# jypjypjypjyp/lvio_fusion

Measured on AMD Instinct MI355X. Metric: local-BA iters/sec (50 KF x 10k pts) + ICP Mpairs/sec, higher is better.
Workload: dtype f64; 1 GPU; configs[3]: full sliding-window LM iteration, 50 keyframes x 10 000 landmarks (10000 TwoCamera + 71789 TwoFrame + 9629 PoseOnly + 49 IMU factors), device-resident LM loop, one independent window per GPU; n_kf=50, n_lm=10000, parallelism=1 independent windows

## Files before the change

### lvio_fusion_amd/csrc/solver_kernels.hip

```cpp
#include <hip/hip_ext.h>
#include <algorithm>
#include <chrono>
#include <cmath>
#include <cstdlib>
#include <memory>
#include <unordered_map>

#include "factor_eval.hpp"
#include "prior_eval.hpp"
#include "lvf_internal.hpp"
#include "imu_eval.hpp"

namespace lvf {
struct TfWork;
struct LmCtl;
struct Chain;
struct StageClock;
struct SpNode { int col, row_off, m, id; };
constexpr int kSpMaxLevels = 12, kSpMaxRows = 768;
struct SpLevels { int n; int first[kSpMaxLevels]; int count[kSpMaxLevels]; };
struct JacobiDev { GP<double> h0; GP<const int> frozen; };
struct SpSrc {
  GP<const double> B; int ldB, dp; GP<const double> gc; GP<const double> radius; GP<const int> rows_nat;
  GP<int> wait_counter; int wait_target; GP<int> done_counter;
  int fenced; unsigned timeout_ticks;
  int strip_end;
  int rmw_read;
  GP<unsigned long long> dbg;
  int s_zero;
  JacobiDev jac{nullptr, nullptr};
};
struct SpArgs {
  GP<const SpNode> nodes; int first, tiles; GP<const int> rows; GP<double> S; int ld; GP<double> W; int wstride; GP<double> Lout; GP<int> fail; int nblocks; GP<const int> done;
  SpSrc src;
};
__device__ __forceinline__ void sp_ride(const int vb, const SpArgs& a);
constexpr int kFailSparse = 100000, kFailHandover = 300000;
}
struct lvf_problem {
  lvf_ctx* ctx = nullptr;
  lvf_state* st = nullptr;
  lvf_batch *tc = nullptr, *tf = nullptr, *po = nullptr, *imu = nullptr, *prior = nullptr;
  int n_kf = 0, n_lm = 0, d = 0, dp = 0, ldE = 0, dpad = 0, nb = 0;
  int ld = 0, off = 0, off_pose = 0, ndense = 0, aug = 0, sp_wstride = 0;
  lvf::SpLevels sp_levels{};
  std::vector<int> sp_tiles, sp_shmem;
  std::vector<int> sp_item0, sp_items;
  std::vector<int32_t> plan_key;
  lvf::DevBuf<lvf::SpNode> sp_nodes;
  lvf::DevBuf<int> sp_rows, sp_rows_nat, sp_owner, perm, iperm;
  lvf::DevBuf<int> lm_kmin, lm_kmax, lm_order, lm_nactive;
  bool band_ready = false;
  bool compact = false;
  lvf::DevBuf<int> lm_eoff, n_slots, tf_slot, run_first;
  lvf::DevBuf<double> slotB, slabP, slabQ, Ct, grt;
  lvf::StageClock* clk = nullptr;
  bool accum_clean = false;
  const double* chain_tcw = nullptr;
  int band_rows = 64;
  lvf::DevBuf<int4> band_work; lvf::DevBuf<int> n_band_work_dev; lvf::HostPin<int> h_n_band_work;
  int n_band_work = 0, band_rows_built = 0;
  bool band_pending = false; hipEvent_t ev_band = nullptr;
  int band_epoch = 0;
  std::vector<lvf_problem_batch*> batches;
  lvf::HostPin<int> h_run_first;
  lvf::DevBuf<unsigned long long> dbg, dbg_lin, dbg_sp;
  lvf::DevBuf<double> dbg_hist;
  lvf::DevBuf<double> sp_sync;
  lvf::DevBuf<double> sp_W, sp_L, Dinv;
  lvf::DevBuf<double> Ldiag;
  std::vector<int> perm_h;
  lvf::DevBuf<double> B, gc, C, gr, E, Cd, S, dxc, dxl, scal;
  lvf::DevBuf<double> jh0;
  lvf::DevBuf<double> poses2, vel2, ba2, bg2, invd2;
  lvf::DevBuf<uint8_t> pose_const;
  lvf::DevBuf<int> fail;
  lvf::DevBuf<lvf::TfWork> tf_work;
  lvf::HostPin<lvf::TfWork> h_tf_work;
  std::vector<uint8_t> pose_const_h;
  bool linearized = false;
  lvf::DevBuf<double2> tfs_fo, tfs_ob;
  lvf::DevBuf<int> tfs_lm, tfs_k1, tfs_k2, tfs_perm;
  lvf::HostPin<int> h_tfs_perm;
  bool tf_sorted_copy = false;
  const double2* tf_fo() const { return tf_sorted_copy ? tfs_fo.p : (const double2*)tf->ob_a.p; }
  const double2* tf_ob() const { return tf_sorted_copy ? tfs_ob.p : (const double2*)tf->ob_b.p; }
  const int* tf_lm() const { return tf_sorted_copy ? tfs_lm.p : tf->idx_a.p; }
  const int* tf_k1() const { return tf_sorted_copy ? tfs_k1.p : tf->idx_b.p; }
  const int* tf_k2() const { return tf_sorted_copy ? tfs_k2.p : tf->idx_c.p; }
  bool tf_unique_lk2 = false;
  bool tf_k1_first = false;
  double last_radius = 0;
  lvf::DevBuf<lvf::LmCtl> ctl;
  lvf::LmCtl* rec = nullptr;
  lvf::HostPin<lvf::LmCtl> h_ctl;
  lvf::Chain* chain = nullptr;
  bool chain_ready = false;
  bool no_chain = false;
  int unchained_solves = 0;
  int handover_retries = 0;
  int force_handover_timeouts = 0;
  const void* chain_state[6] = {nullptr, nullptr, nullptr, nullptr, nullptr, nullptr};
  double huber = 1.0;
  hipGraphExec_t graph_exec = nullptr;
  ~lvf_problem();
};

namespace lvf {

constexpr int kT = 256;
typedef double double4_t __attribute__((ext_vector_type(4)));
constexpr int kStripes = 32;
enum { SC_COST = 0, SC_COST_NEW = 1 * kStripes, SC_MODEL = 2 * kStripes, SC_DXNORM = 3 * kStripes, SC_XNORM = 4 * kStripes, SC_GMAX = 5 * kStripes,
       SC_N = 6 * kStripes, SC_FAIL = SC_N , SC_TICKET = SC_N + 1 , SC_ALLOC = SC_N + 2 };
static inline double stripe_sum(const double* h, int slot) { double s = 0.0; for (int k = 0; k < kStripes; ++k) s += h[slot + k]; return s; }

__device__ __forceinline__ int done_flag_issue(const int* done) { return done ? *reinterpret_cast<const volatile int*>(done) : 0; }

__device__ __forceinline__ void block_add(double v, double* dst) {
  v = wave_sum(v);
  if ((threadIdx.x & 63) == 0 && v != 0.0) atomicAdd(dst + ((blockIdx.x + blockIdx.y) & (kStripes - 1)), v);
}

struct StateP { GP<const double> poses, vel, ba, bg, inv_depth, w_kf; };

struct LmCtl {
  double radius, decrease;
  double last_radius;
  double cost, initial_cost;
  double cost_before, cost_after, model, dxnorm, xnorm, gmax;
  double huber, function_tol, gradient_tol, parameter_tol, min_rel_decrease;
  int max_iters;
  int iter, successes, invalid_run;
  int accepted, solved;
  int done, termination;
  int why, rejected;
  int jfrozen;
};

__device__ __forceinline__ void add_block66(double* __restrict__ B, int ld, int ra, int rb, const double Ja[12], const double Jb[12]) {
#pragma unroll
  for (int i = 0; i < 6; ++i)
#pragma unroll
    for (int j = 0; j < 6; ++j) {
      if (ra == rb && j > i) continue;
      atomicAdd(&B[(size_t)(ra + i) * ld + rb + j], Ja[i] * Jb[j] + Ja[6 + i] * Jb[6 + j]);
    }
}

__device__ __forceinline__ void zero_lower(double* __restrict__ p, const int ld, const unsigned long long wave, const unsigned long long n_waves) {
  const int lane = threadIdx.x & 63;
  for (unsigned long long r = wave; r < (unsigned long long)ld; r += n_waves) {
    double2* row = reinterpret_cast<double2*>(p + r * (unsigned long long)ld);
    const int end2 = min(ld, (((int)r | 63) + 1)) / 2;
    for (int c = lane; c < end2; c += 64) row[c] = make_double2(0.0, 0.0);
  }
}
__global__ __launch_bounds__(kT) void k_zero_multi(ZeroList z) {
  double* p = z.p[blockIdx.y];
  if (z.tri[blockIdx.y] > 0) { zero_lower(p, z.tri[blockIdx.y], (unsigned long long)blockIdx.x * (kT / 64) + (threadIdx.x >> 6), (unsigned long long)gridDim.x * (kT / 64)); return; }
  const unsigned long long n = z.n[blockIdx.y], n2 = n / 2;
  double2* p2 = reinterpret_cast<double2*>(p);
  for (unsigned long long i = (unsigned long long)blockIdx.x * kT + threadIdx.x; i < n2; i += (unsigned long long)gridDim.x * kT) p2[i] = make_double2(0.0, 0.0);
  if ((n & 1) && blockIdx.x == 0 && threadIdx.x == 0) p[n - 1] = 0.0;
}
__global__ __launch_bounds__(kT) void k_zero_multi_ranges(ZeroList z, int n_lm, int* __restrict__ kmin, int* __restrict__ kmax) {
  if ((int)blockIdx.y == z.count) {
    for (int l = blockIdx.x * kT + threadIdx.x; l < n_lm; l += gridDim.x * kT) { kmin[l] = 0x7fffffff; kmax[l] = -1; }
    return;
  }
  double* p = z.p[blockIdx.y];
  const unsigned long long n = z.n[blockIdx.y], n2 = n / 2;
  double2* p2 = reinterpret_cast<double2*>(p);
  for (unsigned long long i = (unsigned long long)blockIdx.x * kT + threadIdx.x; i < n2; i += (unsigned long long)gridDim.x * kT) p2[i] = make_double2(0.0, 0.0);
  if ((n & 1) && blockIdx.x == 0 && threadIdx.x == 0) p[n - 1] = 0.0;
}
__device__ __forceinline__ void zero_list_share(const ZeroList& zero, const int wg, const int n_wgs) {
  const unsigned long long t = (unsigned long long)wg * kT + threadIdx.x, nt = (unsigned long long)n_wgs * kT;
#pragma unroll
  for (int a = 0; a < kZeroListMax; ++a) {
    if (a >= zero.count) break;
    double* p = zero.p[a];
    if (zero.tri[a] > 0) { zero_lower(p, zero.tri[a], (unsigned long long)wg * (kT / 64) + (threadIdx.x >> 6), (unsigned long long)n_wgs * (kT / 64)); continue; }
    const unsigned long long cnt = zero.n[a], n2 = cnt / 2;
    double2* p2 = reinterpret_cast<double2*>(p);
    for (unsigned long long i = t; i < n2; i += nt) p2[i] = make_double2(0.0, 0.0);
    if ((cnt & 1) && t == 0) p[cnt - 1] = 0.0;
  }
}
__global__ __launch_bounds__(kT) void k_zero_table(const ZeroList* __restrict__ t) { zero_list_share(t[blockIdx.y], blockIdx.x, gridDim.x); }

template <bool COST_ONLY>
__device__ __forceinline__ void lin_tc_body(const int vb, int n, const double2* __restrict__ lo, const double2* __restrict__ ro,
                                               const int* __restrict__ lm, const int* __restrict__ kf, const double* __restrict__ wblk, StateP s,
                                               CamD left, CamD right, double huber, double* __restrict__ C,
                                               double* __restrict__ gr, double* __restrict__ cost) {
  const int i = vb * kT + threadIdx.x;
  double c = 0.0;
  if (i < n) {
    const int l = lm[i];
    const double2 a = lo[i], b = ro[i];
    double r[2], J[2];
    eval_two_camera<!COST_ONLY>(left, right, a.x, a.y, b.x, b.y, s.inv_depth[l], wblk ? wblk[i] : 5.0 * s.w_kf[kf[i]], r, J);
    double rho;
    const double sc = robust_scale(huber, r[0] * r[0] + r[1] * r[1], rho);
    c = 0.5 * rho;
    if (!COST_ONLY) {
      const double s2 = sc * sc;
      atomicAdd(&C[l], s2 * (J[0] * J[0] + J[1] * J[1]));
      atomicAdd(&gr[l], s2 * (J[0] * r[0] + J[1] * r[1]));
    }
  }
  block_add(c, cost);
}
template <bool COST_ONLY>
__global__ __launch_bounds__(kT) void k_lin_tc(int n, const double2* __restrict__ lo, const double2* __restrict__ ro,
                                               const int* __restrict__ lm, const int* __restrict__ kf, const double* __restrict__ wblk, StateP s,
                                               CamD left, CamD right, double huber, double* __restrict__ C,
                                               double* __restrict__ gr, double* __restrict__ cost) { lin_tc_body<COST_ONLY>(blockIdx.x, n, lo, ro, lm, kf, wblk, s, left, right, huber, C, gr, cost); }

// ... 467 lines not shown
                                               int ld, double* __restrict__ gc, double* __restrict__ cost) { lin_po_body<COST_ONLY>(blockIdx.x, n, n_kf, ob, kf, pwi, pw, s, cam, huber, pose_const, B, ld, gc, cost); }

struct ImuJ { GP<const double> j[8]; };
__global__ __launch_bounds__(64) void k_lin_imu(int n, int n_kf, const double* __restrict__ res, ImuJ J, const int* __restrict__ kf_i,
                                                const int* __restrict__ kf_j, const double* __restrict__ poses,
                                                const uint8_t* __restrict__ pose_const, double* __restrict__ B, int ld,
                                                double* __restrict__ gc, double* __restrict__ cost) {
  __shared__ double sJ[15 * 30];
  __shared__ double sr[15];
  __shared__ int sidx[30];
  const int f = blockIdx.x, lane = threadIdx.x;
  const int ki = kf_i[f], kj = kf_j[f];
  if (lane < 15) sr[lane] = res[(size_t)f * 15 + lane];
  if (lane < 30) {
    int g;
    if (lane < 6) g = 6 * ki + lane; else if (lane < 15) g = 6 * n_kf + 9 * ki + (lane - 6);
    else if (lane < 21) g = 6 * kj + (lane - 15); else g = 6 * n_kf + 9 * kj + (lane - 21);
    sidx[lane] = g;
  }
  for (int e = lane; e < 30; e += 64) {
    const int row = e % 15, which = e / 15;
    const double* Jr = (which ? J.j[4] : J.j[0]) + (size_t)f * 105 + 7 * row;
    const int kk = which ? kj : ki;
    const double* q = poses + 7 * kk;
    const double sc = (pose_const[kk] & 1) ? 0.0 : 1.0;
    double l3[3];
    quat_row_to_local(Jr, q, l3);
    double* o = sJ + row * 30 + (which ? 15 : 0);
    o[0] = sc * l3[0]; o[1] = sc * l3[1]; o[2] = sc * l3[2]; o[3] = sc * Jr[4]; o[4] = sc * Jr[5]; o[5] = sc * Jr[6];
  }
  for (int e = lane; e < 15 * 18; e += 64) {
    const int row = e / 18, c = e % 18, blk = c / 3, cc = c % 3;
    const int src = blk < 3 ? 1 + blk : 5 + (blk - 3);
    const double* jp = src == 1 ? J.j[1] : (src == 2 ? J.j[2] : (src == 3 ? J.j[3] : (src == 5 ? J.j[5] : (src == 6 ? J.j[6] : J.j[7]))));
    const double scv = ((pose_const[blk < 3 ? ki : kj] >> (1 + blk % 3)) & 1) ? 0.0 : 1.0;
    sJ[row * 30 + (blk < 3 ? 6 + 3 * blk : 21 + 3 * (blk - 3)) + cc] = scv * jp[(size_t)f * 45 + 3 * row + cc];
  }
  __syncthreads();
  double c = 0.0;
  if (lane < 15) c = 0.5 * sr[lane] * sr[lane];
  c = wave_sum(c);
  if (lane == 0) atomicAdd(cost + (blockIdx.x & (kStripes - 1)), c);
  for (int e = lane; e < 30 * 30; e += 64) {
    const int a = e / 30, b = e % 30;
    const int ga = sidx[a], gb = sidx[b];
    if (gb > ga || (ga == gb && a != b)) continue;
    double h = 0.0;
#pragma unroll
    for (int k = 0; k < 15; ++k) h += sJ[k * 30 + a] * sJ[k * 30 + b];
    atomicAdd(&B[(size_t)ga * ld + gb], h);
  }
  if (lane < 30) {
    double g = 0.0;
#pragma unroll
    for (int k = 0; k < 15; ++k) g += sJ[k * 30 + lane] * sr[k];
    atomicAdd(&gc[sidx[lane]], g);
  }
}

template <bool DYN = false>
__device__ __forceinline__ void lin_imu_body4(const int vb, int n, int n_kf, const double* __restrict__ res, ImuJ J, const int* __restrict__ kf_i,
                                              const int* __restrict__ kf_j, const double* __restrict__ poses,
                                              const uint8_t* __restrict__ pose_const, double* __restrict__ B, int ld,
                                              double* __restrict__ gc, double* __restrict__ cost) {
  __shared__ double sJ4[DYN ? 1 : 4 * 15 * 30];
  __shared__ double sr4[DYN ? 1 : 4 * 16];
  __shared__ int sidx4[DYN ? 1 : 4 * 32];
  extern __shared__ double lin_lds[];
  const int w = threadIdx.x >> 6, lane = threadIdx.x & 63;
  const int f = 4 * vb + w;
  const bool active = f < n;
  double* sJ = (DYN ? lin_lds : sJ4) + w * 450;
  double* sr = (DYN ? lin_lds + 1800 : sr4) + w * 16;
  int* sidx = (DYN ? reinterpret_cast<int*>(lin_lds + 1864) : sidx4) + w * 32;
  if (active) {
    const int ki = kf_i[f], kj = kf_j[f];
    if (lane < 15) sr[lane] = res[(size_t)f * 15 + lane];
    if (lane < 30) {
      int g;
      if (lane < 6) g = 6 * ki + lane; else if (lane < 15) g = 6 * n_kf + 9 * ki + (lane - 6);
      else if (lane < 21) g = 6 * kj + (lane - 15); else g = 6 * n_kf + 9 * kj + (lane - 21);
      sidx[lane] = g;
    }
    for (int e = lane; e < 30; e += 64) {
      const int row = e % 15, which = e / 15;
      const double* Jr = (which ? J.j[4] : J.j[0]) + (size_t)f * 105 + 7 * row;
      const int kk = which ? kj : ki;
      const double* q = poses + 7 * kk;
      const double sc = (pose_const[kk] & 1) ? 0.0 : 1.0;
      double l3[3];
      quat_row_to_local(Jr, q, l3);
      double* o = sJ + row * 30 + (which ? 15 : 0);
      o[0] = sc * l3[0]; o[1] = sc * l3[1]; o[2] = sc * l3[2]; o[3] = sc * Jr[4]; o[4] = sc * Jr[5]; o[5] = sc * Jr[6];
    }
    for (int e = lane; e < 15 * 18; e += 64) {
      const int row = e / 18, c = e % 18, blk = c / 3, cc = c % 3;
      const int src = blk < 3 ? 1 + blk : 5 + (blk - 3);
      const double* jp = src == 1 ? J.j[1] : (src == 2 ? J.j[2] : (src == 3 ? J.j[3] : (src == 5 ? J.j[5] : (src == 6 ? J.j[6] : J.j[7]))));
      const double scv = ((pose_const[blk < 3 ? ki : kj] >> (1 + blk % 3)) & 1) ? 0.0 : 1.0;
      sJ[row * 30 + (blk < 3 ? 6 + 3 * blk : 21 + 3 * (blk - 3)) + cc] = scv * jp[(size_t)f * 45 + 3 * row + cc];
    }
  }
  __syncthreads();
  double c = 0.0;
  if (active && lane < 15) c = 0.5 * sr[lane] * sr[lane];
  c = wave_sum(c);
  if (!active) return;
  if (lane == 0) atomicAdd(cost + (f & (kStripes - 1)), c);
  for (int e = lane; e < 30 * 30; e += 64) {
    const int a = e / 30, b = e % 30;
    const int ga = sidx[a], gb = sidx[b];
    if (gb > ga || (ga == gb && a != b)) continue;
    double h = 0.0;
#pragma unroll
    for (int k = 0; k < 15; ++k) h += sJ[k * 30 + a] * sJ[k * 30 + b];
    atomicAdd(&B[(size_t)ga * ld + gb], h);
  }
  if (lane < 30) {
    double g = 0.0;
#pragma unroll
    for (int k = 0; k < 15; ++k) g += sJ[k * 30 + lane] * sr[k];
    atomicAdd(&gc[sidx[lane]], g);
  }
}

constexpr int kEndZeroWgs = 192;
constexpr int kImuWaveLds = 225 + 480 + 480 + 16 + 16 + 16 + 248 + 32 + 2;
__device__ __forceinline__ void lin_imu_eval_body(const int f, const ImuEvalArgs& I, int n_kf, const StateP& s, const uint8_t* __restrict__ pose_const,
                                                  double* __restrict__ B, int ld, double* __restrict__ gc, double* __restrict__ cost, unsigned long long* dbg) {
  extern __shared__ double lin_lds[];
  const int tid = threadIdx.x;
  if (f >= I.n) return;
  if (f != 0 || tid != 0) dbg = nullptr;
  if (dbg) dbg[0] = wall_clock64();
  double* sS = lin_lds;
  double* sM = sS + 225;
  double* sJw = sM + 480;
  double* sr0 = sJw + 480;
  double* sr = sr0 + 16;
  int* sidx = reinterpret_cast<int*>(sr + 16);
  double* sP = reinterpret_cast<double*>(sidx + 32);
  double* sX = sP + 248;
  const int ki = I.kf_i[f], kj = I.kf_j[f];
  for (int k = tid; k < 225; k += kT) sS[k] = I.sqrt_info[(size_t)f * 225 + k];
  for (int k = tid; k < OFF_COV; k += kT) sP[k] = I.pre[(size_t)f * kPre + k];
  if (tid < 32) {
    const int kk = tid < 16 ? ki : kj, c = tid & 15;
    sX[tid] = c < 7 ? s.poses[7 * kk + c] : (c < 10 ? s.vel[3 * kk + c - 7] : (c < 13 ? s.ba[3 * kk + c - 10] : s.bg[3 * kk + c - 13]));
  }
  int* smask = reinterpret_cast<int*>(sX + 32);
  if (tid >= 32 && tid < 34) smask[tid - 32] = pose_const[tid == 32 ? ki : kj];
  for (int k = tid; k < 480; k += kT) sM[k] = 0.0;
  __syncthreads();
  if (dbg) dbg[1] = wall_clock64();
  if (tid == 0) imu_raw16<true>(sP, sX, sr0, sM);
  __syncthreads();
  if (dbg) dbg[2] = wall_clock64();
  {
    const double r = imu_weighted_residual(tid, sS, sr0);
    if (tid < 15) sr[tid] = r;
    for (int e = tid; e < 480; e += kT) sJw[e] = imu_weighted_jacobian(e, sS, sM);
    if (tid < 30) {
      int g;
      if (tid < 6) g = 6 * ki + tid; else if (tid < 15) g = 6 * n_kf + 9 * ki + (tid - 6);
      else if (tid < 21) g = 6 * kj + (tid - 15); else g = 6 * n_kf + 9 * kj + (tid - 21);
      sidx[tid] = g;
    }
  }
  __syncthreads();
  double* sJ = sM;
  if (tid < 30) {
    const int row = tid % 15, which = tid / 15;
    const double* Jr = sJw + 32 * row + (which ? 16 : 0);
    const double sc = (smask[which] & 1) ? 0.0 : 1.0;
    double l3[3];
    quat_row_to_local(Jr, sX + 16 * which, l3);
    double* o = sJ + row * 30 + (which ? 15 : 0);
    o[0] = sc * l3[0]; o[1] = sc * l3[1]; o[2] = sc * l3[2]; o[3] = sc * Jr[4]; o[4] = sc * Jr[5]; o[5] = sc * Jr[6];
  }
  for (int e = tid; e < 15 * 18; e += kT) {
    const int row = e / 18, c = e % 18;
    const int cg = c < 9 ? c / 3 : (c - 9) / 3;
    const double scv = ((smask[c < 9 ? 0 : 1] >> (1 + cg)) & 1) ? 0.0 : 1.0;
    sJ[row * 30 + (c < 9 ? 6 + c : 21 + (c - 9))] = scv * sJw[32 * row + (c < 9 ? 7 + c : 23 + (c - 9))];
  }
  __syncthreads();
  if (dbg) dbg[3] = wall_clock64();
  if (tid < 64) {
    double c = tid < 15 ? 0.5 * sr[tid] * sr[tid] : 0.0;
    c = wave_sum(c);
    if (tid == 0) atomicAdd(cost + (f & (kStripes - 1)), c);
  }
  for (int e = tid; e < 30 * 30; e += kT) {
    const int a = e / 30, b = e % 30;
    const int ga = sidx[a], gb = sidx[b];
    if (gb > ga || (ga == gb && a != b)) continue;
    double h = 0.0;
#pragma unroll
    for (int k = 0; k < 15; ++k) h += sJ[k * 30 + a] * sJ[k * 30 + b];
    atomicAdd(&B[(size_t)ga * ld + gb], h);
  }
  if (tid < 30) {
    double g = 0.0;
#pragma unroll
    for (int k = 0; k < 15; ++k) g += sJ[k * 30 + tid] * sr[k];
    atomicAdd(&gc[sidx[tid]], g);
  }
  if (dbg) dbg[4] = wall_clock64();
}

struct LinVisual {
  int n_tfw, g_tc;
  GP<const TfWork> work; GP<const double2> tf_fo, tf_ob; GP<const int> tf_lm, tf_k1; CamD tf_left, tf_right; int unique_lk2; TfCompact cp;
  int n_tc; GP<const double2> tc_lo, tc_ro; GP<const int> tc_lm, tc_kf; GP<const double> tc_w; CamD tc_left, tc_right;
  int n_po, g_po; GP<const double2> po_ob; GP<const int> po_kf, po_pwi; GP<const double> po_pw; CamD po_cam;
  int n_imu; GP<const double> imu_res; ImuJ imu_J; GP<const int> imu_i, imu_j; ImuEvalArgs imu;
};
struct LinArgs {
  LinVisual v; int n_kf; StateP s; double huber; GP<const uint8_t> pose_const; GP<double> B; int ld; GP<double> gc; GP<double> E; int ldE; GP<double> C, gr, cost;
  int nblocks; GP<const int> done; GP<unsigned long long> dbg; int rows;
  GP<double> scal_reset;
};
__device__ __forceinline__ void reset_step_scalars(double* scal) {
  for (int k = SC_COST_NEW + threadIdx.x; k < SC_N; k += kT) scal[k] = 0.0;
  if (threadIdx.x == 0) { *reinterpret_cast<int*>(scal + SC_FAIL) = 0; *reinterpret_cast<int*>(scal + SC_TICKET) = 0; }
}
__device__ __forceinline__ void lin_visual_body(const int bx, const LinArgs& A) {
  if (bx >= A.nblocks || (A.done && *A.done)) return;
  if (bx == 0 && A.scal_reset) reset_step_scalars(A.scal_reset);
  const LinVisual& a = A.v;
  const int g_imu_first = a.imu.pre ? a.n_imu : 0;
  const int b = bx - g_imu_first;
  const int n_kf = A.n_kf; const StateP s = A.s; const double huber = A.huber; const uint8_t* pose_const = A.pose_const;
  double* B = A.B; const int ld = A.ld; double* gc = A.gc; double* E = A.E; const int ldE = A.ldE; double* C = A.C; double* gr = A.gr; double* cost = A.cost;
  if (bx < g_imu_first)
    lin_imu_eval_body(bx, a.imu, n_kf, s, pose_const, B, ld, gc, cost, A.dbg ? A.dbg + (size_t)a.n_tfw * 8 : nullptr);
  else if (b < a.n_tfw)
    lin_tf_sorted_body<true>(b, a.work, n_kf, a.tf_fo, a.tf_ob, a.tf_lm, a.tf_k1, s, a.tf_left, a.tf_right, huber, pose_const, B, ld, gc, E, ldE, C, gr, cost,
                       a.unique_lk2, A.dbg, a.cp, a.n_tfw);
  else if (b < a.n_tfw + a.g_tc)
    lin_tc_body<false>(b - a.n_tfw, a.n_tc, a.tc_lo, a.tc_ro, a.tc_lm, a.tc_kf, a.tc_w, s, a.tc_left, a.tc_right, huber, C, gr, cost);
  else if (b < a.n_tfw + a.g_tc + a.g_po)
    lin_po_body<false, true>(b - a.n_tfw - a.g_tc, a.n_po, n_kf, a.po_ob, a.po_kf, a.po_pwi, a.po_pw, s, a.po_cam, huber, pose_const, B, ld, gc, cost);
  else
    lin_imu_body4<true>(b - a.n_tfw - a.g_tc - a.g_po, a.n_imu, n_kf, a.imu_res, a.imu_J, a.imu_i, a.imu_j, s.poses, pose_const, B, ld, gc, cost);
}
__global__ __launch_bounds__(kT) __attribute__((amdgpu_waves_per_eu(3))) void k_lin_visual(LinArgs a) { lin_visual_body(blockIdx.x, a); }
__global__ __launch_bounds__(kT) __attribute__((amdgpu_waves_per_eu(3))) void k_lin_visual_b(const LinArgs* __restrict__ t) { lin_visual_body(blockIdx.x, t[blockIdx.y]); }
__global__ __launch_bounds__(kT) __attribute__((amdgpu_waves_per_eu(3))) void k_lin_visual_bt(const LinArgs* __restrict__ t) { lin_visual_body(blockIdx.y, t[blockIdx.x]); }

struct TfReduceArgs {
  int n_kf, n_wg; GP<const int> run_first; GP<const double> slabP, slabQ; GP<double> B; int ld; GP<double> gc; int nblocks; GP<const int> done;
  int own_blocks; SpArgs ride;
};
__device__ __forceinline__ void tf_reduce_body(const int bx0, const TfReduceArgs& A) {
  if (bx0 >= A.nblocks || (A.done && *A.done)) return;
  if (bx0 < A.ride.nblocks) { sp_ride(bx0, A.ride); return; }
  const int bx = bx0 - A.ride.nblocks;
  const int n_kf = A.n_kf;
  const int nchunk = (A.n_wg + 63) / 64;
  if (bx < n_kf * nchunk) {
    __shared__ double part[8][32];
    const int k = bx / nchunk, c = bx - k * nchunk, v = threadIdx.x & 31, g = threadIdx.x >> 5;
    const int r0 = A.run_first[k], r1 = A.run_first[k + 1];
    double acc = 0.0;
    if (v < 27) {
      const double* slabP = A.slabP; const double* slabQ = A.slabQ;
      double t8[8]; bool keep[8];
#pragma unroll
      for (int u = 0; u < 8; ++u) {
        const int wg = 64 * c + g + 8 * u, wgc = min(wg, A.n_wg - 1);
        const bool useP = wgc >= r1;
        keep[u] = (wg < A.n_wg) & (wgc >= r0);
        const double* src = useP ? slabP + ((size_t)wgc * n_kf + k) * kSlabRow + v : slabQ + (size_t)wgc * kSlabQ + v;
        t8[u] = *src;
      }
#pragma unroll
      for (int u = 0; u < 8; ++u) acc = keep[u] ? acc + t8[u] : acc;
    }
    part[g][v] = acc;
    __syncthreads();
    if (threadIdx.x < 27) {
      double t = 0.0;
#pragma unroll
      for (int q = 0; q < 8; ++q) t += part[q][threadIdx.x];
      if (t != 0.0) {
        if (threadIdx.x < 21) {
          int x = 0, rem = threadIdx.x;
          while (rem > x) { rem -= x + 1; ++x; }
          atomicAdd(&A.B[(size_t)(6 * k + x) * A.ld + 6 * k + rem], t);
        } else atomicAdd(&A.gc[6 * k + threadIdx.x - 21], t);
      }
    }
    return;
  }
  const int e = (bx - n_kf * nchunk) * kT + threadIdx.x;
  const int npair = n_kf * (n_kf - 1) / 2;
  if (e >= npair * 36) return;
  const int pr = e / 36, el = e - 36 * pr;
  int k2 = (int)((1.0 + sqrt(1.0 + 8.0 * pr)) * 0.5);
  while (k2 * (k2 - 1) / 2 > pr) --k2;
  while ((k2 + 1) * k2 / 2 <= pr) ++k2;
  const int k1 = pr - k2 * (k2 - 1) / 2;
  double acc = 0.0;
  {
    const double* slabP = A.slabP;
    const int w0 = A.run_first[k2], w1 = A.run_first[k2 + 1];
    for (int wg = w0; wg < w1; wg += 4) {
      double t4[4];
#pragma unroll
      for (int u = 0; u < 4; ++u) t4[u] = slabP[((size_t)min(wg + u, w1 - 1) * n_kf + k1) * kSlabRow + 27 + el];
#pragma unroll
      for (int u = 0; u < 4; ++u) acc = (wg + u < w1) ? acc + t4[u] : acc;
    }
  }
  if (acc != 0.0) {
    const int x = el / 6, y = el - 6 * x;
    A.B[(size_t)(6 * k2 + x) * A.ld + 6 * k1 + y] += acc;
  }
}
__global__ __launch_bounds__(kT) void k_tf_reduce(TfReduceArgs a) { tf_reduce_body(blockIdx.x, a); }
__global__ __launch_bounds__(kT) void k_tf_reduce_b(const TfReduceArgs* __restrict__ t) { tf_reduce_body(blockIdx.x, t[blockIdx.y]); }
__global__ __launch_bounds__(kT) void k_tf_reduce_bt(const TfReduceArgs* __restrict__ t) { tf_reduce_body(blockIdx.y, t[blockIdx.x]); }


__device__ __forceinline__ void lin_prior_block(const int i, const int a, const int b, const double* __restrict__ res, const double* __restrict__ ja,
                                                const double* __restrict__ jb, const double* __restrict__ poses, const uint8_t* __restrict__ pose_const,
                                                double* __restrict__ B, int ld, double* __restrict__ gc, double* __restrict__ cost) {
  double r[6], La[36], Lb[36];
  double c = 0.0;
  for (int k = 0; k < 6; ++k) { r[k] = res[k]; c += 0.5 * r[k] * r[k]; }
  for (int k = 0; k < 6; ++k) {
    const double* row = jb + 7 * k;
    const double sc = (pose_const[b] & 1) ? 0.0 : 1.0;
    double l3[3];
    quat_row_to_local(row, poses + 7 * b, l3);
    Lb[6 * k] = sc * l3[0]; Lb[6 * k + 1] = sc * l3[1]; Lb[6 * k + 2] = sc * l3[2];
    Lb[6 * k + 3] = sc * row[4]; Lb[6 * k + 4] = sc * row[5]; Lb[6 * k + 5] = sc * row[6];
    if (a >= 0) {
      const double* rowa = ja + 7 * k;
      const double sa = (pose_const[a] & 1) ? 0.0 : 1.0;
      quat_row_to_local(rowa, poses + 7 * a, l3);
      La[6 * k] = sa * l3[0]; La[6 * k + 1] = sa * l3[1]; La[6 * k + 2] = sa * l3[2];
      La[6 * k + 3] = sa * rowa[4]; La[6 * k + 4] = sa * rowa[5]; La[6 * k + 5] = sa * rowa[6];
    }
  }
  atomicAdd(cost + (i & (kStripes - 1)), c);
  for (int x = 0; x < 6; ++x) {
    double g = 0.0;
    for (int k = 0; k < 6; ++k) g += Lb[6 * k + x] * r[k];
    atomicAdd(&gc[6 * b + x], g);
    for (int y = 0; y <= x; ++y) {
      double h = 0.0;
      for (int k = 0; k < 6; ++k) h += Lb[6 * k + x] * Lb[6 * k + y];
      atomicAdd(&B[(size_t)(6 * b + x) * ld + 6 * b + y], h);
    }
  }
  if (a >= 0) {
    for (int x = 0; x < 6; ++x) {
      double g = 0.0;
      for (int k = 0; k < 6; ++k) g += La[6 * k + x] * r[k];
      atomicAdd(&gc[6 * a + x], g);
      for (int y = 0; y <= x; ++y) {
        double h = 0.0;
        for (int k = 0; k < 6; ++k) h += La[6 * k + x] * La[6 * k + y];
        atomicAdd(&B[(size_t)(6 * a + x) * ld + 6 * a + y], h);
      }
      for (int y = 0; y < 6; ++y) {
        double h = 0.0;
        for (int k = 0; k < 6; ++k) h += La[6 * k + x] * Lb[6 * k + y];
        if (a > b) atomicAdd(&B[(size_t)(6 * a + x) * ld + 6 * b + y], h);
        else atomicAdd(&B[(size_t)(6 * b + y) * ld + 6 * a + x], h);
      }
    }
  }
}
__global__ __launch_bounds__(64) void k_lin_prior(int n, const double* __restrict__ res, const double* __restrict__ ja,
                                                  const double* __restrict__ jb, const int* __restrict__ kf_a, const int* __restrict__ kf_b,
                                                  const double* __restrict__ poses, const uint8_t* __restrict__ pose_const,
                                                  double* __restrict__ B, int ld, double* __restrict__ gc, double* __restrict__ cost) {
  const int i = blockIdx.x * 64 + threadIdx.x;
  if (i >= n) return;
  lin_prior_block(i, kf_a[i], kf_b[i], res + 6 * i, ja + (size_t)42 * i, jb + (size_t)42 * i, poses, pose_const, B, ld, gc, cost);
}
struct PriorArgs { int n; GP<const int> kf_a, kf_b; GP<const double> target, weight, vv; };
__global__ __launch_bounds__(64) void k_prior_lin(PriorArgs P, const double* __restrict__ poses, const uint8_t* __restrict__ pose_const,
                                                  double* __restrict__ B, int ld, double* __restrict__ gc, double* __restrict__ cost) {
  const int i = blockIdx.x * 64 + threadIdx.x;
  if (i >= P.n) return;
  double res[6], ja[42], jb[42];
  const int a = P.kf_a[i], b = P.kf_b[i];
  pose_prior_eval<true>(a, b, P.target + 7 * i, P.weight[i], P.vv[i], poses, res, ja, jb);
  lin_prior_block(i, a, b, res, ja, jb, poses, pose_const, B, ld, gc, cost);
}
__global__ __launch_bounds__(64) void k_prior_cost(PriorArgs P, const double* __restrict__ poses, double* __restrict__ cost) {
  const int i = blockIdx.x * 64 + threadIdx.x;
  if (i >= P.n) return;
  double res[6];
  pose_prior_eval<false>(P.kf_a[i], P.kf_b[i], P.target + 7 * i, P.weight[i], P.vv[i], poses, res, nullptr, nullptr);
  double c = 0.0;
  for (int k = 0; k < 6; ++k) c += 0.5 * res[k] * res[k];
  atomicAdd(cost + (i & (kStripes - 1)), c);
}
__global__ __launch_bounds__(kT) void k_cost_sq(int n, const double* __restrict__ res, double* __restrict__ cost) {
  const int i = blockIdx.x * kT + threadIdx.x;
  double c = 0.0;
  if (i < n) { const double r = res[i]; c = 0.5 * r * r; }
  block_add(c, cost);
}

__device__ __forceinline__ double lm_damping(double h, double h0) {
  if (h >= 2e-6 * (1.0 + h0) && h < 1e32) return h;
  if (h0 == 0.0) return fmin(fmax(h, 1e-6), 1e32);
  const double sj = 1.0 / (1.0 + sqrt(h0)), s2 = sj * sj;
  return fmin(fmax(h * s2, 1e-6), 1e32) / s2;
}
__device__ __forceinline__ double lm_damping_own(double h, const JacobiDev& j, int slot, int frozen, double h0_loaded) {
  double h0 = h0_loaded;
  if (!frozen) { h0 = h; j.h0[slot] = h; }
  return lm_damping(h, h0);
}

struct PrepArgs {
  int ld, dpad, jl0 ; GP<const int> iperm; GP<const double> B, gc; GP<const double> radius; GP<double> S; unsigned nS_blocks; int n_lm, dp, ldE; GP<const double> C, gr;
  GP<double> Cd, E, scal; int nblocks; GP<const int> done;
  GP<const int> eoff, kmin, kmax; GP<const double> slotB; GP<double> Ct, grt;
  int early, off;
  int own_blocks; SpArgs ride;
  JacobiDev jac;
};
__device__ __forceinline__ void prepare_body(const unsigned bx0, const PrepArgs& A) {
  if (bx0 >= (unsigned)A.nblocks || (A.done && *A.done)) return;
  if (bx0 < (unsigned)A.ride.nblocks) { sp_ride((int)bx0, A.ride); return; }
  const unsigned bx = bx0 - (unsigned)A.ride.nblocks;
  const int ld = A.ld, dpad = A.dpad; const int* __restrict__ iperm = A.iperm; const double* __restrict__ B = A.B; const double* __restrict__ gc = A.gc;
  const double inv_radius = 1.0 / *A.radius;
  const int jf = *A.jac.frozen;
  double* __restrict__ S = A.S; const unsigned nS_blocks = A.nS_blocks; const int n_lm = A.n_lm, dp = A.dp, ldE = A.ldE;
  const double* __restrict__ C = A.C; const double* __restrict__ gr = A.gr; double* __restrict__ Cd = A.Cd; double* __restrict__ E = A.E; double* __restrict__ scal = A.scal;
  if (bx == 0 && scal) reset_step_scalars(scal);
  if (bx >= nS_blocks) {
    if (A.slotB) {
      const int l = ((bx - nS_blocks) * kT + threadIdx.x) >> 3, j0 = threadIdx.x & 7;
      const bool live = l < n_lm;
      const int lc = live ? l : 0;
      const int k1 = A.kmin[lc], len = live ? max(0, A.kmax[lc] - k1) : 0;
      const double h0l = A.jac.h0[A.jl0 + lc];
      const double2* sb = reinterpret_cast<const double2*>(A.slotB + (size_t)A.eoff[lc] * 8);
      double v[8] = {0, 0, 0, 0, 0, 0, 0, 0};
      for (int j = j0; j < len; j += 8) {
        const double2 b0 = sb[4 * j], b1 = sb[4 * j + 1], b2 = sb[4 * j + 2], cg = sb[4 * j + 3];
        v[0] += cg.x; v[1] += cg.y; v[2] += b0.x; v[3] += b0.y; v[4] += b1.x; v[5] += b1.y; v[6] += b2.x; v[7] += b2.y;
      }
#pragma unroll
      for (int q = 0; q < 8; ++q) { v[q] = quad_sum(v[q]); v[q] += quad_perm<0x141>(v[q]); }
      if (live && j0 == 0) {
        const double c = C[l] + v[0], g = gr[l] + v[1];
        A.Ct[l] = c; A.grt[l] = g;
        Cd[l] = c + lm_damping_own(c, A.jac, A.jl0 + l, jf, h0l) * inv_radius;
        double* el = E + (size_t)l * ldE;
        el[dp] = g;
        if (len > 0) {
#pragma unroll
          for (int q = 0; q < 6; ++q) el[6 * k1 + q] = v[2 + q];
        }
      }
      return;
    }
    const int l = (bx - nS_blocks) * kT + threadIdx.x;
    if (l >= n_lm) return;
    const double c = C[l], h0l = A.jac.h0[A.jl0 + l];
    Cd[l] = c + lm_damping_own(c, A.jac, A.jl0 + l, jf, h0l) * inv_radius;
    E[(size_t)l * ldE + dp] = gr[l];
    return;
  }
  const size_t e = (size_t)bx * kT + threadIdx.x;
  const int n0 = A.early ? A.off : 0, nn = ld - n0;
  const int half = (nn + 1) / 2;
  if (e >= (size_t)half * (nn + 1)) return;
  const int q = (int)(e / (nn + 1)), cc = (int)(e % (nn + 1));
  int I, J;
  if (cc <= q) { I = q; J = cc; }
  else { I = nn - 1 - q; J = cc - q - 1; if (I == q) return; }
  I += n0; J += n0;
  const int oi = iperm[I], oj = iperm[J];
  double v = 0.0;
  if (oi >= 0) {
    if (oj >= 0 && J <= I) {
      const double h0d = I == J ? A.jac.h0[oi] : 0.0;
      v = B[(size_t)max(oi, oj) * dpad + min(oi, oj)];
      if (I == J) v += lm_damping_own(v, A.jac, oi, jf, h0d) * inv_radius;
    }
  } else if (oi == -2) {
    v = (oj >= 0) ? -gc[oj] : (J == I ? 1e300 : 0.0);
  } else if (I == J) {
    v = 1.0;
  }
  if (!A.early) S[(size_t)I * ld + J] = v;
  else if (v != 0.0) atomicAdd(&S[(size_t)I * ld + J], v);
}
__global__ __launch_bounds__(kT) void k_prepare(PrepArgs a) { prepare_body(blockIdx.x, a); }
__global__ __launch_bounds__(kT) void k_prepare_b(const PrepArgs* __restrict__ t) { prepare_body(blockIdx.x, t[blockIdx.y]); }
__global__ __launch_bounds__(kT) void k_prepare_bt(const PrepArgs* __restrict__ t) { const PrepArgs a = t[blockIdx.x]; prepare_body(blockIdx.y, a); }

constexpr int kSchurChunk = 512;
__global__ __launch_bounds__(64) void k_schur_syrk(int n_lm, int dp, int ldE, int ntile, const double* __restrict__ E,
                                                   const double* __restrict__ Cd, int d, int ldS, double* __restrict__ S) {
  int t = blockIdx.x, ti = 0;
  while (t >= ti + 1) { t -= ti + 1; ++ti; }
  const int tj = t;
  const int lane = threadIdx.x, lk = lane >> 4, lc = lane & 15;
  const int k_begin = blockIdx.y * kSchurChunk, k_end = min(n_lm, k_begin + kSchurChunk);
  double4_t acc = {0.0, 0.0, 0.0, 0.0};
  for (int k0 = k_begin; k0 < k_end; k0 += 4) {
    const int l = k0 + lk;
    double a = 0.0, b = 0.0;
    if (l < k_end) {
      const double* row = E + (size_t)l * ldE;
      a = row[ti * 16 + lc] / Cd[l];
      b = row[tj * 16 + lc];
    }
    acc = __builtin_amdgcn_mfma_f64_16x16x4f64(a, b, acc, 0, 0, 0);
  }
#pragma unroll
  for (int r = 0; r < 4; ++r) {
    const int gi = ti * 16 + lk + 4 * r, gj = tj * 16 + lc;
    const double v = acc[r];
    if (v == 0.0) continue;
    if (gi < dp && gj < dp) { if (gj <= gi) atomicAdd(&S[(size_t)gi * ldS + gj], -v); }
    else if (gi == dp && gj < dp) atomicAdd(&S[(size_t)d * ldS + gj], v);
  }
}

constexpr int kSchurGroups = 8, kSchurTilesPerWave = 8, kSchurRows = 16;
__global__ __launch_bounds__(256) void k_schur_lds(int n_lm, int dp, int ldE, int ntile, int rows_per_slice, const double* __restrict__ E,
                                                   const double* __restrict__ Cd, int d, int ldS, double* __restrict__ S) {
  extern __shared__ double sh[];
  double* Es = sh;
  double* icd = sh + kSchurRows * ldE;
  const int tid = threadIdx.x, w = tid >> 6, lane = tid & 63, lk = lane >> 4, lc = lane & 15;
  const int g = blockIdx.x, slice = blockIdx.y;
  const int k_begin = slice * rows_per_slice, k_end = min(n_lm, k_begin + rows_per_slice);
  int ti[kSchurTilesPerWave], tj[kSchurTilesPerWave], nt = 0;
#pragma unroll
  for (int s_ = 0; s_ < kSchurTilesPerWave; ++s_) {
    const int t = g + kSchurGroups * (w + 4 * s_);
    ti[s_] = 0; tj[s_] = 0;
    if (t < ntile) {
      int a = (int)((sqrt(8.0 * t + 1.0) - 1.0) * 0.5);
      while ((a + 1) * (a + 2) / 2 <= t) ++a;
      while (a * (a + 1) / 2 > t) --a;
      ti[s_] = a; tj[s_] = t - a * (a + 1) / 2;
      nt = s_ + 1;
    }
  }
  double4_t acc[kSchurTilesPerWave];
#pragma unroll
  for (int s_ = 0; s_ < kSchurTilesPerWave; ++s_) acc[s_] = double4_t{0.0, 0.0, 0.0, 0.0};
  const int per_row = ldE;
  const int total = kSchurRows * per_row;
  constexpr int kPf = 20;
  double pf[kPf];
  auto fetch = [&](int k0) {
#pragma unroll
    for (int u = 0; u < kPf; ++u) {
      const int e = tid + 256 * u;
      double v = 0.0;
      if (e < total) { const int rr = e / per_row, cc = e - rr * per_row; if (k0 + rr < k_end) v = E[(size_t)(k0 + rr) * ldE + cc]; }
      pf[u] = v;
    }
  };
  auto fetch_tail = [&](int k0) {
    for (int e = tid + 256 * kPf; e < total; e += 256) {
      const int rr = e / per_row, cc = e - rr * per_row;
      Es[e] = (k0 + rr < k_end) ? E[(size_t)(k0 + rr) * ldE + cc] : 0.0;
    }
  };
  if (k_begin < k_end) fetch(k_begin);
  for (int k0 = k_begin; k0 < k_end; k0 += kSchurRows) {
    __syncthreads();
#pragma unroll
    for (int u = 0; u < kPf; ++u) { const int e = tid + 256 * u; if (e < total) Es[e] = pf[u]; }
    fetch_tail(k0);
    if (tid < kSchurRows) icd[tid] = (k0 + tid < k_end) ? 1.0 / Cd[k0 + tid] : 0.0;
    __syncthreads();
    if (k0 + kSchurRows < k_end) fetch(k0 + kSchurRows);
// ... 732 lines not shown
        for (int c = 0; c < 9; ++c) { const int oj = nb0 + c; sv[c] += src.B[(size_t)max(oi, oj) * src.ldB + min(oi, oj)]; }
      }
    }
    finish_row(r, sv);
  }
  if (tile == 0 && tid < 9) {
    double xcol[9];
#pragma unroll
    for (int r = 0; r < 9; ++r) {
      double v = (r == tid) ? 1.0 : 0.0;
#pragma unroll
      for (int k = 0; k < r; ++k) v -= L[r * 9 + k] * xcol[k];
      xcol[r] = v * linv[r];
    }
#pragma unroll
    for (int r = 0; r < 9; ++r) Lout[(size_t)ni * 81 + r * 9 + tid] = xcol[r];
  }
  __syncthreads();
  int ns = 0;
  if (src.done_counter && src.strip_end > 0) {
    int lo = 0, hi = m;
    while (lo < hi) { const int mid = (lo + hi) >> 1; if (rws[mid] < src.strip_end) lo = mid + 1; else hi = mid; }
    ns = lo;
  }
  auto pair_value = [&](const int r, const int c2) {
    const double* wr = Ws + r * 9;
    const double* wc = Ws + c2 * 9;
    double v = 0.0;
#pragma unroll
    for (int c = 0; c < 9; ++c) v += wr[c] * wc[c];
    return v;
  };
  auto pair_update = [&](const int r, const int c2) {
    const double v = pair_value(r, c2);
    if (v != 0.0) atomicAdd(&S[(size_t)rws[r] * ld + rws[c2]], -v);
  };
  if (ns > 0) {
    double sink = 0.0;
    for (int q = tile * 256 + tid; q < ns * m; q += tiles * 256) {
      const int r = q / ns, c2 = q - r * ns;
      if (r >= c2) {
        const double v = pair_value(r, c2);
        if (v != 0.0) sink += __hip_atomic_fetch_add(&S[(size_t)rws[r] * ld + rws[c2]], -v, __ATOMIC_RELAXED, __HIP_MEMORY_SCOPE_AGENT);
      }
    }
    if (sink == -1.2345678901234567e301) atomicMax(fail, 50000);
  }
  if (stamp) stamp[5] = wall_clock64();
  if (src.done_counter) {
    __syncthreads();
    if (tid == 0) {
      if (src.fenced) __hip_atomic_fetch_add((int*)src.done_counter, 1, __ATOMIC_RELEASE, __HIP_MEMORY_SCOPE_AGENT);
      else __hip_atomic_fetch_add((int*)src.done_counter, 1, __ATOMIC_RELAXED, __HIP_MEMORY_SCOPE_AGENT);
    }
  }
  if (stamp) stamp[6] = wall_clock64();
  const int m2 = m - ns, P = m2 * (m2 + 1) / 2;
  for (int p = tile * 256 + tid; p < P; p += tiles * 256) {
    int r = (int)((sqrt(8.0 * p + 1.0) - 1.0) * 0.5);
    while ((r + 1) * (r + 2) / 2 <= p) ++r;
    while (r * (r + 1) / 2 > p) --r;
    const int c2 = p - r * (r + 1) / 2;
    pair_update(r + ns, c2 + ns);
  }
  if (stamp) { asm volatile("s_waitcnt vmcnt(0)" ::: "memory"); stamp[7] = wall_clock64(); }
}
__global__ __launch_bounds__(64) void k_band_work(int rows, int dp, const int* __restrict__ n_active_p, const int* __restrict__ order,
                                                  const int* __restrict__ kmin, const int* __restrict__ kmax, int4* __restrict__ work, int* __restrict__ n_work) {
  const int n_active = *n_active_p, lane = threadIdx.x;
  const int k_begin = blockIdx.x * rows, k_end = min(n_active, k_begin + rows);
  if (k_begin >= k_end) return;
  int lo = 0x7fffffff, hi = -1;
  for (int r = k_begin + lane; r < k_end; r += 64) { const int l = order[r]; lo = min(lo, kmin[l]); hi = max(hi, kmax[l]); }
  for (int o = 32; o > 0; o >>= 1) { lo = min(lo, __shfl_xor(lo, o)); hi = max(hi, __shfl_xor(hi, o)); }
  if (lane == 0) {
    const int t0 = (6 * lo) >> 4, t1 = (6 * hi + 5) >> 4, tl = dp >> 4, nbt = t1 - t0 + 1;
    const int ntiles = nbt * (nbt + 1) / 2 + (tl > t1 ? nbt : 0);
    const int groups = (ntiles + kBandTilesPerGroup - 1) / kBandTilesPerGroup;
    const int base = atomicAdd(n_work, groups);
    for (int g = 0; g < groups; ++g) work[base + g] = make_int4((int)blockIdx.x, g, lo | (hi << 16), k_end);
  }
}

__device__ __forceinline__ void sp_ride(const int vb, const SpArgs& a) {
  if (vb >= a.nblocks) return;
  sp_eliminate_body(vb, a.nodes, a.first, a.tiles, a.rows, a.S, a.ld, a.W, a.wstride, a.Lout, a.fail, a.done, a.src);
}
__global__ __launch_bounds__(256) void k_sp_eliminate(SpArgs a) { sp_ride(blockIdx.x, a); }
__global__ __launch_bounds__(256) void k_sp_eliminate_b(const SpArgs* __restrict__ t) { sp_ride(blockIdx.x, t[blockIdx.y]); }
struct SchurSp0Args {
  int n_slices, n_groups, dp, ldE; GP<const double> E, Cd; GP<const int> order, n_active, kmin, kmax; int d_local, ldS; GP<double> S_pose;
  SpArgs sp;
  SpArgs sp_b, sp_c;
  int nblocks; GP<const int> done; GP<unsigned long long> dbg; int rows;
  GP<const int4> work; int n_work;
};
__device__ __forceinline__ void schur_sp0_body(const int b, const SchurSp0Args& A) {
  if (b >= A.nblocks) return;
  if (A.work) {
    const int n_a = A.sp.nblocks, n_b = A.sp_b.nblocks, n_c = A.sp_c.nblocks, n_sp = n_a + n_b + n_c;
    if (b < n_a) sp_ride(b, A.sp);
    else if (b < n_a + n_b) sp_ride(b - n_a, A.sp_b);
    else if (b < n_sp) sp_ride(b - n_a - n_b, A.sp_c);
    else {
      const int dv = done_flag_issue(A.done);
      const int4* item = A.work + (b - n_sp);
      const int4 it = *item;
      if (dv) return;
      schur_band_body(it.x, it.y, A.dp, A.ldE, A.E, A.Cd, A.order, A.n_active, A.kmin, A.kmax, A.d_local, A.ldS, A.S_pose, A.dbg ? A.dbg + (size_t)(b - n_sp) * 8 : nullptr, A.rows, item);
    }
    return;
  }
  if (A.done && *A.done) return;
  const int ns = A.n_slices * A.n_groups;
  if (b < ns) schur_band_body(b % A.n_slices, b / A.n_slices, A.dp, A.ldE, A.E, A.Cd, A.order, A.n_active, A.kmin, A.kmax, A.d_local, A.ldS, A.S_pose, A.dbg ? A.dbg + (size_t)b * 8 : nullptr, A.rows);
  else sp_ride(b - ns, A.sp);
}
__global__ __launch_bounds__(256) __attribute__((amdgpu_waves_per_eu(2))) void k_schur_sp0(SchurSp0Args a) { schur_sp0_body(blockIdx.x, a); }
__global__ __launch_bounds__(256) __attribute__((amdgpu_waves_per_eu(2))) void k_schur_sp0_b(const SchurSp0Args* __restrict__ t) { schur_sp0_body(blockIdx.x, t[blockIdx.y]); }
__global__ __launch_bounds__(256) __attribute__((amdgpu_waves_per_eu(2))) void k_schur_sp0_bt(const SchurSp0Args* __restrict__ t) { schur_sp0_body(blockIdx.y, t[blockIdx.x]); }
struct SpBack {
  SpLevels lv;
  int item0[kSpMaxLevels], items[kSpMaxLevels];
  GP<const SpNode> nodes; GP<const int> rows; GP<const int> owner; GP<const double> W; GP<const double> Linv; GP<const int> perm;
  int off, aug, d_total, total_items, n_nodes, max_count, linv_in_lds;
  int prod_items;
  GP<unsigned long long> dbg;
};

__device__ __forceinline__ void lds_barrier() { asm volatile("s_waitcnt lgkmcnt(0)\n\ts_barrier" ::: "memory"); }

template <typename T>
__device__ __forceinline__ T ld_off32(const T* base, unsigned byte_off) {
  return *reinterpret_cast<const T*>(reinterpret_cast<const char*>(base) + byte_off);
}
constexpr int kBT = 512, kBParts = kBT / 64, kBackPre = 256 / kBParts, kBackInv = 64 / kBParts, kTailPre = 6;
struct BackArgs { GP<const double> Sd; int ld, d; GP<const double> Dinv; GP<double> xout; SpBack sp; GP<const int> done; GP<const double> Ldiag; GP<int> pose_ready = nullptr; int n_pose = 0; int pose_fenced = 0; };
__device__ __forceinline__ void chol_backsolve_body(const BackArgs& A) {
  const int dv = done_flag_issue(A.done);
  const double* S = A.Sd; const int ld = A.ld, d = A.d; const double* Dinv = A.Dinv; double* xout = A.xout; const SpBack& sp = A.sp;
  extern __shared__ double sm[];
  const int tid = threadIdx.x, c = tid & 63, part = tid >> 6;
  const int nblk = (d + kNB - 1) / kNB, n = nblk * kNB;
  double* x = sm + sp.off;
  double* partial = x + n;
  double* rhs = partial + kBParts * kNB;
  double* accs = rhs + kNB;
  double* linv = accs + 9 * sp.max_count;
  double* part1 = linv + (sp.linv_in_lds ? 81 * sp.n_nodes : 0);
  double* prod = part1 + kBT;
  int* snode = reinterpret_cast<int*>(prod + 9 * (size_t)sp.prod_items);
  int stamp = 0;
  auto mark = [&]() { if (sp.dbg && tid == 0) sp.dbg[stamp++] = wall_clock64(); };
  mark();
  const int rend = min(n, d);
  double gl[kBackPre], xi[kBackInv], yv;
  const int part_u = __builtin_amdgcn_readfirstlane(part);
  const unsigned c_off = 8u * (unsigned)c;
  auto prefetch = [&](int kb) {
    const int r0 = kb * kNB, below = nblk - 1 - kb;
    const double* row = S + (size_t)(r0 + kNB + part_u) * ld + r0;
#pragma unroll
    for (int g = 0; g < kBackPre / 8; ++g)
      if (g < below) {
#pragma unroll
        for (int j = 0; j < 8; ++j) gl[8 * g + j] = ld_off32(row + (size_t)(kBParts * (8 * g + j)) * ld, c_off);
      }
    const double* dv = Dinv + (size_t)kb * kNB * kNB + kBackInv * part_u;
#pragma unroll
    for (int t = 0; t < kBackInv; ++t) xi[t] = ld_off32(dv + t, (unsigned)kNB * c_off);
    const double* yrow = (d / kNB == kb) ? A.Ldiag + (size_t)kb * kNB * kNB + (size_t)(d - r0) * kNB : S + (size_t)d * ld + r0;
    yv = (r0 + c < d) ? ld_off32(yrow, c_off) : 0.0;
  };
  prefetch(nblk - 1);
  constexpr int kLinvPre = 8;
  double lpre[kLinvPre];
  const int n_linv = sp.linv_in_lds ? 81 * sp.n_nodes : 0;
#pragma unroll
  for (int u = 0; u < kLinvPre; ++u) { const int i = tid + kBT * u; lpre[u] = i < n_linv ? ld_off32((const double*)sp.Linv, 8u * (unsigned)i) : 0.0; }
  SpNode ndpre = SpNode{0, 0, 0, 0};
  if (tid < sp.n_nodes) ndpre = sp.nodes[tid];
#pragma unroll
  for (int u = 0; u < kLinvPre; ++u) { const int i = tid + kBT * u; if (i < n_linv) linv[i] = lpre[u]; }
  for (int i = tid + kBT * kLinvPre; i < n_linv; i += kBT) linv[i] = sp.Linv[i];
  if (tid < sp.n_nodes) { snode[2 * tid] = ndpre.row_off; snode[2 * tid + 1] = ndpre.m; }
  for (int i = tid + kBT; i < sp.n_nodes; i += kBT) { const SpNode nd = sp.nodes[i]; snode[2 * i] = nd.row_off; snode[2 * i + 1] = nd.m; }
  asm volatile("" ::: "memory");
  int tR[kTailPre], tK[kTailPre];
  double tW[kTailPre][9];
#pragma unroll
  for (int u = 0; u < kTailPre; ++u) {
    const int g = tid + kBT * u;
    const bool ok = g < sp.total_items;
    tR[u] = -1; tK[u] = 0;
#pragma unroll
    for (int q = 0; q < 9; ++q) tW[u][q] = 0.0;
    if (ok) {
      tR[u] = ld_off32((const int*)sp.rows, 4u * (unsigned)g);
      tK[u] = ld_off32((const int*)sp.owner, 4u * (unsigned)g);
#pragma unroll
      for (int q = 0; q < 9; ++q) tW[u][q] = ld_off32((const double*)sp.W, 8u * ((unsigned)q * (unsigned)sp.total_items + (unsigned)g));
    }
  }
// ... 129 lines not shown
    const int i0 = kmin ? 6 * min(kmin[l], dp / 6) : 0, i1 = kmin ? 6 * (kmax[l] + 1) : dp;
    for (int i = (i0 & ~15) + q; i < i1; i += 16) ed += e[i] * sdx[i];
    ed = row16_sum(ed);
    if (q == 0) {
      const double g_l = gr[l];
      const double dl = (-g_l - ed) / Cd[l];
      gmx = fmax(gmx, fabs(g_l));
      dxl[l] = dl;
      invd2[l] = inv_depth[l] + dl;
      m += -0.5 * dl * ((Cd[l] - C[l]) * dl - g_l);
      n2 += dl * dl; x2 += inv_depth[l] * inv_depth[l];
    }
  }
  __shared__ double red[4][NT / 64];
  m = wave_sum(m); n2 = wave_sum(n2); x2 = wave_sum(x2);
  for (int o = 32; o > 0; o >>= 1) gmx = fmax(gmx, __shfl_down(gmx, o));
  if ((threadIdx.x & 63) == 0) { red[0][threadIdx.x >> 6] = m; red[1][threadIdx.x >> 6] = n2; red[2][threadIdx.x >> 6] = x2; red[3][threadIdx.x >> 6] = gmx; }
  __syncthreads();
  if (threadIdx.x < 3) {
    double v = 0.0;
    for (int k = 0; k < NT / 64; ++k) v += red[threadIdx.x][k];
    double* dst = scal + (threadIdx.x == 0 ? SC_MODEL : (threadIdx.x == 1 ? SC_DXNORM : SC_XNORM));
    if (v != 0.0) atomicAdd(dst + (vb & (kStripes - 1)), v);
  } else if (threadIdx.x == 3) {
    double v = 0.0;
    for (int k = 0; k < NT / 64; ++k) v = fmax(v, red[3][k]);
    if (v != 0.0) atomicMax(reinterpret_cast<unsigned long long*>(scal + SC_GMAX + (vb & (kStripes - 1))), (unsigned long long)__double_as_longlong(v));
  }
}
template <int NT = kT, int PARTS = 3>
__device__ __forceinline__ void apply_step_body(const int vb, int n_kf, int n_lm, StateP s, const double* __restrict__ dxc, const double* __restrict__ dxl,
                                                double* __restrict__ poses2, double* __restrict__ vel2, double* __restrict__ ba2,
                                                double* __restrict__ bg2, double* __restrict__ invd2, double* __restrict__ scal, int d, int ld,
                                                const double* __restrict__ B, const double* __restrict__ gc, double inv_radius,
                                                const unsigned char* __restrict__ pose_const, const JacobiDev jac) {
  const int i = vb * NT + threadIdx.x;
  double m = 0.0, n2 = 0.0, g = 0.0, x2 = 0.0;
  if (i < d && ((PARTS & 1) || i >= 6 * n_kf) && ((PARTS & 2) || i < 6 * n_kf)) {
    const double dx = dxc[i];
    const double h = B[(size_t)i * ld + i], h0d = jac.h0[i];
    m = -0.5 * dx * (lm_damping(h, *jac.frozen ? h0d : h) * inv_radius * dx - gc[i]);
    const bool rot = i < 6 * n_kf && (i % 6) < 3;
    n2 = rot ? 0.0 : dx * dx;
    g = fabs(gc[i]);
  }
  const int cm_kf = (i < n_kf && pose_const) ? pose_const[i] : 0;
  if (i < n_kf && (PARTS & 1)) {
    const double* p = s.poses + 7 * i; const double* dlt = dxc + 6 * i;
    const double nrm = sqrt(dlt[0] * dlt[0] + dlt[1] * dlt[1] + dlt[2] * dlt[2]);
    double* o = poses2 + 7 * i;
    if (nrm > 0.0) {
      const double sn = sin(nrm) / nrm, cw = cos(nrm);
      const double dx = sn * dlt[0], dy = sn * dlt[1], dz = sn * dlt[2];
      const double xw = p[3], xx = p[0], xy = p[1], xz = p[2];
      o[3] = cw * xw - dx * xx - dy * xy - dz * xz;
      o[0] = cw * xx + dx * xw + dy * xz - dz * xy;
      o[1] = cw * xy - dx * xz + dy * xw + dz * xx;
      o[2] = cw * xz + dx * xy - dy * xx + dz * xw;
    } else { o[0] = p[0]; o[1] = p[1]; o[2] = p[2]; o[3] = p[3]; }
    for (int c = 0; c < 3; ++c) o[4 + c] = p[4 + c] + dlt[3 + c];
    for (int c = 0; c < 4; ++c) n2 += (o[c] - p[c]) * (o[c] - p[c]);
    if (!(cm_kf & 1)) for (int c = 0; c < 7; ++c) x2 += p[c] * p[c];
  }
  if (i < n_kf && (PARTS & 2)) {
    const int cm = cm_kf;
    const double* dv = dxc + 6 * n_kf + 9 * i;
    for (int c = 0; c < 3; ++c) { vel2[3 * i + c] = s.vel[3 * i + c] + dv[c]; ba2[3 * i + c] = s.ba[3 * i + c] + dv[3 + c]; bg2[3 * i + c] = s.bg[3 * i + c] + dv[6 + c]; }
    for (int c = 0; c < 3; ++c)
      x2 += ((cm & 2) ? 0.0 : s.vel[3 * i + c] * s.vel[3 * i + c]) + ((cm & 4) ? 0.0 : s.ba[3 * i + c] * s.ba[3 * i + c]) + ((cm & 8) ? 0.0 : s.bg[3 * i + c] * s.bg[3 * i + c]);
  }
  if (i < n_lm) invd2[i] = s.inv_depth[i] + dxl[i];
  if (vb * NT < d) {
    block_add(m, scal + SC_MODEL); block_add(n2, scal + SC_DXNORM);
    for (int o = 32; o > 0; o >>= 1) g = fmax(g, __shfl_down(g, o));
    if ((threadIdx.x & 63) == 0) atomicMax(reinterpret_cast<unsigned long long*>(scal + SC_GMAX + (vb & (kStripes - 1))), (unsigned long long)__double_as_longlong(g));
  }
  block_add(x2, scal + SC_XNORM);
}

struct TailArgs {
  int g_lm, n_lm, dp, ldE; GP<const double> E, C, Cd, gr, dxc; GP<double> dxl, scal; GP<const int> kmin, kmax; int n_kf; StateP s;
  GP<double> poses2, vel2, ba2, bg2, invd2; int d, ld; GP<const double> B, gc; GP<const double> radius; int nblocks; GP<const int> done;
  GP<const unsigned char> pose_const; JacobiDev jac;
};
__device__ __forceinline__ void step_tail_body(const int bx, const TailArgs& A) {
  if (bx >= A.nblocks || (A.done && *A.done)) return;
  if (bx < A.g_lm) landmark_back_body(bx, A.g_lm, A.n_lm, A.dp, A.ldE, A.E, A.C, A.Cd, A.gr, A.dxc, A.s.inv_depth, A.dxl, A.invd2, A.scal, A.kmin, A.kmax);
  else apply_step_body(bx - A.g_lm, A.n_kf, 0, A.s, A.dxc, A.dxl, A.poses2, A.vel2, A.ba2, A.bg2, A.invd2, A.scal, A.d, A.ld, A.B, A.gc, 1.0 / *A.radius, A.pose_const, A.jac);
}
__global__ __launch_bounds__(kT) void k_step_tail(TailArgs a) { step_tail_body(blockIdx.x, a); }
__global__ __launch_bounds__(kT) void k_step_tail_b(const TailArgs* __restrict__ t) { step_tail_body(blockIdx.x, t[blockIdx.y]); }
__global__ __launch_bounds__(kT) void k_step_tail_bt(const TailArgs* __restrict__ t) { step_tail_body(blockIdx.y, t[blockIdx.x]); }

struct BackTailArgs { BackArgs back; TailArgs tail; int g_lm; int fenced; unsigned timeout_ticks; GP<int> fail; };
__global__ __launch_bounds__(kBT) void k_backsolve_tail(BackTailArgs a) {
  if (a.back.done && *a.back.done) return;
  const TailArgs& T = a.tail;
  if (blockIdx.x == 0) {
    chol_backsolve_body(a.back);
    __builtin_amdgcn_fence(__ATOMIC_RELEASE, "workgroup");
    __syncthreads();
    const double inv_radius = 1.0 / *T.radius;
    for (int vb = 0; vb * kBT < max(T.d, T.n_kf); ++vb)
      apply_step_body<kBT, 2>(vb, T.n_kf, 0, T.s, T.dxc, T.dxl, T.poses2, T.vel2, T.ba2, T.bg2, T.invd2, T.scal, T.d, T.ld, T.B, T.gc, inv_radius, T.pose_const, T.jac);
    if (a.back.sp.dbg && threadIdx.x == 0) a.back.sp.dbg[55] = wall_clock64();
    return;
  }
  unsigned long long* ldbg = (a.back.sp.dbg && (blockIdx.x == 2 || blockIdx.x == gridDim.x - 1) && threadIdx.x == 0) ? a.back.sp.dbg + (blockIdx.x == 2 ? 56 : 59) : nullptr;
  if (ldbg) ldbg[0] = wall_clock64();
  if (threadIdx.x == 0) {
    const unsigned long long t0 = wall_clock64();
    while (__hip_atomic_load((int*)a.back.pose_ready, __ATOMIC_RELAXED, __HIP_MEMORY_SCOPE_AGENT) == 0) {
      __builtin_amdgcn_s_sleep(16);
      if (wall_clock64() - t0 > (unsigned long long)a.timeout_ticks) { atomicMax(a.fail, kFailHandover + 90000); break; }
    }
  }
  __syncthreads();
  if (a.fenced) __builtin_amdgcn_fence(__ATOMIC_ACQUIRE, "agent");
  if (ldbg) ldbg[1] = wall_clock64();
  if (blockIdx.x == 1) {
    extern __shared__ double sdx_pose[];
    for (int i = threadIdx.x; i < T.dp; i += kBT) sdx_pose[i] = __hip_atomic_load(T.dxc + i, __ATOMIC_RELAXED, __HIP_MEMORY_SCOPE_AGENT);
    __syncthreads();
    const double inv_radius = 1.0 / *T.radius;
    for (int vb = 0; vb * kBT < max(T.dp, T.n_kf); ++vb)
      apply_step_body<kBT, 1>(vb, T.n_kf, 0, T.s, sdx_pose, T.dxl, T.poses2, T.vel2, T.ba2, T.bg2, T.invd2, T.scal, T.d, T.ld, T.B, T.gc, inv_radius, T.pose_const, T.jac);
    return;
  }
  landmark_back_body<kBT, true>((int)blockIdx.x - 2, a.g_lm, T.n_lm, T.dp, T.ldE, T.E, T.C, T.Cd, T.gr, T.dxc, T.s.inv_depth, T.dxl, T.invd2, T.scal, T.kmin, T.kmax);
  if (ldbg) ldbg[2] = wall_clock64();
}

struct DecideArgs {
  GP<const double> scal; GP<LmCtl> ctl; GP<LmCtl> rec; GP<int> ticket;
  int n_kf, n_lm;
  GP<double> poses, vel, ba, bg, invd;
  GP<const double> poses2, vel2, ba2, bg2, invd2;
  GP<unsigned long long> dbg;
  GP<double> hist;
};
constexpr int kDT = 256;
template <bool COHERENT = false>
__device__ __forceinline__ void lm_decide_body(const DecideArgs& A) {
  __shared__ int s_commit, s_skip, s_iter, s_done;
  __shared__ double s_sum[8];
  LmCtl* c = A.ctl;
  if (A.dbg && threadIdx.x == 0) A.dbg[1] = wall_clock64();
  if (threadIdx.x == 0) s_skip = c->done;
  {
    const int wv = threadIdx.x >> 6, lane = threadIdx.x & 63;
    for (int slot = wv; slot < 6; slot += kDT / 64) {
      double v = lane < kStripes ? (COHERENT ? __hip_atomic_load(A.scal + slot * kStripes + lane, __ATOMIC_RELAXED, __HIP_MEMORY_SCOPE_AGENT) : A.scal[slot * kStripes + lane]) : 0.0;
      if (slot == SC_GMAX / kStripes) { for (int o = 32; o > 0; o >>= 1) v = fmax(v, __shfl_down(v, o)); }
      else v = wave_sum(v);
      if (lane == 0) s_sum[slot] = v;
    }
  }
  __syncthreads();
  if (s_skip) return;
  if (A.dbg && threadIdx.x == 0) A.dbg[2] = wall_clock64();
  if (threadIdx.x < kStripes) const_cast<double*>((const double*)A.scal)[SC_COST + threadIdx.x] = 0.0;
  if (threadIdx.x == 0) {
    struct { double radius, decrease, last_radius, cost, initial_cost, cost_before, cost_after, model, dxnorm, xnorm, gmax;
             double function_tol, gradient_tol, parameter_tol, min_rel_decrease; int max_iters, iter, successes, invalid_run, accepted, solved, done, termination, why, rejected; } lc;
    lc.radius = c->radius; lc.decrease = c->decrease; lc.cost = c->cost; lc.initial_cost = c->initial_cost;
    lc.function_tol = c->function_tol; lc.gradient_tol = c->gradient_tol; lc.parameter_tol = c->parameter_tol; lc.min_rel_decrease = c->min_rel_decrease;
    lc.max_iters = c->max_iters; lc.iter = c->iter; lc.successes = c->successes; lc.invalid_run = c->invalid_run; lc.done = c->done; lc.termination = c->termination; lc.why = c->why; lc.rejected = c->rejected;
    const int hfail = *reinterpret_cast<const int*>(A.scal + SC_FAIL);
    const double cost_before = s_sum[SC_COST / kStripes], cost_new = s_sum[SC_COST_NEW / kStripes], model = -s_sum[SC_MODEL / kStripes];
    const double dxnorm = sqrt(s_sum[SC_DXNORM / kStripes]), xnorm = sqrt(s_sum[SC_XNORM / kStripes]);
    const double gmax = s_sum[SC_GMAX / kStripes];
    const bool solved = hfail == 0 && isfinite(cost_new) && isfinite(model);
    const int it = lc.iter;
    if (it == 0) { lc.initial_cost = cost_before; lc.cost = cost_before; }
    lc.cost_before = cost_before; lc.model = model; lc.dxnorm = dxnorm; lc.xnorm = xnorm; lc.gmax = gmax; lc.solved = solved ? 1 : 0;
    lc.last_radius = lc.radius;
    bool accepted = false, done = false;
    int termination = 1, why = LVF_WHY_MAX_ITERATIONS;
    if (hfail >= kFailHandover) { done = true; termination = 2; why = LVF_WHY_HANDOVER; }
    else if (gmax <= lc.gradient_tol) { done = true; termination = 0; why = LVF_WHY_GRADIENT; }
    else if (lc.radius < 1e-32) { done = true; termination = 0; why = LVF_WHY_MIN_RADIUS; }
    else {
      const bool valid = solved && model > 0.0;
      if (!valid) {
        lc.iter = it + 1;
        lc.rejected += 1;
        lc.invalid_run += 1;
        if (lc.invalid_run >= 5) { done = true; termination = 2; why = LVF_WHY_INVALID_STEPS; }
        else lc.radius *= 0.5;
      } else {
        lc.invalid_run = 0;
        if (dxnorm <= lc.parameter_tol * (xnorm + lc.parameter_tol)) { done = true; termination = 0; why = LVF_WHY_PARAMETER; }
        else if (fabs(cost_before - cost_new) <= lc.function_tol * cost_before) { done = true; termination = 0; why = LVF_WHY_FUNCTION; }
        else {
          lc.iter = it + 1;
          const double rho = (cost_before - cost_new) / model;
          if (rho > lc.min_rel_decrease) {
            accepted = true;
            const double t = 2.0 * rho - 1.0;
            lc.radius = fmin(lc.radius / fmax(1.0 / 3.0, 1.0 - t * t * t), 1e16);
            lc.decrease = 2.0;
            lc.successes += 1;
            lc.cost = cost_new;
          } else {
            lc.radius = lc.radius / lc.decrease;
            lc.decrease *= 2.0;
            lc.rejected += 1;
          }
        }
      }
      if (!done && lc.iter >= lc.max_iters) { done = true; termination = 1; why = LVF_WHY_MAX_ITERATIONS; }
      else if (!done && lc.radius < 1e-32) { done = true; termination = 0; why = LVF_WHY_MIN_RADIUS; }
    }
    lc.cost_after = accepted ? cost_new : (solved ? cost_new : cost_before);
    lc.accepted = accepted ? 1 : 0;
    if (done) { lc.termination = termination; lc.why = why; lc.done = 1; }
    s_commit = accepted ? 1 : 0;
    c->radius = lc.radius; c->decrease = lc.decrease; c->last_radius = lc.last_radius; c->cost = lc.cost; c->initial_cost = lc.initial_cost;
    c->cost_before = lc.cost_before; c->cost_after = lc.cost_after; c->model = lc.model; c->dxnorm = lc.dxnorm; c->xnorm = lc.xnorm; c->gmax = lc.gmax;
    c->iter = lc.iter; c->successes = lc.successes; c->invalid_run = lc.invalid_run; c->accepted = lc.accepted; c->solved = lc.solved;
    c->done = lc.done; c->termination = lc.termination; c->why = lc.why; c->rejected = lc.rejected;
    if (hfail < kFailHandover) c->jfrozen = 1;
    s_iter = lc.iter; s_done = lc.done;
    if (A.hist) {
      double* h = A.hist + 8 * (it & 63);
      h[0] = (double)it; h[1] = cost_before; h[2] = cost_new; h[3] = model; h[4] = accepted ? 1.0 : 0.0; h[5] = (double)hfail; h[6] = lc.last_radius; h[7] = gmax;
    }
    if (A.dbg) A.dbg[3] = wall_clock64();
  }
  __syncthreads();
  if (s_commit) {
    const double2* __restrict__ p2 = reinterpret_cast<const double2*>((const double*)A.invd2);
    double2* __restrict__ q2 = reinterpret_cast<double2*>((double*)A.invd);
    const int n2 = A.n_lm / 2;
    for (int i0 = 0; i0 < n2; i0 += 8 * kDT) {
      double vx[8], vy[8];
#pragma unroll
      for (int u = 0; u < 8; ++u) { const double2 t = p2[min(i0 + u * kDT + (int)threadIdx.x, n2 - 1)]; vx[u] = t.x; vy[u] = t.y; }
#pragma unroll
      for (int u = 0; u < 8; ++u) q2[min(i0 + u * kDT + (int)threadIdx.x, n2 - 1)] = make_double2(vx[u], vy[u]);
    }
    if ((A.n_lm & 1) && threadIdx.x == 0) A.invd[A.n_lm - 1] = A.invd2[A.n_lm - 1];
    for (int i = threadIdx.x; i < 7 * A.n_kf; i += kDT) A.poses[i] = A.poses2[i];
    for (int i = threadIdx.x; i < 3 * A.n_kf; i += kDT) { A.vel[i] = A.vel2[i]; A.ba[i] = A.ba2[i]; A.bg[i] = A.bg2[i]; }
  }
  if (A.dbg && threadIdx.x == 0) A.dbg[4] = wall_clock64();
  if (A.rec && threadIdx.x == 0) {
    __hip_atomic_store(&A.rec->why, c->why, __ATOMIC_RELAXED, __HIP_MEMORY_SCOPE_SYSTEM);
    __hip_atomic_store(&A.rec->done, s_done, __ATOMIC_RELAXED, __HIP_MEMORY_SCOPE_SYSTEM);
    __hip_atomic_store(&A.rec->iter, s_iter, __ATOMIC_RELAXED, __HIP_MEMORY_SCOPE_SYSTEM);
  }
}
__global__ __launch_bounds__(kDT) void k_lm_decide(DecideArgs a) { lm_decide_body(a); }
__global__ __launch_bounds__(kDT) void k_lm_decide_b(const DecideArgs* __restrict__ t) { lm_decide_body(t[blockIdx.y]); }

static_assert(kDT == kT, "the last workgroup of the cost pass runs the decision with its own threads");
__device__ __forceinline__ void cost_decide_body(const int b, const CostArgs& A, const DecideArgs& D, const int end_zero) {
  if (b >= A.nblocks) {
    if (end_zero && b - A.nblocks < A.zero_wgs) zero_list_share(A.zero, b - A.nblocks, A.zero_wgs);
    return;
  }
  if (A.done && *A.done) return;
  __shared__ double s_part[kT / 64];
  if (D.dbg && threadIdx.x == 0 && (b == 0 || b == A.g_imu)) D.dbg[b == 0 ? 8 : 12] = wall_clock64();
  {
    double c;
    if (b >= A.g_imu) c = cost_visual_value(b - A.g_imu, A);
    else {
      __shared__ double sS[225];
      __shared__ double sP[OFF_COV];
      __shared__ double sr0[16];
      const int f = b;
      for (int k = threadIdx.x; k < 225; k += kT) sS[k] = A.imu.sqrt_info[(size_t)f * 225 + k];
      for (int k = threadIdx.x; k < OFF_COV; k += kT) sP[k] = A.imu.pre[(size_t)f * kPre + k];
      __syncthreads();
      if (D.dbg && threadIdx.x == 0 && b == 0) D.dbg[9] = wall_clock64();
      if (threadIdx.x == 0) imu_raw<false>(f, sP, A.imu.kf_i, A.imu.kf_j, A.s.poses, A.s.vel, A.s.ba, A.s.bg, sr0, nullptr);
      __syncthreads();
      if (D.dbg && threadIdx.x == 0 && b == 0) D.dbg[10] = wall_clock64();
      const double r = imu_weighted_residual(threadIdx.x, sS, sr0);
      c = threadIdx.x < 15 ? 0.5 * r * r : 0.0;
    }
    const double v = wave_sum(c);
    if ((threadIdx.x & 63) == 0) s_part[threadIdx.x >> 6] = v;
  }
  __shared__ int s_last;
  __syncthreads();
  if (threadIdx.x == 0) {
    double v = 0.0;
#pragma unroll
    for (int k = 0; k < kT / 64; ++k) v += s_part[k];
    if (v != 0.0) {
      const double old = atomicAdd(A.cost + (b & (kStripes - 1)), v);
      asm volatile("" ::"v"(old) : "memory");
    }
    if (D.dbg && (b == 0 || b == A.g_imu)) D.dbg[b == 0 ? 11 : 13] = wall_clock64();
    const int t = atomicAdd(D.ticket, 1);
    s_last = t == A.nblocks - 1;
    if (s_last) atomicExch(D.ticket, 0);
  }
  __syncthreads();
  if (s_last) lm_decide_body<true>(D);
  if (s_last && D.dbg && threadIdx.x == 0) D.dbg[5] = wall_clock64();
}
__global__ __launch_bounds__(kT) void k_cost_decide(CostArgs a, DecideArgs d, int end_zero) { cost_decide_body(blockIdx.x, a, d, end_zero); }
__global__ __launch_bounds__(kT) void k_cost_decide_b(const CostArgs* __restrict__ t, const DecideArgs* __restrict__ d, int end_zero) { cost_decide_body(blockIdx.x, t[blockIdx.y], d[blockIdx.y], end_zero); }
__global__ __launch_bounds__(kT) void k_cost_decide_bt(const CostArgs* __restrict__ t, const DecideArgs* __restrict__ d, int end_zero) { cost_decide_body(blockIdx.y, t[blockIdx.x], d[blockIdx.x], end_zero); }

static StateP state_ptrs(const lvf_state* st) { return StateP{st->poses.p, st->vel.p, st->ba.p, st->bg.p, st->inv_depth.p, st->w_visual.p}; }
static inline int grid(int n) { return (n + kT - 1) / kT; }

struct Chain {
  bool fast = false;
  bool batchable = false;
  bool has_imu = false, has_prior = false, imu_in_cost = false;
  ZeroList zero_end{};
  ZeroList zero{};
  ImuArgs imu_lin{}, imu_cost{};
  LinArgs lin{}; size_t lin_lds = 0;
  TfReduceArgs red{}; size_t red_lds = 0;
  PrepArgs prep{};
  bool early = false;
  PrepArgs prep_early{}; size_t prep_lds = 0;
  int first_own_level = 0;
  bool merged_level0 = false;
  SchurSp0Args ssp0{}; size_t ssp0_lds = 0;
  int n_levels = 0; SpArgs sp[kSpMaxLevels]; int sp_lds[kSpMaxLevels] = {0};
  CholArgs chol{};
  BackArgs back{}; size_t back_lds = 0;
  TailArgs tail{}; size_t tail_lds = 0;
  bool back_tail_merged = false; BackTailArgs bt{}; size_t bt_lds = 0;
  CostArgs cost{};
  DecideArgs dec{};
};

void stage_clock_free(StageClock* k);
void batch_orphan(lvf_problem_batch* b, lvf_problem* dying);
}
lvf_problem::~lvf_problem() {
  for (lvf_problem_batch* b : batches) lvf::batch_orphan(b, this);
  delete chain;
  lvf::stage_clock_free(clk);
  if (rec && !lvf::HostPinPool::get().give(rec, lvf::Pool::bucket(sizeof(lvf::LmCtl)))) (void)hipHostFree(rec);
  if (graph_exec) (void)hipGraphExecDestroy(graph_exec);
  if (ev_band) (void)hipEventDestroy(ev_band);
}
namespace lvf {

static void fill_cost_visual(const lvf_problem* p, CostVisual& a) {
  a = CostVisual{};
  if (p->tc && p->tc->n) {
    a.n_tc = p->tc->n; a.tc_lo = (const double2*)p->tc->ob_a.p; a.tc_ro = (const double2*)p->tc->ob_b.p; a.tc_lm = p->tc->idx_a.p; a.tc_kf = p->tc->idx_b.p;
    a.tc_w = p->tc->wblk.n ? p->tc->wblk.p : nullptr; a.tc_left = p->tc->cam_a; a.tc_right = p->tc->cam_b;
  }
  if (p->tf && p->tf->n) {
    a.n_tf = p->tf->n; a.tf_fo = p->tf_fo(); a.tf_ob = p->tf_ob(); a.tf_lm = p->tf_lm(); a.tf_k1 = p->tf_k1();
    a.tf_k2 = p->tf_k2(); a.tf_left = p->tf->cam_a; a.tf_right = p->tf->cam_b;
  }
  if (p->po && p->po->n) {
    a.n_po = p->po->n; a.po_ob = (const double2*)p->po->ob_a.p; a.po_kf = p->po->idx_a.p; a.po_pwi = p->po->idx_b.p; a.po_pw = p->po->table.p; a.po_cam = p->po->cam_a;
  }
  a.g_tc = grid(a.n_tc); a.g_tf = grid(a.n_tf);
}

struct StateView {
  lvf_state v;
  StateView(lvf_ctx* ctx, int n_kf, int n_lm, double* poses, double* vel, double* ba, double* bg, double* invd, double* wv) {
    v.ctx = ctx; v.n_kf = n_kf; v.n_lm = n_lm;
    v.poses.p = poses; v.vel.p = vel; v.ba.p = ba; v.bg.p = bg; v.inv_depth.p = invd; v.w_visual.p = wv;
  }
  ~StateView() { v.poses.p = v.vel.p = v.ba.p = v.bg.p = v.inv_depth.p = v.w_visual.p = nullptr; }
};

static int enqueue_cost(lvf_problem* p, const StateP& s, const lvf_state* imu_state_view, double huber, double* cost_slot) {
  hipStream_t q = p->ctx->stream;
  CostArgs c{};
  fill_cost_visual(p, c.a);
  c.n_kf = p->n_kf; c.s = s; c.huber = huber; c.cost = cost_slot; c.done = nullptr;
  c.nblocks = c.a.g_tc + c.a.g_tf + grid(c.a.n_po);
  if (c.nblocks > 0) hipLaunchKernelGGL(k_cost_visual, dim3(c.nblocks), dim3(kT), 0, q, c);
  if (p->imu && p->imu->n) {
    static_assert(kStripes == 32, "k_imu stripes its cost over 32 slots");
    LVF_TRY(launch_imu(p->imu, imu_state_view, false, cost_slot));
  }
  if (p->prior && p->prior->n) {
    LVF_TRY(launch_pose_prior(p->prior, imu_state_view, false));
    hipLaunchKernelGGL(k_cost_sq, dim3(grid(6 * p->prior->n)), dim3(kT), 0, q, 6 * p->prior->n, p->prior->res.p, cost_slot);
  }
  LVF_HIP(hipGetLastError());
  return LVF_OK;
}

static void fill_back_args(lvf_problem* p, BackArgs& ba, size_t* lds_bytes) {
  SpBack sb{};
  sb.lv = p->sp_levels; sb.rows = p->sp_rows.p; sb.owner = p->sp_owner.p; sb.W = p->sp_W.p; sb.Linv = p->sp_L.p; sb.perm = p->perm.p;
  sb.off = p->off; sb.aug = p->aug; sb.d_total = p->d;
  sb.dbg = nullptr;
  int max_count = 0;
  for (int lv = 0; lv < p->sp_levels.n; ++lv) {
    max_count = std::max(max_count, p->sp_levels.count[lv]);
    sb.item0[lv] = p->sp_item0[lv]; sb.items[lv] = p->sp_items[lv];
  }
  const int n_nodes = p->sp_levels.n ? p->sp_levels.first[p->sp_levels.n - 1] + p->sp_levels.count[p->sp_levels.n - 1] : 0;
  sb.total_items = p->sp_levels.n ? p->sp_item0[p->sp_levels.n - 1] + p->sp_items[p->sp_levels.n - 1] : 0;
  sb.n_nodes = n_nodes; sb.max_count = max_count;
  sb.nodes = p->sp_nodes.p;
  static const bool big_lds = [] {
    return hipFuncSetAttribute(reinterpret_cast<const void*>(k_chol_backsolve), hipFuncAttributeMaxDynamicSharedMemorySize, 156 * 1024) == hipSuccess &&
           hipFuncSetAttribute(reinterpret_cast<const void*>(k_chol_backsolve_b), hipFuncAttributeMaxDynamicSharedMemorySize, 156 * 1024) == hipSuccess;
  }();
  const size_t lds_cap = big_lds ? 156 * 1024 : 64 * 1024;
  size_t doubles = (size_t)p->off + (size_t)((p->ndense + 63) / 64) * 64 + (size_t)(kBParts + 1) * kNB + 9 * (size_t)max_count + kBT + (size_t)n_nodes + 2;
  sb.linv_in_lds = (doubles + 81 * (size_t)n_nodes) * sizeof(double) <= 48 * 1024 ? 1 : 0;
  if (sb.linv_in_lds) doubles += 81 * (size_t)n_nodes;
  int max_items = 0;
  for (int lv = 0; lv < p->sp_levels.n; ++lv) max_items = std::max(max_items, p->sp_items[lv]);
// ... 179 lines not shown
      next_level = ride;
      if (ride < c.n_levels) { a.sp = c.sp[ride]; c.ssp0_lds = std::max(c.ssp0_lds, (size_t)p->sp_shmem[ride]); next_level = ride + 1; }
      if (c.early && chain_n > 0) {
        int* cnt = reinterpret_cast<int*>(p->sp_sync.p);
        SpArgs* slot[2] = {&a.sp_b, &a.sp_c};
        SpArgs* prev = &a.sp;
        for (int k = 0; k < std::min(2, chain_n) && next_level < c.n_levels && (size_t)p->sp_shmem[next_level] <= 64 * 1024; ++k) {
          *slot[k] = c.sp[next_level];
          prev->src.done_counter = cnt + 2 * (next_level - 1);
          slot[k]->src.wait_counter = cnt + 2 * (next_level - 1); slot[k]->src.wait_target = prev->nblocks;
          if (p->force_handover_timeouts > 0 && k == 0) { slot[k]->src.wait_target = prev->nblocks + 1; slot[k]->src.timeout_ticks = 2000u; }
          c.ssp0_lds = std::max(c.ssp0_lds, (size_t)p->sp_shmem[next_level]);
          prev = slot[k];
          ++next_level;
        }
      }
      a.work = p->band_work.p; a.n_work = p->n_band_work;
      a.nblocks = a.n_work + a.sp.nblocks + a.sp_b.nblocks + a.sp_c.nblocks; a.done = done;
      c.merged_level0 = true;
      c.first_own_level = next_level;
    }
  }
  c.chol.Sd = p->S.p + (size_t)p->off * (p->ld + 1); c.chol.ld = p->ld; c.chol.nb = p->nb; c.chol.fail = fail; c.chol.Dinv = p->Dinv.p; c.chol.Ldiag = p->Ldiag.p; c.chol.done = done;
  c.chol.last_cols = p->ndense + 1 - kNB * (p->nb - 1);
  fill_back_args(p, c.back, &c.back_lds);
  c.back.done = done;
  {
    TailArgs& a = c.tail;
    static const int tail_cap = [] { const char* e = std::getenv("LVF_TAIL_WGS"); return e ? std::atoi(e) : 640; }();
    a.g_lm = p->n_lm ? std::min(tail_cap, (p->n_lm + kT / 16 - 1) / (kT / 16)) : 0;
    a.n_lm = p->n_lm; a.dp = p->dp; a.ldE = p->ldE; a.E = p->E.p; a.C = p->compact ? p->Ct.p : p->C.p; a.Cd = p->Cd.p;
    a.gr = p->compact ? p->grt.p : p->gr.p; a.dxc = p->dxc.p; a.dxl = p->dxl.p; a.scal = p->scal.p;
    a.kmin = p->band_ready ? p->lm_kmin.p : nullptr; a.kmax = p->lm_kmax.p; a.n_kf = p->n_kf; a.s = s; a.poses2 = p->poses2.p; a.vel2 = p->vel2.p; a.ba2 = p->ba2.p;
    a.bg2 = p->bg2.p; a.invd2 = p->invd2.p; a.d = p->d; a.ld = p->dpad; a.B = p->B.p; a.gc = p->gc.p; a.radius = radius; a.nblocks = a.g_lm + grid(p->d); a.done = done; a.pose_const = p->pose_const.p; a.jac = jac;
    c.tail_lds = (size_t)p->ldE * sizeof(double);
  }
  {
    static const unsigned bt_timeout = [] { const char* e = std::getenv("LVF_CHAIN_TIMEOUT_US"); return e ? (unsigned)std::max(1, std::atoi(e)) * 100u : 50000u; }();
    static const int bt_fenced = [] { const char* e = std::getenv("LVF_CHAIN_FENCE"); return e ? std::atoi(e) : 1; }();
    static const bool bt_big_lds = hipFuncSetAttribute(reinterpret_cast<const void*>(k_backsolve_tail), hipFuncAttributeMaxDynamicSharedMemorySize, 156 * 1024) == hipSuccess;
    c.back_tail_merged = bt_wanted && c.tail.g_lm > 0;
    if (c.back_tail_merged) {
      BackTailArgs& m = c.bt;
      m.back = c.back; m.tail = c.tail;
      m.back.pose_ready = reinterpret_cast<int*>(p->sp_sync.p) + 2 * kSpMaxLevels - 2;
      m.back.n_pose = p->dp;
      static const int bt_wgs = [] { const char* e = std::getenv("LVF_BACK_TAIL_WGS"); return e ? std::max(1, std::atoi(e)) : 224; }();
      m.g_lm = std::min(bt_wgs, (p->n_lm + kBT / 16 - 1) / (kBT / 16));
      m.fenced = bt_fenced == 2; m.back.pose_fenced = bt_fenced == 2; m.timeout_ticks = bt_timeout; m.fail = fail;
      if (p->force_handover_timeouts > 1) { m.back.pose_ready = reinterpret_cast<int*>(p->sp_sync.p) + 2 * kSpMaxLevels - 4; m.timeout_ticks = 2000u; }
      c.bt_lds = std::max(c.back_lds, c.tail_lds);
      if (c.bt_lds > 64 * 1024 && !bt_big_lds) c.back_tail_merged = false;
    }
    static const bool chain_info = std::getenv("LVF_CHAIN_INFO") != nullptr;
    if (chain_info) std::fprintf(stderr, "chain: n_kf %d n_lm %d fast %d has_imu %d early %d compact %d levels %d no_chain %d merged_level0 %d back_tail_merged %d (g_lm %d, lds %zu)\n", p->n_kf, p->n_lm, (int)c.fast, (int)c.has_imu,
                                 (int)c.early, (int)p->compact, c.n_levels, (int)p->no_chain, (int)c.merged_level0, (int)c.back_tail_merged, c.bt.g_lm, c.bt_lds);
  }
  fill_cost_visual(p, c.cost.a);
  c.cost.n_kf = p->n_kf; c.cost.s = s2; c.cost.huber = 0.0; c.cost.cost = p->scal.p + SC_COST_NEW; c.cost.done = done;
  c.cost.nblocks = c.cost.a.g_tc + c.cost.a.g_tf + grid(c.cost.a.n_po);
  {
    static const int cost_tiles = [] { const char* e = std::getenv("LVF_COST_TILES"); return e ? std::atoi(e) : 2; }();
    if (cost_tiles > 1) {
      CostArgs& k = c.cost;
      const int per = kT * cost_tiles;
      k.tiles = cost_tiles;
      k.a.g_tc = (k.a.n_tc + per - 1) / per; k.a.g_tf = (k.a.n_tf + per - 1) / per;
      k.nblocks = k.a.g_tc + k.a.g_tf + (k.a.n_po + per - 1) / per;
    }
  }
  c.cost.g_imu = 0; c.cost.imu = ImuEvalArgs{};
  c.imu_in_cost = c.fast && c.has_imu && c.cost.nblocks > 0;
  if (c.imu_in_cost) { c.cost.imu = ImuEvalArgs{p->imu->n, p->imu->pre.p, p->imu->sqrt_info.p, p->imu->idx_a.p, p->imu->idx_b.p}; c.cost.g_imu = p->imu->n; c.cost.nblocks += p->imu->n; }
  c.cost.zero = c.zero_end; c.cost.zero_wgs = c.fast ? kEndZeroWgs : 0;
  {
    DecideArgs& a = c.dec;
    a.scal = p->scal.p; a.ctl = ctl; a.rec = p->rec; a.ticket = reinterpret_cast<int*>(p->scal.p + SC_TICKET); a.n_kf = p->n_kf; a.n_lm = p->n_lm;
    a.poses = p->st->poses.p; a.vel = p->st->vel.p; a.ba = p->st->ba.p; a.bg = p->st->bg.p; a.invd = p->st->inv_depth.p;
    a.poses2 = p->poses2.p; a.vel2 = p->vel2.p; a.ba2 = p->ba2.p; a.bg2 = p->bg2.p; a.invd2 = p->invd2.p;
    static const bool lm_history = std::getenv("LVF_LM_HISTORY") != nullptr;
    a.hist = nullptr;
    if (lm_history) { LVF_TRY(p->dbg_hist.ensure(8 * 64)); a.hist = p->dbg_hist.p; }
  }
  c.batchable = c.fast && p->compact && c.has_imu && !c.has_prior && c.merged_level0 && c.lin.nblocks > 0 && c.cost.nblocks > 0;
  { const StateP sp = state_ptrs(p->st); std::memcpy(p->chain_state, &sp, sizeof(sp)); }
  p->chain_tcw = p->tc && p->tc->wblk.n ? p->tc->wblk.p : nullptr;
  p->chain_ready = true;
  return LVF_OK;
}
static bool chain_stale(const lvf_problem* p) {
  if (!p->chain_ready || !p->chain) return true;
  const StateP s = state_ptrs(p->st);
  static_assert(sizeof(StateP) == sizeof(p->chain_state), "StateP is six pointers");
  if (std::memcmp(&s, p->chain_state, sizeof(StateP)) != 0) return true;
  const double* w = p->tc && p->tc->wblk.n ? p->tc->wblk.p : nullptr;
  return w != p->chain_tcw;
}

enum { ST_IMU_LIN = 0, ST_LIN_VISUAL, ST_TF_REDUCE, ST_PREPARE, ST_SCHUR_SP0, ST_SP_LEVELS, ST_CHOL, ST_BACKSOLVE, ST_STEP_TAIL, ST_COST, ST_DECIDE, ST_N };
static const char* const kStageNames[ST_N] = {"k_zero_multi (only when the accumulators are not known clean)", "k_lin_visual", "k_tf_reduce (+ sparse level 0)", "k_prepare (+ sparse level 1)", "k_schur_sp0 (+ a sparse level)", "k_sp_eliminate (the levels left)",
                                             "k_chol_step (all block steps)", "k_chol_backsolve", "k_step_tail", "k_cost_decide (candidate cost incl. the ImuError factors; its last workgroup closes the iteration; + prior passes)", "k_lm_decide (windows without visual blocks)"};
constexpr int kClockReps = 16, kClockLaunches = 48;
struct StageClock {
  hipEvent_t ev[kClockReps][ST_N + 1]; int launches[ST_N]; bool on = false; int rep = 0;
  hipEvent_t kstart[kClockReps][kClockLaunches], kstop[kClockReps][kClockLaunches]; int kstage[kClockLaunches]; int nk = 0; bool kernel_events = false;
};
void stage_clock_free(StageClock* k) {
  if (!k) return;
  for (auto& r : k->ev) for (auto& e : r) (void)hipEventDestroy(e);
  if (k->kernel_events) { for (auto& r : k->kstart) for (auto& e : r) (void)hipEventDestroy(e); for (auto& r : k->kstop) for (auto& e : r) (void)hipEventDestroy(e); }
  delete k;
}
#define LVF_CHAIN_LAUNCH(p_, stage_, kernel_, grid_, block_, lds_, q_, ...)                                                          \
  do {                                                                                                                              \
    StageClock* k__ = (p_)->clk;                                                                                                    \
    if (k__ && k__->on && k__->kernel_events && k__->nk < kClockLaunches) {                                                         \
      const int i__ = k__->nk++;                                                                                                    \
      k__->kstage[i__] = (stage_);                                                                                                  \
      hipExtLaunchKernelGGL(kernel_, grid_, block_, lds_, q_, k__->kstart[k__->rep][i__], k__->kstop[k__->rep][i__], 0, __VA_ARGS__); \
    } else hipLaunchKernelGGL(kernel_, grid_, block_, lds_, q_, __VA_ARGS__);                                                       \
  } while (0)
static inline void stage_mark(lvf_problem* p, int stage_done, int launches) {
  StageClock* k = p->clk;
  if (!k || !k->on) return;
  (void)hipEventRecord(k->ev[k->rep][stage_done + 1], p->ctx->stream);
  k->launches[stage_done] = launches;
}

static int enqueue_linearize(lvf_problem* p, double huber, bool gated, bool iteration = false) {
  hipStream_t q = p->ctx->stream;
  if (chain_stale(p)) LVF_TRY(build_chain(p));
  const Chain& c = *p->chain;
  const StateP s = state_ptrs(p->st);
  double* cost = p->scal.p + SC_COST;
  bool imu_done = false;
  const bool clean = c.fast && p->accum_clean;
  p->accum_clean = false;
  if (p->clk && p->clk->on) (void)hipEventRecord(p->clk->ev[p->clk->rep][0], q);
  if (!clean) LVF_CHAIN_LAUNCH(p, ST_IMU_LIN, k_zero_multi, dim3(512, c.zero.count), dim3(kT), 0, q, c.zero);
  if (c.fast) {
    imu_done = true;
    stage_mark(p, ST_IMU_LIN, clean ? 0 : 1);
    LinArgs la = c.lin;
    la.huber = huber;
    if (!gated) la.done = nullptr;
    if (!iteration) la.scal_reset = nullptr;
    static const bool lin_timing = std::getenv("LVF_LIN_TIMING") != nullptr;
    if (lin_timing) { LVF_TRY(p->dbg_lin.ensure((size_t)la.v.n_tfw * 24 + 8)); la.dbg = p->dbg_lin.p; }
    static const size_t lds_pad = [] { const char* e = std::getenv("LVF_LIN_LDS_PAD"); return e ? (size_t)std::atoi(e) : (size_t)0; }();
    LVF_CHAIN_LAUNCH(p, ST_LIN_VISUAL, k_lin_visual, dim3(la.nblocks), dim3(kT), c.lin_lds + lds_pad, q, la);
    stage_mark(p, ST_LIN_VISUAL, 1);
    if (p->compact) {
      TfReduceArgs ra = c.red;
      if (!gated) ra.done = nullptr;
      if (!iteration) { ra.nblocks = ra.own_blocks; ra.ride.nblocks = 0; }
      LVF_CHAIN_LAUNCH(p, ST_TF_REDUCE, k_tf_reduce, dim3(ra.nblocks), dim3(kT), ra.ride.nblocks > 0 ? c.red_lds : 0, q, ra);
    }
    stage_mark(p, ST_TF_REDUCE, p->compact ? 1 : 0);
    if (lin_timing) {
      std::vector<unsigned long long> t((size_t)la.v.n_tfw * 8);
      LVF_HIP(hipStreamSynchronize(q));
      LVF_HIP(hipMemcpy(t.data(), p->dbg_lin.p, t.size() * 8, hipMemcpyDeviceToHost));
      double ph[5] = {0, 0, 0, 0, 0}; unsigned long long first = ~0ull, last = 0, last_start = 0;
      for (int w = 0; w < la.v.n_tfw; ++w) {
        for (int k = 0; k < 5; ++k) ph[k] += (double)(t[(size_t)w * 8 + k + 1] - t[(size_t)w * 8 + k]) * 0.01;
        first = std::min(first, t[(size_t)w * 8]); last = std::max(last, t[(size_t)w * 8 + 5]); last_start = std::max(last_start, t[(size_t)w * 8]);
      }
      {
        double mx[5] = {0, 0, 0, 0, 0}; int slow = 0; double slow_t = 0;
        for (int w = 0; w < la.v.n_tfw; ++w) {
          for (int k = 0; k < 5; ++k) mx[k] = std::max(mx[k], (double)(t[(size_t)w * 8 + k + 1] - t[(size_t)w * 8 + k]) * 0.01);
          const double tot = (double)(t[(size_t)w * 8 + 5] - t[(size_t)w * 8]) * 0.01;
          if (tot > slow_t) { slow_t = tot; slow = w; }
        }
        std::vector<TfWork> hw((size_t)la.v.n_tfw);
        LVF_HIP(hipMemcpy(hw.data(), la.v.work, hw.size() * sizeof(TfWork), hipMemcpyDeviceToHost));
        std::fprintf(stderr, "lin_tf: per-phase MAX over the workgroups (us): %.2f | %.2f | %.2f | %.2f | %.2f ; slowest workgroup %d (k2 = %d, %d blocks): %.2f us =", mx[0], mx[1], mx[2], mx[3], mx[4], slow, hw[slow].k2, hw[slow].count, slow_t);
        for (int k = 0; k < 5; ++k) std::fprintf(stderr, " %.2f", (double)(t[(size_t)slow * 8 + k + 1] - t[(size_t)slow * 8 + k]) * 0.01);
        {
          unsigned long long u[16];
          LVF_HIP(hipMemcpy(u, p->dbg_lin.p + (size_t)la.v.n_tfw * 8 + 8 + (size_t)slow * 16, sizeof(u), hipMemcpyDeviceToHost));
          std::fprintf(stderr, " ; its waves (eval us, k1-sum us, groups):");
          for (int wv = 0; wv < 4; ++wv) std::fprintf(stderr, " [%.2f %.2f %llu]", (double)(u[4 * wv + 1] - u[4 * wv]) * 0.01, (double)(u[4 * wv + 2] - u[4 * wv + 1]) * 0.01, u[4 * wv + 3]);
        }
        std::fprintf(stderr, " ; mean duration by k2 decile:");
        const int nk = la.n_kf;
        for (int dcl = 0; dcl < 5; ++dcl) {
          double sum = 0; int cnt = 0;
          for (int w = 0; w < la.v.n_tfw; ++w) if (hw[w].k2 * 5 / std::max(nk, 1) == dcl) { sum += (double)(t[(size_t)w * 8 + 5] - t[(size_t)w * 8]) * 0.01; ++cnt; }
          std::fprintf(stderr, " %.1f(%d)", cnt ? sum / cnt : 0.0, cnt);
        }
        std::fprintf(stderr, "\n");
      }
      std::fprintf(stderr, "lin_tf: the TwoFrame workgroups START within %.2f us of each other; starts of workgroups 0, 1/4, 1/2, 3/4, last (us after the first): %.2f %.2f %.2f %.2f %.2f\n", (double)(last_start - first) * 0.01,
                   (double)(t[0] - first) * 0.01, (double)(t[(size_t)(la.v.n_tfw / 4) * 8] - first) * 0.01, (double)(t[(size_t)(la.v.n_tfw / 2) * 8] - first) * 0.01,
                   (double)(t[(size_t)(3 * la.v.n_tfw / 4) * 8] - first) * 0.01, (double)(t[(size_t)(la.v.n_tfw - 1) * 8] - first) * 0.01);
      std::fprintf(stderr, "lin_tf phases (us, mean over %d workgroups): stage %.2f | eval+landmark atomics %.2f | k1 sums %.2f | k2 sums %.2f | flush %.2f ; first start -> last end %.2f\n",
                   la.v.n_tfw, ph[0] / la.v.n_tfw, ph[1] / la.v.n_tfw, ph[2] / la.v.n_tfw, ph[3] / la.v.n_tfw, ph[4] / la.v.n_tfw, (double)(last - first) * 0.01);
      if (la.v.imu.pre) {
        unsigned long long u[5];
        LVF_HIP(hipMemcpy(u, p->dbg_lin.p + (size_t)la.v.n_tfw * 8, sizeof(u), hipMemcpyDeviceToHost));
        std::fprintf(stderr, "lin_imu phases of factor 0 (us): stage %.2f | raw residual + pre-weighting Jacobian (one lane) %.2f | weight + to tangent %.2f | J^T J, J^T r %.2f ; start %.2f after the first TwoFrame workgroup, end %.2f before the last one's end\n",
                     (double)(u[1] - u[0]) * 0.01, (double)(u[2] - u[1]) * 0.01, (double)(u[3] - u[2]) * 0.01, (double)(u[4] - u[3]) * 0.01, ((double)u[0] - (double)first) * 0.01, ((double)last - (double)u[4]) * 0.01);
      }
    }
  } else {
    if (p->tc && p->tc->n)
      hipLaunchKernelGGL(k_lin_tc<false>, dim3(grid(p->tc->n)), dim3(kT), 0, q, p->tc->n, (const double2*)p->tc->ob_a.p, (const double2*)p->tc->ob_b.p,
                         p->tc->idx_a.p, p->tc->idx_b.p, p->tc->wblk.n ? p->tc->wblk.p : (const double*)nullptr, s, p->tc->cam_a, p->tc->cam_b, huber, p->C.p, p->gr.p, cost);
    if (p->tf && p->tf->n)
      hipLaunchKernelGGL(k_lin_tf<false>, dim3(grid(p->tf->n)), dim3(kT), 0, q, p->tf->n, p->n_kf, (const double2*)p->tf->ob_a.p, (const double2*)p->tf->ob_b.p,
                         p->tf->idx_a.p, p->tf->idx_b.p, p->tf->idx_c.p, s, p->tf->cam_a, p->tf->cam_b, huber, p->pose_const.p, p->B.p, p->dpad,
                         p->gc.p, p->E.p, p->ldE, p->C.p, p->gr.p, cost);
    if (p->po && p->po->n)
      hipLaunchKernelGGL(k_lin_po<false>, dim3(grid(p->po->n)), dim3(kT), 0, q, p->po->n, p->n_kf, (const double2*)p->po->ob_a.p, p->po->idx_a.p,
                         p->po->idx_b.p, p->po->table.p, s, p->po->cam_a, huber, p->pose_const.p, p->B.p, p->dpad, p->gc.p, cost);
  }
  if (c.has_imu && !imu_done) {
    LVF_TRY(launch_imu(p->imu, p->st, true));
    ImuJ J;
    for (int k = 0; k < 8; ++k) J.j[k] = p->imu->jac[k].p;
    hipLaunchKernelGGL(k_lin_imu, dim3(p->imu->n), dim3(64), 0, q, p->imu->n, p->n_kf, p->imu->res.p, J, p->imu->idx_a.p, p->imu->idx_b.p,
                       p->st->poses.p, p->pose_const.p, p->B.p, p->dpad, p->gc.p, cost);
  }
  if (c.has_prior) {
    const lvf_batch* pb = p->prior;
    const PriorArgs P{pb->n, pb->idx_a.p, pb->idx_b.p, pb->table.p, pb->ob_a.p, pb->ob_b.p};
    hipLaunchKernelGGL(k_prior_lin, dim3((pb->n + 63) / 64), dim3(64), 0, q, P, p->st->poses.p, p->pose_const.p, p->B.p, p->dpad, p->gc.p, cost);
  }
  LVF_HIP(hipGetLastError());
  p->linearized = true;
  return LVF_OK;
}

static int await_band_work(lvf_problem* p) {
  if (!p->band_pending) return LVF_OK;
  LVF_HIP(hipEventSynchronize(p->ev_band));
  p->band_pending = false;
  p->n_band_work = p->h_n_band_work[0];
  if (p->chain && p->chain->merged_level0) {
    SchurSp0Args& a = p->chain->ssp0;
    a.n_work = p->n_band_work;
    a.nblocks = a.n_work + a.sp.nblocks + a.sp_b.nblocks + a.sp_c.nblocks;
  }
  return LVF_OK;
}

static int enqueue_reduced_system(lvf_problem* p, const double* radius_dev, bool reset_scalars, bool gated, bool* level0_done) {
  hipStream_t q = p->ctx->stream;
  const Chain& c = *p->chain;
  const bool early = c.early && level0_done != nullptr;
  PrepArgs pa = early ? c.prep_early : c.prep;
  pa.radius = radius_dev;
  if (!reset_scalars) pa.scal = nullptr;
  if (!gated) pa.done = nullptr;
  static const bool poison = std::getenv("LVF_POISON_S") != nullptr;
  if (poison) LVF_HIP(hipMemsetAsync(p->S.p, 0xff, (size_t)p->ld * p->ld * 8, q));
  LVF_CHAIN_LAUNCH(p, ST_PREPARE, k_prepare, dim3(pa.nblocks), dim3(kT), pa.ride.nblocks > 0 ? c.prep_lds : 0, q, pa);
  stage_mark(p, ST_PREPARE, 1);
  if (!early && c.early) p->accum_clean = false;
  if (level0_done) *level0_done = false;
  if (p->n_lm) {
    LVF_TRY(await_band_work(p));
    if (c.merged_level0) {
      SchurSp0Args sa = c.ssp0;
      if (!gated) sa.done = nullptr;
      if (!level0_done) { sa.nblocks = sa.n_work; sa.sp.nblocks = 0; sa.sp_b.nblocks = 0; sa.sp_c.nblocks = 0; }
      static const bool schur_timing = std::getenv("LVF_SCHUR_TIMING") != nullptr;
      const int ns = sa.n_work;
      if (schur_timing) { LVF_TRY(p->dbg_lin.ensure((size_t)ns * 8 + 8)); LVF_HIP(hipMemsetAsync(p->dbg_lin.p, 0, (size_t)ns * 64, q)); sa.dbg = p->dbg_lin.p; }
      if (sa.nblocks > 0) LVF_CHAIN_LAUNCH(p, ST_SCHUR_SP0, k_schur_sp0, dim3(sa.nblocks), dim3(256), c.ssp0_lds, q, sa);
      stage_mark(p, ST_SCHUR_SP0, 1);
      if (schur_timing) {
        std::vector<unsigned long long> t((size_t)ns * 8);
        LVF_HIP(hipStreamSynchronize(q));
        LVF_HIP(hipMemcpy(t.data(), p->dbg_lin.p, t.size() * 8, hipMemcpyDeviceToHost));
        double ph[3] = {0, 0, 0}; int cnt = 0; unsigned long long first = ~0ull, last = 0;
        for (int w = 0; w < ns; ++w) {
          if (!t[(size_t)w * 8 + 3]) continue;
          ++cnt;
          for (int k = 0; k < 3; ++k) ph[k] += (double)(t[(size_t)w * 8 + k + 1] - t[(size_t)w * 8 + k]) * 0.01;
          first = std::min(first, t[(size_t)w * 8]); last = std::max(last, t[(size_t)w * 8 + 3]);
        }
        std::fprintf(stderr, "schur band phases (us, mean over %d of %d workgroups): setup + first fetch issue %.2f | chunks (stage + mfma) %.2f | output atomics %.2f ; first start -> last end %.2f\n",
                     cnt, ns, ph[0] / std::max(cnt, 1), ph[1] / std::max(cnt, 1), ph[2] / std::max(cnt, 1), (double)(last - first) * 0.01);
      }
      if (level0_done) *level0_done = true;
    } else {
      double* S_pose = p->S.p + (size_t)p->off_pose * (p->ld + 1);
      const LmBand band{p->band_ready ? p->lm_order.p : nullptr, p->lm_nactive.p, p->lm_kmin.p, p->lm_kmax.p};
      LVF_TRY(launch_schur(q, p->n_lm, p->dp, p->ldE, p->E.p, p->Cd.p, p->dp, p->ld, S_pose, band));
    }
  }
  LVF_HIP(hipGetLastError());
  return LVF_OK;
}

static int enqueue_iteration(lvf_problem* p, bool end_zero) {
  hipStream_t q = p->ctx->stream;
  if (chain_stale(p)) LVF_TRY(build_chain(p));
  const Chain& c = *p->chain;
  static const bool sp_timing = std::getenv("LVF_SP_TIMING") != nullptr;
  if (sp_timing && c.early) {
    const int n_nodes = p->sp_levels.n ? p->sp_levels.first[p->sp_levels.n - 1] + p->sp_levels.count[p->sp_levels.n - 1] : 0;
    if (p->dbg_sp.n == 0) {
      LVF_TRY(p->dbg_sp.ensure((size_t)n_nodes * 8 + 8)); p->dbg_sp.n = (size_t)n_nodes * 8;
      LVF_HIP(hipMemsetAsync(p->dbg_sp.p, 0, (size_t)n_nodes * 64, q));
      Chain& cw = *p->chain;
      for (int lv = 0; lv < cw.n_levels; ++lv) cw.sp[lv].src.dbg = p->dbg_sp.p;
      cw.red.ride.src.dbg = p->dbg_sp.p; cw.prep_early.ride.src.dbg = p->dbg_sp.p; cw.ssp0.sp.src.dbg = p->dbg_sp.p; cw.ssp0.sp_b.src.dbg = p->dbg_sp.p; cw.ssp0.sp_c.src.dbg = p->dbg_sp.p;
    } else {
      std::vector<unsigned long long> t((size_t)n_nodes * 8);
      LVF_HIP(hipStreamSynchronize(q));
      LVF_HIP(hipMemcpy(t.data(), p->dbg_sp.p, t.size() * 8, hipMemcpyDeviceToHost));
      for (int lv = 0; lv < p->sp_levels.n; ++lv) {
        const int f0 = p->sp_levels.first[lv], cnt = p->sp_levels.count[lv];
        double ph[7] = {0, 0, 0, 0, 0, 0, 0}; unsigned long long first = ~0ull, last = 0;
        for (int k = f0; k < f0 + cnt; ++k) {
          for (int j = 0; j < 7; ++j) ph[j] += (double)(t[(size_t)k * 8 + j + 1] - t[(size_t)k * 8 + j]) * 0.01 / cnt;
          first = std::min(first, t[(size_t)k * 8]); last = std::max(last, t[(size_t)k * 8 + 7]);
        }
        std::fprintf(stderr, "sparse level %d (%d blocks, us): requests by address %.2f | wait for the level below %.2f | S entries %.2f | factor %.2f | W + first adds (returning) %.2f | arrive %.2f | rest of the adds %.2f ; start %.2f after level 0's first start, span %.2f\n",
                     lv, cnt, ph[0], ph[1], ph[2], ph[3], ph[4], ph[5], ph[6], (double)(first - t[0]) * 0.01, (double)(last - first) * 0.01);
      }
    }
  }
  LVF_TRY(enqueue_linearize(p, p->huber, true, true));
  bool level0_done = false;
  LVF_TRY(enqueue_reduced_system(p, &p->ctl.p->radius, true, true, &level0_done));
  const int own0 = level0_done ? c.first_own_level : 0;
  for (int lv = own0; lv < c.n_levels; ++lv)
    LVF_CHAIN_LAUNCH(p, ST_SP_LEVELS, k_sp_eliminate, dim3(c.sp[lv].nblocks), dim3(256), c.sp_lds[lv], q, c.sp[lv]);
  stage_mark(p, ST_SP_LEVELS, std::max(0, c.n_levels - own0));
  for (int kb = 0; kb < p->nb; ++kb) {
    CholArgs cha = c.chol;
    static const bool chol_timing = std::getenv("LVF_CHOL_TIMING") != nullptr;
    if (chol_timing) { LVF_TRY(p->dbg.ensure(64)); cha.dbg = p->dbg.p; }
    LVF_CHAIN_LAUNCH(p, ST_CHOL, k_chol_step, dim3(chol_step_grid(p->nb, kb)), dim3(kCT), 0, q, cha, kb);
  }
  {
    BackArgs ba = c.back;
    static const bool back_timing = std::getenv("LVF_BACK_TIMING") != nullptr;
    if (back_timing) { LVF_TRY(p->dbg.ensure(64)); ba.sp.dbg = p->dbg.p; }
    stage_mark(p, ST_CHOL, p->nb);
    if (c.back_tail_merged) {
      BackTailArgs bt = c.bt;
      if (back_timing) bt.back.sp.dbg = p->dbg.p;
      LVF_CHAIN_LAUNCH(p, ST_BACKSOLVE, k_backsolve_tail, dim3(2 + c.bt.g_lm), dim3(kBT), c.bt_lds, q, bt);
      stage_mark(p, ST_BACKSOLVE, 1);
      stage_mark(p, ST_STEP_TAIL, 0);
    } else {
      LVF_CHAIN_LAUNCH(p, ST_BACKSOLVE, k_chol_backsolve, dim3(1), dim3(kBT), c.back_lds, q, ba);
      stage_mark(p, ST_BACKSOLVE, 1);
      LVF_CHAIN_LAUNCH(p, ST_STEP_TAIL, k_step_tail, dim3(c.tail.nblocks), dim3(kT), c.tail_lds, q, c.tail);
      stage_mark(p, ST_STEP_TAIL, 1);
    }
  }
  CostArgs ca = c.cost;
  ca.huber = p->huber;
  if (c.has_imu && !c.imu_in_cost) LVF_TRY(launch_imu_args(q, c.imu_cost, false));
  if (c.has_prior) {
    const lvf_batch* pb = p->prior;
    const PriorArgs P{pb->n, pb->idx_a.p, pb->idx_b.p, pb->table.p, pb->ob_a.p, pb->ob_b.p};
    hipLaunchKernelGGL(k_prior_cost, dim3((pb->n + 63) / 64), dim3(64), 0, q, P, p->poses2.p, p->scal.p + SC_COST_NEW);
  }
  if (ca.nblocks > 0) {
    if (!end_zero) ca.zero_wgs = 0;
    DecideArgs da = c.dec;
    static const bool cost_timing = std::getenv("LVF_COST_TIMING") != nullptr;
    if (cost_timing) { LVF_TRY(p->dbg.ensure(64)); da.dbg = p->dbg.p; }
    LVF_CHAIN_LAUNCH(p, ST_COST, k_cost_decide, dim3(ca.nblocks + ca.zero_wgs), dim3(kT), 0, q, ca, da, end_zero ? 1 : 0);
    p->accum_clean = ca.zero_wgs > 0;
    if (p->accum_clean) p->linearized = false;
    stage_mark(p, ST_COST, 1 + (c.has_imu && !c.imu_in_cost ? 1 : 0) + (c.has_prior ? 1 : 0));
  } else {
    stage_mark(p, ST_COST, (c.has_imu ? 1 : 0) + (c.has_prior ? 1 : 0));
    LVF_CHAIN_LAUNCH(p, ST_DECIDE, k_lm_decide, dim3(1), dim3(kDT), 0, q, c.dec);
    stage_mark(p, ST_DECIDE, 1);
  }
  LVF_HIP(hipGetLastError());
  return LVF_OK;
}

static void ctl_from_options(const lvf_solver_options* o, double radius, double decrease, int max_iters, bool with_tolerances, LmCtl* c) {
  std::memset(c, 0, sizeof(*c));
  c->radius = radius; c->decrease = decrease; c->last_radius = radius;
  c->huber = o->huber_a; c->min_rel_decrease = o->min_relative_decrease;
  c->function_tol = with_tolerances ? o->function_tolerance : -1.0;
  c->gradient_tol = with_tolerances ? o->gradient_tolerance : -1.0;
  c->parameter_tol = with_tolerances ? o->parameter_tolerance : -1.0;
  c->max_iters = max_iters;
  c->termination = 1; c->why = LVF_WHY_MAX_ITERATIONS;
}
static int upload_ctl(lvf_problem* p, const LmCtl& c) {
  if (chain_stale(p)) LVF_TRY(build_chain(p));
  *p->rec = c;
  LVF_TRY(p->h_ctl.reserve(1));
  p->h_ctl[0] = c;
  LVF_HIP(hipMemcpyAsync(p->ctl.p, p->h_ctl.p, sizeof(LmCtl), hipMemcpyHostToDevice, p->ctx->stream));
  return LVF_OK;
}
static int download_ctl(lvf_problem* p, LmCtl* out) {
  hipStream_t q = p->ctx->stream;
  LVF_TRY(p->h_ctl.reserve(2));
  LVF_HIP(hipMemcpyAsync(&p->h_ctl[1], p->ctl.p, sizeof(LmCtl), hipMemcpyDeviceToHost, q));
  LVF_HIP(hipStreamSynchronize(q));
  *out = p->h_ctl[1];
  return LVF_OK;
}

static bool handover_pending(const lvf_problem* p, const LmCtl& c) { return c.done && c.why == LVF_WHY_HANDOVER && !p->no_chain; }
static int rearm_after_handover(lvf_problem* p, LmCtl* c) {
  p->no_chain = true; p->unchained_solves = 0; p->chain_ready = false; p->handover_retries += 1;
  if (p->force_handover_timeouts > 0) p->force_handover_timeouts -= 1;
  c->done = 0; c->termination = 1; c->why = LVF_WHY_MAX_ITERATIONS;
  p->accum_clean = false;
  return upload_ctl(p, *c);
}

struct IterOut { double cost_before, cost_after, model, dxnorm, xnorm, gmax; bool accepted, solved; };

static int lm_iteration(lvf_problem* p, const lvf_solver_options* o, double* radius, double* decrease, IterOut* out) {
  LmCtl c;
  ctl_from_options(o, *radius, *decrease, 1, false, &c);
  p->huber = o->huber_a;
  LVF_TRY(upload_ctl(p, c));
  LVF_TRY(enqueue_iteration(p, false));
  LVF_TRY(download_ctl(p, &c));
  if (handover_pending(p, c)) {
    LVF_TRY(rearm_after_handover(p, &c));
    LVF_TRY(enqueue_iteration(p, false));
    LVF_TRY(download_ctl(p, &c));
  }
  if (p->dbg.p && std::getenv("LVF_CHOL_TIMING")) {
    unsigned long long t[64];
    LVF_HIP(hipMemcpy(t, p->dbg.p, sizeof(t), hipMemcpyDeviceToHost));
    for (int kb = 0; kb < p->nb && kb < 8; ++kb) {
      const unsigned long long* u = t + 8 * kb;
      if (kb == 0) std::fprintf(stderr, "chol step 0 (us): loads %.2f | factor %.2f (%llu shader clocks) | store %.2f\n", (double)(u[3] - u[0]) * 0.01, (double)(u[4] - u[3]) * 0.01, u[7] - u[6], (double)(u[5] - u[4]) * 0.01);
      else if (kb + 2 < p->nb + 1) std::fprintf(stderr, "chol step %d (us): stage %.2f | mfma %.2f | relayout %.2f | factor %.2f | store %.2f ; since previous step's end %.2f\n", kb, (double)(u[1] - u[0]) * 0.01,
                        (double)(u[2] - u[1]) * 0.01, (double)(u[3] - u[2]) * 0.01, (double)(u[4] - u[3]) * 0.01, (double)(u[5] - u[4]) * 0.01, (double)(u[0] - u[-3]) * 0.01);
    }
  }
  if (p->dbg.p && std::getenv("LVF_COST_TIMING")) {
    unsigned long long t[64];
    LVF_HIP(hipMemcpy(t, p->dbg.p, sizeof(t), hipMemcpyDeviceToHost));
    auto us = [&](int a, int b) { return ((double)t[b] - (double)t[a]) * 0.01; };
    std::fprintf(stderr, "cost+decide (us): imu wg0 stage %.2f | raw (one lane) %.2f | weight+sum %.2f ; first visual wg %.2f (starts %.2f after imu wg0) ; decision starts %.2f after imu wg0's start: sums %.2f | logic %.2f | commit %.2f | record %.2f\n",
                 us(8, 9), us(9, 10), us(10, 11), us(12, 13), us(8, 12), us(8, 1), us(1, 2), us(2, 3), us(3, 4), us(4, 5));
  }
  if (p->dbg.p && std::getenv("LVF_BACK_TIMING")) {
    unsigned long long t[64];
    LVF_HIP(hipMemcpy(t, p->dbg.p, sizeof(t), hipMemcpyDeviceToHost));
    std::fprintf(stderr, "backsolve phases (us):");
    for (unsigned long long k = 1; k < t[63] && k < 55; ++k) std::fprintf(stderr, " %.2f", (double)(t[k] - t[k - 1]) * 0.01);
    if (p->chain && p->chain->back_tail_merged)
      std::fprintf(stderr, " | merged launch, us after workgroup 0's start: step applied %.2f ; first landmark workgroup starts %.2f, sees the poses %.2f, done %.2f ; last one starts %.2f, sees %.2f, done %.2f",
                   (double)(t[55] - t[0]) * 0.01, (double)(t[56] - t[0]) * 0.01, (double)(t[57] - t[0]) * 0.01, (double)(t[58] - t[0]) * 0.01, (double)(t[59] - t[0]) * 0.01,
                   (double)(t[60] - t[0]) * 0.01, (double)(t[61] - t[0]) * 0.01);
    std::fprintf(stderr, "\n");
  }
  out->cost_before = c.cost_before; out->cost_after = c.cost_after; out->model = c.model; out->dxnorm = c.dxnorm; out->xnorm = c.xnorm; out->gmax = c.gmax;
  out->solved = c.solved != 0; out->accepted = c.accepted != 0;
  p->last_radius = c.last_radius;
  *radius = c.radius; *decrease = c.decrease;
  return LVF_OK;
}

static int wait_for_iteration(lvf_problem* p, int iter) {
  const volatile LmCtl* r = p->rec;
  const auto t0 = std::chrono::steady_clock::now();
  while (r->iter < iter && !r->done) {
    if (std::chrono::duration<double>(std::chrono::steady_clock::now() - t0).count() > 0.05) {
      LmCtl c;
      LVF_TRY(download_ctl(p, &c));
      *p->rec = c;
      break;
    }
#if defined(__x86_64__)
    __builtin_ia32_pause();
#endif
  }
  return LVF_OK;
}

static int build_elimination_plan(lvf_problem* p) {
  const int n = p->n_kf;
  std::vector<int32_t> key;
  key.push_back(n);
  const lvf_batch* imu = p->imu;
  const bool have_idx = imu && imu->n > 0 && (int)imu->host_kf1.size() == imu->n && (int)imu->host_kf2.size() == imu->n;
  if (imu && imu->n > 0) {
    key.push_back(have_idx ? 1 : 0);
    if (have_idx) { key.insert(key.end(), imu->host_kf1.begin(), imu->host_kf1.end()); key.insert(key.end(), imu->host_kf2.begin(), imu->host_kf2.end()); }
  }
  if (key == p->plan_key && p->ld > 0) return LVF_OK;
  static const bool sparse_on = [] { const char* e = std::getenv("LVF_SPARSE_VB"); return !(e && e[0] == '0'); }();
  std::vector<std::vector<char>> va(n, std::vector<char>(n, 0)), pa(n, std::vector<char>(n, 0));
// ... 478 lines not shown
    if (b) {
      LVF_REQUIRE(b->ctx == ctx, "batch belongs to another context");
      LVF_REQUIRE(b->min_n_kf <= st->n_kf && b->min_n_lm <= st->n_lm, "batch indices exceed the state (n_kf=%d n_lm=%d)", st->n_kf, st->n_lm);
    }
  LVF_REQUIRE(st->n_kf > 0, "lvf_problem_create: empty window");
  LVF_TRY(lvf::enter(ctx));
  auto* p = new lvf_problem();
  p->ctx = ctx; p->st = st; p->tc = two_camera; p->tf = two_frame; p->po = pose_only; p->imu = imu;
  const int rc = problem_configure(p);
  if (rc != LVF_OK) { delete p; return rc; }
  *out = p;
  return LVF_OK;
}
int lvf_problem_destroy(lvf_problem* p) { delete p; return LVF_OK; }

int lvf_problem_set_pose_priors(lvf_problem* p, lvf_batch* pose_priors) {
  LVF_REQUIRE(p, "lvf_problem_set_pose_priors: null problem");
  if (pose_priors) {
    LVF_REQUIRE(pose_priors->kind == LVF_K_POSE_PRIOR, "pose_priors batch has the wrong kind");
    LVF_REQUIRE(pose_priors->ctx == p->ctx, "batch belongs to another context");
    LVF_REQUIRE(pose_priors->min_n_kf <= p->n_kf, "pose-prior batch references keyframe %d but the window has %d", pose_priors->min_n_kf - 1, p->n_kf);
  }
  p->prior = pose_priors;
  p->linearized = false;
  p->chain_ready = false;
  return LVF_OK;
}

int lvf_problem_set_vbb_constant(lvf_problem* p, int kf, int v_constant, int ba_constant, int bg_constant) {
  LVF_REQUIRE(p, "null problem");
  LVF_REQUIRE(kf >= 0 && kf < p->n_kf, "keyframe %d out of range", kf);
  p->pose_const_h[kf] = (uint8_t)((p->pose_const_h[kf] & 1) | (v_constant ? 2 : 0) | (ba_constant ? 4 : 0) | (bg_constant ? 8 : 0));
  LVF_HIP(hipMemcpyAsync(p->pose_const.p, p->pose_const_h.data(), p->n_kf, hipMemcpyHostToDevice, p->ctx->stream));
  LVF_HIP(hipStreamSynchronize(p->ctx->stream));
  return LVF_OK;
}

int lvf_problem_set_pose_constant(lvf_problem* p, int kf, int is_constant) {
  LVF_REQUIRE(p, "null problem");
  LVF_REQUIRE(kf >= 0 && kf < p->n_kf, "keyframe %d out of range", kf);
  p->pose_const_h[kf] = (uint8_t)((p->pose_const_h[kf] & ~1) | (is_constant ? 1 : 0));
  LVF_HIP(hipMemcpyAsync(p->pose_const.p, p->pose_const_h.data(), p->n_kf, hipMemcpyHostToDevice, p->ctx->stream));
  LVF_HIP(hipStreamSynchronize(p->ctx->stream));
  return LVF_OK;
}

int lvf_problem_cost(lvf_problem* p, const lvf_solver_options* o, double* cost) {
  LVF_REQUIRE(p && o && cost, "lvf_problem_cost: null argument");
  LVF_TRY(lvf::enter(p->ctx));
  hipStream_t q = p->ctx->stream;
  LVF_HIP(hipMemsetAsync(p->scal.p, 0, SC_N * 8, q));
  LVF_TRY(enqueue_cost(p, state_ptrs(p->st), p->st, o->huber_a, p->scal.p + SC_COST));
  double hc[kStripes];
  LVF_HIP(hipMemcpyAsync(hc, p->scal.p + SC_COST, sizeof(hc), hipMemcpyDeviceToHost, q));
  LVF_HIP(hipMemsetAsync(p->scal.p + SC_COST, 0, kStripes * 8, q));
  LVF_HIP(hipStreamSynchronize(q));
  *cost = stripe_sum(hc, 0);
  return LVF_OK;
}

int lvf_problem_stage_count(void) { return ST_N; }
const char* lvf_problem_stage_name(int stage) { return stage >= 0 && stage < ST_N ? kStageNames[stage] : ""; }

int lvf_problem_stage_times2(lvf_problem* p, const lvf_solver_options* o, double radius, int reps, double* us, double* spans_us, int* launches) {
  LVF_REQUIRE(p && o && us && reps > 0, "lvf_problem_stage_times: bad argument");
  LVF_TRY(lvf::enter(p->ctx));
  hipStream_t q = p->ctx->stream;
  if (!p->clk) {
    p->clk = new StageClock();
    for (auto& r : p->clk->ev) for (auto& e : r) LVF_HIP(hipEventCreate(&e));
    for (auto& r : p->clk->kstart) for (auto& e : r) LVF_HIP(hipEventCreate(&e));
    for (auto& r : p->clk->kstop) for (auto& e : r) LVF_HIP(hipEventCreate(&e));
    p->clk->kernel_events = true;
  }
  StageClock& k = *p->clk;
  for (int i = 0; i < ST_N; ++i) { us[i] = 0.0; k.launches[i] = 0; }
  std::vector<double> span(ST_N, 0.0), kern(ST_N, 0.0);
  std::vector<int> kcount(ST_N, 0);
  reps = std::min(reps, kClockReps);
  LmCtl c;
  ctl_from_options(o, radius, 2.0, reps + 2, false, &c);
  p->huber = o->huber_a;
  LVF_TRY(upload_ctl(p, c));
  LVF_TRY(enqueue_iteration(p, true));
  int nk = 0;
  for (int r = 0; r < reps; ++r) {
    k.on = true; k.rep = r; k.nk = 0;
    const int rc = enqueue_iteration(p, true);
    k.on = false;
    nk = k.nk;
    LVF_TRY(rc);
  }
  LVF_HIP(hipStreamSynchronize(q));
  for (int r = 0; r < reps; ++r) {
    for (int i = 0; i < ST_N; ++i) {
      if (k.launches[i] == 0) continue;
      int prev = i;
      while (prev > 0 && k.launches[prev - 1] == 0) --prev;
      float ms = 0.f;
      LVF_HIP(hipEventElapsedTime(&ms, k.ev[r][prev], k.ev[r][i + 1]));
      span[i] += 1e3 * (double)ms / reps;
    }
    for (int j = 0; j < nk; ++j) {
      float ms = 0.f;
      LVF_HIP(hipEventElapsedTime(&ms, k.kstart[r][j], k.kstop[r][j]));
      kern[k.kstage[j]] += 1e3 * (double)ms / reps;
      if (r == 0) kcount[k.kstage[j]] += 1;
    }
  }
  for (int i = 0; i < ST_N; ++i) us[i] = (k.launches[i] > 0 && kcount[i] == k.launches[i]) ? kern[i] : span[i];
  if (spans_us) for (int i = 0; i < ST_N; ++i) spans_us[i] = span[i];
  if (launches) for (int i = 0; i < ST_N; ++i) launches[i] = k.launches[i];
  return LVF_OK;
}
int lvf_problem_stage_times(lvf_problem* p, const lvf_solver_options* o, double radius, int reps, double* us, int* launches) {
  return lvf_problem_stage_times2(p, o, radius, reps, us, nullptr, launches);
}

int lvf_problem_gradient(lvf_problem* p, const lvf_solver_options* o, double* gc, double* gl) {
  LVF_REQUIRE(p && o && gc, "lvf_problem_gradient: null argument");
  LVF_TRY(lvf::enter(p->ctx));
  hipStream_t q = p->ctx->stream;
  LVF_TRY(enqueue_linearize(p, o->huber_a, false));
  const double* gr = p->gr.p;
  if (gl && p->n_lm && p->compact) {
    LmCtl c;
    ctl_from_options(o, o->initial_trust_region_radius, 2.0, 1, false, &c);
    LVF_TRY(upload_ctl(p, c));
    PrepArgs pa = p->chain->prep;
    pa.radius = &p->ctl.p->radius; pa.scal = nullptr; pa.done = nullptr;
    hipLaunchKernelGGL(k_prepare, dim3(pa.nblocks), dim3(kT), 0, q, pa);
    LVF_HIP(hipGetLastError());
    gr = p->grt.p;
  }
  LVF_HIP(hipMemcpyAsync(gc, p->gc.p, (size_t)p->d * 8, hipMemcpyDeviceToHost, q));
  if (gl && p->n_lm) LVF_HIP(hipMemcpyAsync(gl, gr, (size_t)p->n_lm * 8, hipMemcpyDeviceToHost, q));
  LVF_HIP(hipStreamSynchronize(q));
  return LVF_OK;
}

int lvf_problem_lm_iteration(lvf_problem* p, const lvf_solver_options* o, double* radius, double* decrease_factor,
                             double* cost_before, double* cost_after, int* accepted) {
  LVF_REQUIRE(p && o && radius && decrease_factor, "lvf_problem_lm_iteration: null argument");
  LVF_REQUIRE(*radius > 0.0 && *decrease_factor > 0.0, "radius and decrease_factor must be positive");
  LVF_TRY(lvf::enter(p->ctx));
  IterOut it;
  LVF_TRY(lm_iteration(p, o, radius, decrease_factor, &it));
  if (cost_before) *cost_before = it.cost_before;
  if (cost_after) *cost_after = it.cost_after;
  if (accepted) *accepted = it.accepted ? 1 : 0;
  return LVF_OK;
}

static void summary_from_ctl(const lvf_problem* p, const LmCtl& c, lvf_solver_summary* s) {
  std::memset(s, 0, sizeof(*s));
  s->num_residual_blocks = (p->tc ? p->tc->n : 0) + (p->tf ? p->tf->n : 0) + (p->po ? p->po->n : 0) + (p->imu ? p->imu->n : 0) + (p->prior ? p->prior->n : 0);
  s->initial_cost = c.initial_cost; s->final_cost = c.cost; s->num_iterations = c.iter; s->num_successful_steps = c.successes; s->termination = c.termination;
  s->num_unsuccessful_steps = c.rejected; s->termination_reason = c.why; s->hand_over_retries = p->handover_retries;
}


int lvf_problem_solve(lvf_problem* p, const lvf_solver_options* o, lvf_solver_summary* summary) { return lvf_problem_solve_then(p, o, summary, nullptr, nullptr); }

int lvf_problem_solve_then(lvf_problem* p, const lvf_solver_options* o, lvf_solver_summary* summary, int (*tail)(void*), void* user) {
  LVF_REQUIRE(p && o && summary, "lvf_problem_solve: null argument");
  LVF_TRY(lvf::enter(p->ctx));
  LmCtl c;
  ctl_from_options(o, o->initial_trust_region_radius, 2.0, o->max_num_iterations, true, &c);
  p->huber = o->huber_a;
  if (o->max_num_iterations <= 0) {
    double cost = 0.0;
    LVF_TRY(lvf_problem_cost(p, o, &cost));
    c.initial_cost = c.cost = cost;
    summary_from_ctl(p, c, summary);
    if (tail) LVF_TRY(tail(user));
    return LVF_OK;
  }
  constexpr int kUnchainedSolves = 32;
  if (p->no_chain && ++p->unchained_solves > kUnchainedSolves && p->force_handover_timeouts == 0) { p->no_chain = false; p->unchained_solves = 0; p->chain_ready = false; }
  LVF_TRY(upload_ctl(p, c));
  const auto wall0 = std::chrono::steady_clock::now();
  bool timed_out = false;
  for (int first = 0;;) {
    for (int it = first; it < o->max_num_iterations; ++it) {
      LVF_TRY(enqueue_iteration(p, true));
      if (it >= first + 1) LVF_TRY(wait_for_iteration(p, it));
      if (p->rec->done) break;
      if (o->max_solver_time_in_seconds > 0.0 &&
          std::chrono::duration<double>(std::chrono::steady_clock::now() - wall0).count() >= o->max_solver_time_in_seconds) { timed_out = true; break; }
    }
    const bool known_handover = p->rec->done && p->rec->why == LVF_WHY_HANDOVER && !p->no_chain;
    if (tail && !known_handover) LVF_TRY(tail(user));
    LVF_TRY(download_ctl(p, &c));
    if (!handover_pending(p, c)) break;
    LVF_TRY(rearm_after_handover(p, &c));
    first = c.iter;
  }
  p->last_radius = c.last_radius;
  summary_from_ctl(p, c, summary);
  if (timed_out && !c.done) summary->termination_reason = LVF_WHY_TIME;
  return LVF_OK;
}

int lvf_problem_reduced_dim(lvf_problem* p) { return p ? p->d : -1; }

int lvf_problem_download_reduced(lvf_problem* p, double* S, double* rhs) {
  LVF_REQUIRE(p && S && rhs, "lvf_problem_download_reduced: null argument");
  if (!p->linearized || !p->chain_ready) { set_error("no linearisation yet"); return LVF_ERR_STATE; }
  LVF_TRY(lvf::enter(p->ctx));
  hipStream_t q = p->ctx->stream;
  const size_t nS = (size_t)p->ld * p->ld;
  LVF_TRY(enqueue_reduced_system(p, &p->ctl.p->last_radius, false, false, nullptr));
  std::vector<double> h(nS);
  LVF_HIP(hipMemcpyAsync(h.data(), p->S.p, nS * 8, hipMemcpyDeviceToHost, q));
  LVF_HIP(hipStreamSynchronize(q));
  const int d = p->d, ld = p->ld;
  const std::vector<int>& pm = p->perm_h;
  for (int i = 0; i < d; ++i)
    for (int j = 0; j <= i; ++j) {
      const double v = h[(size_t)std::max(pm[i], pm[j]) * ld + std::min(pm[i], pm[j])];
      S[(size_t)i * d + j] = v; S[(size_t)j * d + i] = v;
    }
  for (int j = 0; j < d; ++j) rhs[j] = h[(size_t)p->aug * ld + pm[j]];
  return LVF_OK;
}

int lvf_problem_batch_create(lvf_ctx* ctx, lvf_problem* const* problems, int n, lvf_problem_batch** out) {
  LVF_REQUIRE(ctx && out && n >= 1 && problems, "lvf_problem_batch_create: bad arguments");
  for (int i = 0; i < n; ++i) {
    LVF_REQUIRE(problems[i], "lvf_problem_batch_create: problem %d is null", i);
    LVF_REQUIRE(problems[i]->ctx == ctx, "lvf_problem_batch_create: problem %d belongs to another context", i);
    for (int j = 0; j < i; ++j) LVF_REQUIRE(problems[j] != problems[i] && problems[j]->st != problems[i]->st, "lvf_problem_batch_create: windows %d and %d share state", j, i);
  }
  auto* b = new lvf_problem_batch();
  b->ctx = ctx; b->W = n; b->probs.assign(problems, problems + n);
  for (lvf_problem* p : b->probs) p->batches.push_back(b);
  *out = b;
  return LVF_OK;
}
int lvf_problem_batch_destroy(lvf_problem_batch* b) {
  if (b && !b->orphaned)
    for (lvf_problem* p : b->probs) p->batches.erase(std::remove(p->batches.begin(), p->batches.end(), b), p->batches.end());
  delete b;
  return LVF_OK;
}
int lvf_problem_batch_size(const lvf_problem_batch* b) { return b ? b->W : -1; }
int lvf_problem_debug_history(lvf_problem* p, double* out512) {
  LVF_REQUIRE(p && out512, "lvf_problem_debug_history: null argument");
  if (!p->dbg_hist.p) { set_error("lvf_problem_debug_history: LVF_LM_HISTORY is not set"); return LVF_ERR_STATE; }
  LVF_TRY(lvf::enter(p->ctx));
  LVF_HIP(hipMemcpyAsync(out512, p->dbg_hist.p, 512 * 8, hipMemcpyDeviceToHost, p->ctx->stream));
  LVF_HIP(hipStreamSynchronize(p->ctx->stream));
  return LVF_OK;
}
int lvf_problem_debug_force_handover_timeout(lvf_problem* p, int n) {
  LVF_REQUIRE(p && n >= 0, "lvf_problem_debug_force_handover_timeout: bad argument");
  p->force_handover_timeouts = n; p->no_chain = false; p->chain_ready = false;
  return LVF_OK;
}
int lvf_problem_batch_uses_tables(lvf_problem_batch* b, const lvf_solver_options* o) {
  if (!b || !o || lvf::enter(b->ctx) != LVF_OK || batch_build_tables(b, o->huber_a) != LVF_OK) return -1;
  return b->tables ? 1 : 0;
}

int lvf_problem_batch_lm_iteration(lvf_problem_batch* b, const lvf_solver_options* o, double* radius, double* decrease_factor, double* cost_before,
                                   double* cost_after, int* accepted) {
  LVF_REQUIRE(b && o && radius && decrease_factor, "lvf_problem_batch_lm_iteration: null argument");
  LVF_TRY(lvf::enter(b->ctx));
  LVF_TRY(batch_build_tables(b, o->huber_a));
  for (int w = 0; w < b->W; ++w) {
    LVF_REQUIRE(radius[w] > 0.0 && decrease_factor[w] > 0.0, "radius and decrease_factor must be positive");
    LmCtl c;
// ... 73 lines not shown
```

Measured before the change: 4927 iter/s.

## Double-buffer accumulators and fuse next-iteration linearize with cost/decision stage

```diff
diff --git a/lvio_fusion_amd/csrc/solver_kernels.hip b/lvio_fusion_amd/csrc/solver_kernels.hip
--- a/lvio_fusion_amd/csrc/solver_kernels.hip
+++ b/lvio_fusion_amd/csrc/solver_kernels.hip
@@ -29,11 +29,13 @@
   GP<unsigned long long> dbg;
   int s_zero;
   JacobiDev jac{nullptr, nullptr};
+  GP<const int> sel{nullptr}; GP<const double> B1{nullptr}, gc1{nullptr};
 };
 struct SpArgs {
   GP<const SpNode> nodes; int first, tiles; GP<const int> rows; GP<double> S; int ld; GP<double> W; int wstride; GP<double> Lout; GP<int> fail; int nblocks; GP<const int> done;
   SpSrc src;
 };
+template <bool SEL = false>
 __device__ __forceinline__ void sp_ride(const int vb, const SpArgs& a);
 constexpr int kFailSparse = 100000, kFailHandover = 300000;
 }
@@ -71,6 +73,7 @@
   lvf::DevBuf<double> Ldiag;
   std::vector<int> perm_h;
   lvf::DevBuf<double> B, gc, C, gr, E, Cd, S, dxc, dxl, scal;
+  lvf::DevBuf<double> B1, gc1, C1, gr1, E1, slotB1;
   lvf::DevBuf<double> jh0;
   lvf::DevBuf<double> poses2, vel2, ba2, bg2, invd2;
   lvf::DevBuf<uint8_t> pose_const;
@@ -79,6 +82,7 @@
   lvf::HostPin<lvf::TfWork> h_tf_work;
   std::vector<uint8_t> pose_const_h;
   bool linearized = false;
+  bool acc1_ready = false;
   lvf::DevBuf<double2> tfs_fo, tfs_ob;
   lvf::DevBuf<int> tfs_lm, tfs_k1, tfs_k2, tfs_perm;
   lvf::HostPin<int> h_tfs_perm;
@@ -124,6 +128,10 @@
 
 struct StateP { GP<const double> poses, vel, ba, bg, inv_depth, w_kf; };
 
+struct AccSel { GP<const int> sel; GP<double> B, gc, C, gr, E, slotB; };
+__device__ __forceinline__ int acc_set(const AccSel& a) { return a.sel ? *a.sel : 0; }
+template <bool SEL> __device__ __forceinline__ int acc_set_t(const AccSel& a) { return SEL ? acc_set(a) : 0; }
+
 struct LmCtl {
   double radius, decrease;
   double last_radius;
@@ -136,6 +144,8 @@
   int done, termination;
   int why, rejected;
   int jfrozen;
+  int aset;
+  int lin_pending;
 };
 
 __device__ __forceinline__ void add_block66(double* __restrict__ B, int ld, int ra, int rb, const double Ja[12], const double Jb[12]) {
@@ -769,23 +779,28 @@
       else if (lane < 21) g = 6 * kj + (lane - 15); else g = 6 * n_kf + 9 * kj + (lane - 21);
       sidx[lane] = g;
     }
-    for (int e = lane; e < 30; e += 64) {
-      const int row = e % 15, which = e / 15;
-      const double* Jr = (which ? J.j[4] : J.j[0]) + (size_t)f * 105 + 7 * row;
-      const int kk = which ? kj : ki;
-      const double* q = poses + 7 * kk;
-      const double sc = (pose_const[kk] & 1) ? 0.0 : 1.0;
-      double l3[3];
-      quat_row_to_local(Jr, q, l3);
-      double* o = sJ + row * 30 + (which ? 15 : 0);
-      o[0] = sc * l3[0]; o[1] = sc * l3[1]; o[2] = sc * l3[2]; o[3] = sc * Jr[4]; o[4] = sc * Jr[5]; o[5] = sc * Jr[6];
-    }
-    for (int e = lane; e < 15 * 18; e += 64) {
-      const int row = e / 18, c = e % 18, blk = c / 3, cc = c % 3;
-      const int src = blk < 3 ? 1 + blk : 5 + (blk - 3);
-      const double* jp = src == 1 ? J.j[1] : (src == 2 ? J.j[2] : (src == 3 ? J.j[3] : (src == 5 ? J.j[5] : (src == 6 ? J.j[6] : J.j[7]))));
+#pragma unroll
+    for (int which = 0; which < 2; ++which) {
+      if (lane < 15) {
+        const int row = lane;
+        const double* Jr = J.j[which ? 4 : 0] + (size_t)f * 105 + 7 * row;
+        const int kk = which ? kj : ki;
+        const double* q = poses + 7 * kk;
+        const double sc = (pose_const[kk] & 1) ? 0.0 : 1.0;
+        double l3[3];
+        quat_row_to_local(Jr, q, l3);
+        double* o = sJ + row * 30 + (which ? 15 : 0);
+        o[0] = sc * l3[0]; o[1] = sc * l3[1]; o[2] = sc * l3[2]; o[3] = sc * Jr[4]; o[4] = sc * Jr[5]; o[5] = sc * Jr[6];
+      }
+    }
+#pragma unroll
+    for (int blk = 0; blk < 6; ++blk) {
+      const double* jp = J.j[blk < 3 ? 1 + blk : 2 + blk];
       const double scv = ((pose_const[blk < 3 ? ki : kj] >> (1 + blk % 3)) & 1) ? 0.0 : 1.0;
-      sJ[row * 30 + (blk < 3 ? 6 + 3 * blk : 21 + 3 * (blk - 3)) + cc] = scv * jp[(size_t)f * 45 + 3 * row + cc];
+      if (lane < 45) {
+        const int row = lane / 3, cc = lane % 3;
+        sJ[row * 30 + (blk < 3 ? 6 + 3 * blk : 21 + 3 * (blk - 3)) + cc] = scv * jp[(size_t)f * 45 + 3 * row + cc];
+      }
     }
   }
   __syncthreads();
@@ -907,24 +922,27 @@
   LinVisual v; int n_kf; StateP s; double huber; GP<const uint8_t> pose_const; GP<double> B; int ld; GP<double> gc; GP<double> E; int ldE; GP<double> C, gr, cost;
   int nblocks; GP<const int> done; GP<unsigned long long> dbg; int rows;
   GP<double> scal_reset;
+  AccSel acc;
 };
 __device__ __forceinline__ void reset_step_scalars(double* scal) {
   for (int k = SC_COST_NEW + threadIdx.x; k < SC_N; k += kT) scal[k] = 0.0;
   if (threadIdx.x == 0) { *reinterpret_cast<int*>(scal + SC_FAIL) = 0; *reinterpret_cast<int*>(scal + SC_TICKET) = 0; }
 }
-__device__ __forceinline__ void lin_visual_body(const int bx, const LinArgs& A) {
-  if (bx >= A.nblocks || (A.done && *A.done)) return;
-  if (bx == 0 && A.scal_reset) reset_step_scalars(A.scal_reset);
+__device__ __forceinline__ void lin_visual_run(const int bx, const LinArgs& A, const int set, const StateP s, double* cost) {
   const LinVisual& a = A.v;
   const int g_imu_first = a.imu.pre ? a.n_imu : 0;
   const int b = bx - g_imu_first;
-  const int n_kf = A.n_kf; const StateP s = A.s; const double huber = A.huber; const uint8_t* pose_const = A.pose_const;
-  double* B = A.B; const int ld = A.ld; double* gc = A.gc; double* E = A.E; const int ldE = A.ldE; double* C = A.C; double* gr = A.gr; double* cost = A.cost;
+  const int n_kf = A.n_kf; const double huber = A.huber; const uint8_t* pose_const = A.pose_const;
+  auto pick = [set](GP<double> p0, GP<double> p1) -> double* { return (double*)(p0.p + (p1.p - p0.p) * (ptrdiff_t)set); };
+  double* B = pick(A.B, A.acc.B); const int ld = A.ld; double* gc = pick(A.gc, A.acc.gc); double* E = pick(A.E, A.acc.E); const int ldE = A.ldE;
+  double* C = pick(A.C, A.acc.C); double* gr = pick(A.gr, A.acc.gr);
+  TfCompact cp = a.cp;
+  cp.slotB = pick(a.cp.slotB, A.acc.slotB);
   if (bx < g_imu_first)
     lin_imu_eval_body(bx, a.imu, n_kf, s, pose_const, B, ld, gc, cost, A.dbg ? A.dbg + (size_t)a.n_tfw * 8 : nullptr);
   else if (b < a.n_tfw)
     lin_tf_sorted_body<true>(b, a.work, n_kf, a.tf_fo, a.tf_ob, a.tf_lm, a.tf_k1, s, a.tf_left, a.tf_right, huber, pose_const, B, ld, gc, E, ldE, C, gr, cost,
-                       a.unique_lk2, A.dbg, a.cp, a.n_tfw);
+                       a.unique_lk2, A.dbg, cp, a.n_tfw);
   else if (b < a.n_tfw + a.g_tc)
     lin_tc_body<false>(b - a.n_tfw, a.n_tc, a.tc_lo, a.tc_ro, a.tc_lm, a.tc_kf, a.tc_w, s, a.tc_left, a.tc_right, huber, C, gr, cost);
   else if (b < a.n_tfw + a.g_tc + a.g_po)
@@ -932,6 +950,11 @@
   else
     lin_imu_body4<true>(b - a.n_tfw - a.g_tc - a.g_po, a.n_imu, n_kf, a.imu_res, a.imu_J, a.imu_i, a.imu_j, s.poses, pose_const, B, ld, gc, cost);
 }
+__device__ __forceinline__ void lin_visual_body(const int bx, const LinArgs& A) {
+  if (bx >= A.nblocks || (A.done && *A.done)) return;
+  if (bx == 0 && A.scal_reset) reset_step_scalars(A.scal_reset);
+  lin_visual_run(bx, A, 0, A.s, A.cost);
+}
 __global__ __launch_bounds__(kT) __attribute__((amdgpu_waves_per_eu(3))) void k_lin_visual(LinArgs a) { lin_visual_body(blockIdx.x, a); }
 __global__ __launch_bounds__(kT) __attribute__((amdgpu_waves_per_eu(3))) void k_lin_visual_b(const LinArgs* __restrict__ t) { lin_visual_body(blockIdx.x, t[blockIdx.y]); }
 __global__ __launch_bounds__(kT) __attribute__((amdgpu_waves_per_eu(3))) void k_lin_visual_bt(const LinArgs* __restrict__ t) { lin_visual_body(blockIdx.y, t[blockIdx.x]); }
@@ -939,10 +962,24 @@
 struct TfReduceArgs {
   int n_kf, n_wg; GP<const int> run_first; GP<const double> slabP, slabQ; GP<double> B; int ld; GP<double> gc; int nblocks; GP<const int> done;
   int own_blocks; SpArgs ride;
+  AccSel acc; GP<const int> pending; ZeroList stand0, stand1; int zero_wgs;
 };
+template <bool SEL>
 __device__ __forceinline__ void tf_reduce_body(const int bx0, const TfReduceArgs& A) {
-  if (bx0 >= A.nblocks || (A.done && *A.done)) return;
-  if (bx0 < A.ride.nblocks) { sp_ride(bx0, A.ride); return; }
+  if (bx0 >= A.nblocks) {
+    const int zw = (int)bx0 - A.nblocks;
+    if (SEL && zw < A.zero_wgs) {
+      if (acc_set(A.acc)) zero_list_share(A.stand0, zw, A.zero_wgs);
+      else zero_list_share(A.stand1, zw, A.zero_wgs);
+    }
+    return;
+  }
+  if (A.done && *A.done) return;
+  if (bx0 < A.ride.nblocks) { sp_ride<SEL>(bx0, A.ride); return; }
+  if (SEL && A.pending && !*A.pending) return;
+  const bool s1 = acc_set_t<SEL>(A.acc) != 0;
+  double* const Bs = s1 ? (double*)A.acc.B : (double*)A.B;
+  double* const gcs = s1 ? (double*)A.acc.gc : (double*)A.gc;
   const int bx = bx0 - A.ride.nblocks;
   const int n_kf = A.n_kf;
   const int nchunk = (A.n_wg + 63) / 64;
@@ -975,8 +1012,8 @@
         if (threadIdx.x < 21) {
           int x = 0, rem = threadIdx.x;
           while (rem > x) { rem -= x + 1; ++x; }
-          atomicAdd(&A.B[(size_t)(6 * k + x) * A.ld + 6 * k + rem], t);
-        } else atomicAdd(&A.gc[6 * k + threadIdx.x - 21], t);
+          atomicAdd(&Bs[(size_t)(6 * k + x) * A.ld + 6 * k + rem], t);
+        } else atomicAdd(&gcs[6 * k + threadIdx.x - 21], t);
       }
     }
     return;
@@ -1003,12 +1040,12 @@
   }
   if (acc != 0.0) {
     const int x = el / 6, y = el - 6 * x;
-    A.B[(size_t)(6 * k2 + x) * A.ld + 6 * k1 + y] += acc;
-  }
-}
-__global__ __launch_bounds__(kT) void k_tf_reduce(TfReduceArgs a) { tf_reduce_body(blockIdx.x, a); }
-__global__ __launch_bounds__(kT) void k_tf_reduce_b(const TfReduceArgs* __restrict__ t) { tf_reduce_body(blockIdx.x, t[blockIdx.y]); }
-__global__ __launch_bounds__(kT) void k_tf_reduce_bt(const TfReduceArgs* __restrict__ t) { tf_reduce_body(blockIdx.y, t[blockIdx.x]); }
+    Bs[(size_t)(6 * k2 + x) * A.ld + 6 * k1 + y] += acc;
+  }
+}
+__global__ __launch_bounds__(kT) void k_tf_reduce(TfReduceArgs a) { tf_reduce_body<true>(blockIdx.x, a); }
+__global__ __launch_bounds__(kT) void k_tf_reduce_b(const TfReduceArgs* __restrict__ t) { tf_reduce_body<false>(blockIdx.x, t[blockIdx.y]); }
+__global__ __launch_bounds__(kT) void k_tf_reduce_bt(const TfReduceArgs* __restrict__ t) { tf_reduce_body<false>(blockIdx.y, t[blockIdx.x]); }
 
 
 __device__ __forceinline__ void lin_prior_block(const int i, const int a, const int b, const double* __restrict__ res, const double* __restrict__ ja,
@@ -1115,25 +1152,31 @@
   int early, off;
   int own_blocks; SpArgs ride;
   JacobiDev jac;
+  AccSel acc;
 };
+template <bool SEL>
 __device__ __forceinline__ void prepare_body(const unsigned bx0, const PrepArgs& A) {
   if (bx0 >= (unsigned)A.nblocks || (A.done && *A.done)) return;
-  if (bx0 < (unsigned)A.ride.nblocks) { sp_ride((int)bx0, A.ride); return; }
+  if (bx0 < (unsigned)A.ride.nblocks) { sp_ride<SEL>((int)bx0, A.ride); return; }
   const unsigned bx = bx0 - (unsigned)A.ride.nblocks;
-  const int ld = A.ld, dpad = A.dpad; const int* __restrict__ iperm = A.iperm; const double* __restrict__ B = A.B; const double* __restrict__ gc = A.gc;
+  const bool s1 = acc_set_t<SEL>(A.acc) != 0;
+  const int ld = A.ld, dpad = A.dpad; const int* __restrict__ iperm = A.iperm; const double* __restrict__ B = s1 ? (const double*)A.acc.B : (const double*)A.B;
+  const double* __restrict__ gc = s1 ? (const double*)A.acc.gc : (const double*)A.gc;
   const double inv_radius = 1.0 / *A.radius;
   const int jf = *A.jac.frozen;
   double* __restrict__ S = A.S; const unsigned nS_blocks = A.nS_blocks; const int n_lm = A.n_lm, dp = A.dp, ldE = A.ldE;
-  const double* __restrict__ C = A.C; const double* __restrict__ gr = A.gr; double* __restrict__ Cd = A.Cd; double* __restrict__ E = A.E; double* __restrict__ scal = A.scal;
+  const double* __restrict__ C = s1 ? (const double*)A.acc.C : (const double*)A.C; const double* __restrict__ gr = s1 ? (const double*)A.acc.gr : (const double*)A.gr;
+  double* __restrict__ Cd = A.Cd; double* __restrict__ E = s1 ? (double*)A.acc.E : (double*)A.E; double* __restrict__ scal = A.scal;
+  const double* const slotB = (s1 && A.slotB) ? (const double*)A.acc.slotB : (const double*)A.slotB;
   if (bx == 0 && scal) reset_step_scalars(scal);
   if (bx >= nS_blocks) {
-    if (A.slotB) {
+    if (slotB) {
       const int l = ((bx - nS_blocks) * kT + threadIdx.x) >> 3, j0 = threadIdx.x & 7;
       const bool live = l < n_lm;
       const int lc = live ? l : 0;
       const int k1 = A.kmin[lc], len = live ? max(0, A.kmax[lc] - k1) : 0;
       const double h0l = A.jac.h0[A.jl0 + lc];
-      const double2* sb = reinterpret_cast<const double2*>(A.slotB + (size_t)A.eoff[lc] * 8);
+      const double2* sb = reinterpret_cast<const double2*>(slotB + (size_t)A.eoff[lc] * 8);
       double v[8] = {0, 0, 0, 0, 0, 0, 0, 0};
       for (int j = j0; j < len; j += 8) {
         const double2 b0 = sb[4 * j], b1 = sb[4 * j + 1], b2 = sb[4 * j + 2], cg = sb[4 * j + 3];
@@ -1186,9 +1229,9 @@
   if (!A.early) S[(size_t)I * ld + J] = v;
   else if (v != 0.0) atomicAdd(&S[(size_t)I * ld + J], v);
 }
-__global__ __launch_bounds__(kT) void k_prepare(PrepArgs a) { prepare_body(blockIdx.x, a); }
-__global__ __launch_bounds__(kT) void k_prepare_b(const PrepArgs* __restrict__ t) { prepare_body(blockIdx.x, t[blockIdx.y]); }
-__global__ __launch_bounds__(kT) void k_prepare_bt(const PrepArgs* __restrict__ t) { const PrepArgs a = t[blockIdx.x]; prepare_body(blockIdx.y, a); }
+__global__ __launch_bounds__(kT) void k_prepare(PrepArgs a) { prepare_body<true>(blockIdx.x, a); }
+__global__ __launch_bounds__(kT) void k_prepare_b(const PrepArgs* __restrict__ t) { prepare_body<false>(blockIdx.x, t[blockIdx.y]); }
+__global__ __launch_bounds__(kT) void k_prepare_bt(const PrepArgs* __restrict__ t) { const PrepArgs a = t[blockIdx.x]; prepare_body<false>(blockIdx.y, a); }
 
 constexpr int kSchurChunk = 512;
 __global__ __launch_bounds__(64) void k_schur_syrk(int n_lm, int dp, int ldE, int ntile, const double* __restrict__ E,
@@ -2087,43 +2130,50 @@
   }
 }
 
+template <bool SEL>
 __device__ __forceinline__ void sp_ride(const int vb, const SpArgs& a) {
   if (vb >= a.nblocks) return;
-  sp_eliminate_body(vb, a.nodes, a.first, a.tiles, a.rows, a.S, a.ld, a.W, a.wstride, a.Lout, a.fail, a.done, a.src);
-}
-__global__ __launch_bounds__(256) void k_sp_eliminate(SpArgs a) { sp_ride(blockIdx.x, a); }
-__global__ __launch_bounds__(256) void k_sp_eliminate_b(const SpArgs* __restrict__ t) { sp_ride(blockIdx.x, t[blockIdx.y]); }
+  if (!SEL) { sp_eliminate_body(vb, a.nodes, a.first, a.tiles, a.rows, a.S, a.ld, a.W, a.wstride, a.Lout, a.fail, a.done, a.src); return; }
+  SpSrc src = a.src;
+  if (src.sel && *src.sel) { src.B = src.B1; src.gc = src.gc1; }
+  sp_eliminate_body(vb, a.nodes, a.first, a.tiles, a.rows, a.S, a.ld, a.W, a.wstride, a.Lout, a.fail, a.done, src);
+}
+__global__ __launch_bounds__(256) void k_sp_eliminate(SpArgs a) { sp_ride<true>(blockIdx.x, a); }
+__global__ __launch_bounds__(256) void k_sp_eliminate_b(const SpArgs* __restrict__ t) { sp_ride<false>(blockIdx.x, t[blockIdx.y]); }
 struct SchurSp0Args {
   int n_slices, n_groups, dp, ldE; GP<const double> E, Cd; GP<const int> order, n_active, kmin, kmax; int d_local, ldS; GP<double> S_pose;
   SpArgs sp;
   SpArgs sp_b, sp_c;
   int nblocks; GP<const int> done; GP<unsigned long long> dbg; int rows;
   GP<const int4> work; int n_work;
+  AccSel acc;
 };
+template <bool SEL>
 __device__ __forceinline__ void schur_sp0_body(const int b, const SchurSp0Args& A) {
   if (b >= A.nblocks) return;
   if (A.work) {
     const int n_a = A.sp.nblocks, n_b = A.sp_b.nblocks, n_c = A.sp_c.nblocks, n_sp = n_a + n_b + n_c;
-    if (b < n_a) sp_ride(b, A.sp);
-    else if (b < n_a + n_b) sp_ride(b - n_a, A.sp_b);
-    else if (b < n_sp) sp_ride(b - n_a - n_b, A.sp_c);
+    if (b < n_a) sp_ride<SEL>(b, A.sp);
+    else if (b < n_a + n_b) sp_ride<SEL>(b - n_a, A.sp_b);
+    else if (b < n_sp) sp_ride<SEL>(b - n_a - n_b, A.sp_c);
     else {
       const int dv = done_flag_issue(A.done);
+      const int set = acc_set_t<SEL>(A.acc);
       const int4* item = A.work + (b - n_sp);
       const int4 it = *item;
       if (dv) return;
-      schur_band_body(it.x, it.y, A.dp, A.ldE, A.E, A.Cd, A.order, A.n_active, A.kmin, A.kmax, A.d_local, A.ldS, A.S_pose, A.dbg ? A.dbg + (size_t)(b - n_sp) * 8 : nullptr, A.rows, item);
+      schur_band_body(it.x, it.y, A.dp, A.ldE, set ? (const double*)A.acc.E : (const double*)A.E, A.Cd, A.order, A.n_active, A.kmin, A.kmax, A.d_local, A.ldS, A.S_pose, A.dbg ? A.dbg + (size_t)(b - n_sp) * 8 : nullptr, A.rows, item);
     }
     return;
   }
   if (A.done && *A.done) return;
   const int ns = A.n_slices * A.n_groups;
-  if (b < ns) schur_band_body(b % A.n_slices, b / A.n_slices, A.dp, A.ldE, A.E, A.Cd, A.order, A.n_active, A.kmin, A.kmax, A.d_local, A.ldS, A.S_pose, A.dbg ? A.dbg + (size_t)b * 8 : nullptr, A.rows);
-  else sp_ride(b - ns, A.sp);
-}
-__global__ __launch_bounds__(256) __attribute__((amdgpu_waves_per_eu(2))) void k_schur_sp0(SchurSp0Args a) { schur_sp0_body(blockIdx.x, a); }
-__global__ __launch_bounds__(256) __attribute__((amdgpu_waves_per_eu(2))) void k_schur_sp0_b(const SchurSp0Args* __restrict__ t) { schur_sp0_body(blockIdx.x, t[blockIdx.y]); }
-__global__ __launch_bounds__(256) __attribute__((amdgpu_waves_per_eu(2))) void k_schur_sp0_bt(const SchurSp0Args* __restrict__ t) { schur_sp0_body(blockIdx.y, t[blockIdx.x]); }
+  if (b < ns) schur_band_body(b % A.n_slices, b / A.n_slices, A.dp, A.ldE, acc_set_t<SEL>(A.acc) ? (const double*)A.acc.E : (const double*)A.E, A.Cd, A.order, A.n_active, A.kmin, A.kmax, A.d_local, A.ldS, A.S_pose, A.dbg ? A.dbg + (size_t)b * 8 : nullptr, A.rows);
+  else sp_ride<SEL>(b - ns, A.sp);
+}
+__global__ __launch_bounds__(256) __attribute__((amdgpu_waves_per_eu(2))) void k_schur_sp0(SchurSp0Args a) { schur_sp0_body<true>(blockIdx.x, a); }
+__global__ __launch_bounds__(256) __attribute__((amdgpu_waves_per_eu(2))) void k_schur_sp0_b(const SchurSp0Args* __restrict__ t) { schur_sp0_body<false>(blockIdx.x, t[blockIdx.y]); }
+__global__ __launch_bounds__(256) __attribute__((amdgpu_waves_per_eu(2))) void k_schur_sp0_bt(const SchurSp0Args* __restrict__ t) { schur_sp0_body<false>(blockIdx.y, t[blockIdx.x]); }
 struct SpBack {
   SpLevels lv;
   int item0[kSpMaxLevels], items[kSpMaxLevels];
@@ -2419,15 +2469,20 @@
   int g_lm, n_lm, dp, ldE; GP<const double> E, C, Cd, gr, dxc; GP<double> dxl, scal; GP<const int> kmin, kmax; int n_kf; StateP s;
   GP<double> poses2, vel2, ba2, bg2, invd2; int d, ld; GP<const double> B, gc; GP<const double> radius; int nblocks; GP<const int> done;
   GP<const unsigned char> pose_const; JacobiDev jac;
+  AccSel acc;
 };
+template <bool SEL = true> __device__ __forceinline__ const double* tail_E(const TailArgs& A) { return acc_set_t<SEL>(A.acc) ? (const double*)A.acc.E : (const double*)A.E; }
+template <bool SEL = true> __device__ __forceinline__ const double* tail_B(const TailArgs& A) { return acc_set_t<SEL>(A.acc) ? (const double*)A.acc.B : (const double*)A.B; }
+template <bool SEL = true> __device__ __forceinline__ const double* tail_gc(const TailArgs& A) { return acc_set_t<SEL>(A.acc) ? (const double*)A.acc.gc : (const double*)A.gc; }
+template <bool SEL>
 __device__ __forceinline__ void step_tail_body(const int bx, const TailArgs& A) {
   if (bx >= A.nblocks || (A.done && *A.done)) return;
-  if (bx < A.g_lm) landmark_back_body(bx, A.g_lm, A.n_lm, A.dp, A.ldE, A.E, A.C, A.Cd, A.gr, A.dxc, A.s.inv_depth, A.dxl, A.invd2, A.scal, A.kmin, A.kmax);
-  else apply_step_body(bx - A.g_lm, A.n_kf, 0, A.s, A.dxc, A.dxl, A.poses2, A.vel2, A.ba2, A.bg2, A.invd2, A.scal, A.d, A.ld, A.B, A.gc, 1.0 / *A.radius, A.pose_const, A.jac);
-}
-__global__ __launch_bounds__(kT) void k_step_tail(TailArgs a) { step_tail_body(blockIdx.x, a); }
-__global__ __launch_bounds__(kT) void k_step_tail_b(const TailArgs* __restrict__ t) { step_tail_body(blockIdx.x, t[blockIdx.y]); }
-__global__ __launch_bounds__(kT) void k_step_tail_bt(const TailArgs* __restrict__ t) { step_tail_body(blockIdx.y, t[blockIdx.x]); }
+  if (bx < A.g_lm) landmark_back_body(bx, A.g_lm, A.n_lm, A.dp, A.ldE, tail_E<SEL>(A), A.C, A.Cd, A.gr, A.dxc, A.s.inv_depth, A.dxl, A.invd2, A.scal, A.kmin, A.kmax);
+  else apply_step_body(bx - A.g_lm, A.n_kf, 0, A.s, A.dxc, A.dxl, A.poses2, A.vel2, A.ba2, A.bg2, A.invd2, A.scal, A.d, A.ld, tail_B<SEL>(A), tail_gc<SEL>(A), 1.0 / *A.radius, A.pose_const, A.jac);
+}
+__global__ __launch_bounds__(kT) void k_step_tail(TailArgs a) { step_tail_body<true>(blockIdx.x, a); }
+__global__ __launch_bounds__(kT) void k_step_tail_b(const TailArgs* __restrict__ t) { step_tail_body<false>(blockIdx.x, t[blockIdx.y]); }
+__global__ __launch_bounds__(kT) void k_step_tail_bt(const TailArgs* __restrict__ t) { step_tail_body<false>(blockIdx.y, t[blockIdx.x]); }
 
 struct BackTailArgs { BackArgs back; TailArgs tail; int g_lm; int fenced; unsigned timeout_ticks; GP<int> fail; };
 __global__ __launch_bounds__(kBT) void k_backsolve_tail(BackTailArgs a) {
@@ -2438,8 +2493,9 @@
     __builtin_amdgcn_fence(__ATOMIC_RELEASE, "workgroup");
     __syncthreads();
     const double inv_radius = 1.0 / *T.radius;
+    const double* const Bt = tail_B(T); const double* const gct = tail_gc(T);
     for (int vb = 0; vb * kBT < max(T.d, T.n_kf); ++vb)
-      apply_step_body<kBT, 2>(vb, T.n_kf, 0, T.s, T.dxc, T.dxl, T.poses2, T.vel2, T.ba2, T.bg2, T.invd2, T.scal, T.d, T.ld, T.B, T.gc, inv_radius, T.pose_const, T.jac);
+      apply_step_body<kBT, 2>(vb, T.n_kf, 0, T.s, T.dxc, T.dxl, T.poses2, T.vel2, T.ba2, T.bg2, T.invd2, T.scal, T.d, T.ld, Bt, gct, inv_radius, T.pose_const, T.jac);
     if (a.back.sp.dbg && threadIdx.x == 0) a.back.sp.dbg[55] = wall_clock64();
     return;
   }
@@ -2460,11 +2516,12 @@
     for (int i = threadIdx.x; i < T.dp; i += kBT) sdx_pose[i] = __hip_atomic_load(T.dxc + i, __ATOMIC_RELAXED, __HIP_MEMORY_SCOPE_AGENT);
     __syncthreads();
     const double inv_radius = 1.0 / *T.radius;
+    const double* const Bt = tail_B(T); const double* const gct = tail_gc(T);
     for (int vb = 0; vb * kBT < max(T.dp, T.n_kf); ++vb)
-      apply_step_body<kBT, 1>(vb, T.n_kf, 0, T.s, sdx_pose, T.dxl, T.poses2, T.vel2, T.ba2, T.bg2, T.invd2, T.scal, T.d, T.ld, T.B, T.gc, inv_radius, T.pose_const, T.jac);
+      apply_step_body<kBT, 1>(vb, T.n_kf, 0, T.s, sdx_pose, T.dxl, T.poses2, T.vel2, T.ba2, T.bg2, T.invd2, T.scal, T.d, T.ld, Bt, gct, inv_radius, T.pose_const, T.jac);
     return;
   }
-  landmark_back_body<kBT, true>((int)blockIdx.x - 2, a.g_lm, T.n_lm, T.dp, T.ldE, T.E, T.C, T.Cd, T.gr, T.dxc, T.s.inv_depth, T.dxl, T.invd2, T.scal, T.kmin, T.kmax);
+  landmark_back_body<kBT, true>((int)blockIdx.x - 2, a.g_lm, T.n_lm, T.dp, T.ldE, tail_E(T), T.C, T.Cd, T.gr, T.dxc, T.s.inv_depth, T.dxl, T.invd2, T.scal, T.kmin, T.kmax);
   if (ldbg) ldbg[2] = wall_clock64();
 }
 
@@ -2475,6 +2532,7 @@
   GP<const double> poses2, vel2, ba2, bg2, invd2;
   GP<unsigned long long> dbg;
   GP<double> hist;
+  int fused;
 };
 constexpr int kDT = 256;
 template <bool COHERENT = false>
@@ -2496,7 +2554,7 @@
   __syncthreads();
   if (s_skip) return;
   if (A.dbg && threadIdx.x == 0) A.dbg[2] = wall_clock64();
-  if (threadIdx.x < kStripes) const_cast<double*>((const double*)A.scal)[SC_COST + threadIdx.x] = 0.0;
+  if (!A.fused && threadIdx.x < kStripes) const_cast<double*>((const double*)A.scal)[SC_COST + threadIdx.x] = 0.0;
   if (threadIdx.x == 0) {
     struct { double radius, decrease, last_radius, cost, initial_cost, cost_before, cost_after, model, dxnorm, xnorm, gmax;
              double function_tol, gradient_tol, parameter_tol, min_rel_decrease; int max_iters, iter, successes, invalid_run, accepted, solved, done, termination, why, rejected; } lc;
@@ -2558,6 +2616,10 @@
     c->iter = lc.iter; c->successes = lc.successes; c->invalid_run = lc.invalid_run; c->accepted = lc.accepted; c->solved = lc.solved;
     c->done = lc.done; c->termination = lc.termination; c->why = lc.why; c->rejected = lc.rejected;
     if (hfail < kFailHandover) c->jfrozen = 1;
+    if (A.fused) {
+      c->lin_pending = accepted ? 1 : 0;
+      if (accepted) c->aset = c->aset ^ 1;
+    }
     s_iter = lc.iter; s_done = lc.done;
     if (A.hist) {
       double* h = A.hist + 8 * (it & 63);
@@ -2580,6 +2642,14 @@
     if ((A.n_lm & 1) && threadIdx.x == 0) A.invd[A.n_lm - 1] = A.invd2[A.n_lm - 1];
     for (int i = threadIdx.x; i < 7 * A.n_kf; i += kDT) A.poses[i] = A.poses2[i];
     for (int i = threadIdx.x; i < 3 * A.n_kf; i += kDT) { A.vel[i] = A.vel2[i]; A.ba[i] = A.ba2[i]; A.bg[i] = A.bg2[i]; }
+  }
+  if (A.fused) {
+    double* sc = const_cast<double*>((const double*)A.scal);
+    if (threadIdx.x < kStripes) {
+      if (s_done) sc[SC_COST + threadIdx.x] = 0.0;
+      else if (s_commit) sc[SC_COST + threadIdx.x] = __hip_atomic_load(sc + SC_COST_NEW + threadIdx.x, __ATOMIC_RELAXED, __HIP_MEMORY_SCOPE_AGENT);
+    }
+    reset_step_scalars(sc);
   }
   if (A.dbg && threadIdx.x == 0) A.dbg[4] = wall_clock64();
   if (A.rec && threadIdx.x == 0) {
@@ -2643,6 +2713,38 @@
 __global__ __launch_bounds__(kT) void k_cost_decide(CostArgs a, DecideArgs d, int end_zero) { cost_decide_body(blockIdx.x, a, d, end_zero); }
 __global__ __launch_bounds__(kT) void k_cost_decide_b(const CostArgs* __restrict__ t, const DecideArgs* __restrict__ d, int end_zero) { cost_decide_body(blockIdx.x, t[blockIdx.y], d[blockIdx.y], end_zero); }
 __global__ __launch_bounds__(kT) void k_cost_decide_bt(const CostArgs* __restrict__ t, const DecideArgs* __restrict__ d, int end_zero) { cost_decide_body(blockIdx.y, t[blockIdx.x], d[blockIdx.x], end_zero); }
+
+struct FusedArgs { LinArgs lin; DecideArgs dec; GP<double> cost_new; int nblocks; GP<const int> done; ZeroList zero; int zero_wgs; };
+__device__ __forceinline__ void lin_cost_decide_body(const int b, const FusedArgs& A) {
+  if (b >= A.nblocks) {
+    if (b - A.nblocks < A.zero_wgs) zero_list_share(A.zero, b - A.nblocks, A.zero_wgs);
+    return;
+  }
+  if (A.done && *A.done) return;
+  __shared__ double s_cost[kStripes];
+  __shared__ int s_last;
+  if (threadIdx.x < kStripes) s_cost[threadIdx.x] = 0.0;
+  const int standby = acc_set(A.lin.acc) ^ 1;
+  __syncthreads();
+  lin_visual_run(b, A.lin, standby, A.lin.s, s_cost);
+  __syncthreads();
+  if (threadIdx.x < 64) {
+    double v = threadIdx.x < kStripes ? s_cost[threadIdx.x] : 0.0;
+    v = wave_sum(v);
+    if (threadIdx.x == 0) {
+      if (v != 0.0) {
+        const double old = atomicAdd(A.cost_new + (b & (kStripes - 1)), v);
+        asm volatile("" ::"v"(old) : "memory");
+      }
+      const int t = atomicAdd(A.dec.ticket, 1);
+      s_last = t == A.nblocks - 1;
+      if (s_last) atomicExch(A.dec.ticket, 0);
+    }
+  }
+  __syncthreads();
+  if (s_last) lm_decide_body<true>(A.dec);
+}
+__global__ __launch_bounds__(kT) __attribute__((amdgpu_waves_per_eu(3))) void k_lin_cost_decide(FusedArgs a) { lin_cost_decide_body(blockIdx.x, a); }
 
 static StateP state_ptrs(const lvf_state* st) { return StateP{st->poses.p, st->vel.p, st->ba.p, st->bg.p, st->inv_depth.p, st->w_visual.p}; }
 static inline int grid(int n) { return (n + kT - 1) / kT; }
@@ -2669,6 +2771,10 @@
   bool back_tail_merged = false; BackTailArgs bt{}; size_t bt_lds = 0;
   CostArgs cost{};
   DecideArgs dec{};
+  bool fused_ok = false;
+  AccSel acc{};
+  ZeroList stand0{}, stand1{};
+  FusedArgs fused{};
 };
 
 void stage_clock_free(StageClock* k);
@@ -3014,6 +3120,24 @@
     a.hist = nullptr;
     if (lm_history) { LVF_TRY(p->dbg_hist.ensure(8 * 64)); a.hist = p->dbg_hist.p; }
   }
+  {
+    static const bool fused_on = [] { const char* e = std::getenv("LVF_FUSED_LIN"); return !(e && e[0] == '0'); }();
+    c.fused_ok = fused_on && c.fast && p->compact && !c.has_prior && c.merged_level0 && p->n_lm > 0 && c.lin.nblocks > 0 && c.cost.nblocks > 0 &&
+                 (!c.has_imu || (c.imu_in_cost && c.lin.v.imu.pre));
+    p->acc1_ready = false;
+    if (c.fused_ok) {
+      ZeroList fz{};
+      for (int k = 0; k < c.zero_end.count; ++k) {
+        double* q0 = c.zero_end.p[k];
+        if (q0 == p->B.p || q0 == p->gc.p || q0 == p->C.p || q0 == p->gr.p) continue;
+        fz.p[fz.count] = q0; fz.n[fz.count] = c.zero_end.n[k]; fz.tri[fz.count] = c.zero_end.tri[k]; ++fz.count;
+      }
+      FusedArgs& f = c.fused;
+      f.lin = c.lin; f.lin.s = s2; f.lin.cost = nullptr; f.lin.scal_reset = nullptr; f.lin.dbg = nullptr;
+      f.dec = c.dec; f.dec.fused = 1;
+      f.cost_new = p->scal.p + SC_COST_NEW; f.nblocks = c.lin.nblocks; f.done = done; f.zero = fz; f.zero_wgs = kEndZeroWgs;
+    }
+  }
   c.batchable = c.fast && p->compact && c.has_imu && !c.has_prior && c.merged_level0 && c.lin.nblocks > 0 && c.cost.nblocks > 0;
   { const StateP sp = state_ptrs(p->st); std::memcpy(p->chain_state, &sp, sizeof(sp)); }
   p->chain_tcw = p->tc && p->tc->wblk.n ? p->tc->wblk.p : nullptr;
@@ -3028,10 +3152,34 @@
   const double* w = p->tc && p->tc->wblk.n ? p->tc->wblk.p : nullptr;
   return w != p->chain_tcw;
 }
-
-enum { ST_IMU_LIN = 0, ST_LIN_VISUAL, ST_TF_REDUCE, ST_PREPARE, ST_SCHUR_SP0, ST_SP_LEVELS, ST_CHOL, ST_BACKSOLVE, ST_STEP_TAIL, ST_COST, ST_DECIDE, ST_N };
+static int ensure_acc1(lvf_problem* p) {
+  Chain& c = *p->chain;
+  if (!c.fused_ok || p->acc1_ready) return LVF_OK;
+  hipStream_t q = p->ctx->stream;
+  LVF_TRY(p->B1.ensure(p->B.n)); LVF_TRY(p->gc1.ensure(p->gc.n)); LVF_TRY(p->C1.ensure(p->C.n)); LVF_TRY(p->gr1.ensure(p->gr.n));
+  LVF_TRY(p->E1.ensure(p->E.n)); LVF_TRY(p->slotB1.ensure(p->slotB.n));
+  LVF_HIP(hipMemsetAsync(p->E1.p, 0, p->E1.n * 8, q));
+  hipLaunchKernelGGL(k_tf_slots_zero, dim3(256), dim3(kT), 0, q, 0, 0, (const int*)nullptr, (const int*)nullptr, (const int*)nullptr, (const int*)nullptr,
+                     (int*)nullptr, p->n_slots.p, p->slotB1.p);
+  LVF_HIP(hipGetLastError());
+  c.acc = AccSel{&p->ctl.p->aset, p->B1.p, p->gc1.p, p->C1.p, p->gr1.p, p->E1.p, p->slotB1.p};
+  c.stand0 = ZeroList{}; c.stand1 = ZeroList{};
+  for (int k = 0; k < c.zero_end.count; ++k) {
+    double* q0 = c.zero_end.p[k];
+    double* q1 = q0 == p->B.p ? p->B1.p : q0 == p->gc.p ? p->gc1.p : q0 == p->C.p ? p->C1.p : q0 == p->gr.p ? p->gr1.p : nullptr;
+    if (!q1) continue;
+    c.stand0.p[c.stand0.count] = q0; c.stand0.n[c.stand0.count] = c.zero_end.n[k]; c.stand0.tri[c.stand0.count] = c.zero_end.tri[k]; ++c.stand0.count;
+    c.stand1.p[c.stand1.count] = q1; c.stand1.n[c.stand1.count] = c.zero_end.n[k]; c.stand1.tri[c.stand1.count] = c.zero_end.tri[k]; ++c.stand1.count;
+  }
+  c.fused.lin.acc = c.acc;
+  p->acc1_ready = true;
+  return LVF_OK;
+}
+
+enum { ST_IMU_LIN = 0, ST_LIN_VISUAL, ST_TF_REDUCE, ST_PREPARE, ST_SCHUR_SP0, ST_SP_LEVELS, ST_CHOL, ST_BACKSOLVE, ST_STEP_TAIL, ST_COST, ST_DECIDE, ST_FUSED, ST_N };
 static const char* const kStageNames[ST_N] = {"k_zero_multi (only when the accumulators are not known clean)", "k_lin_visual", "k_tf_reduce (+ sparse level 0)", "k_prepare (+ sparse level 1)", "k_schur_sp0 (+ a sparse level)", "k_sp_eliminate (the levels left)",
-                                             "k_chol_step (all block steps)", "k_chol_backsolve", "k_step_tail", "k_cost_decide (candidate cost incl. the ImuError factors; its last workgroup closes the iteration; + prior passes)", "k_lm_decide (windows without visual blocks)"};
+                                             "k_chol_step (all block steps)", "k_chol_backsolve", "k_step_tail", "k_cost_decide (candidate cost incl. the ImuError factors; its last workgroup closes the iteration; + prior passes)", "k_lm_decide (windows without visual blocks)",
+                                             "k_lin_cost_decide (fused chain: linearisation at the candidate + its cost; its last workgroup closes the iteration)"};
 constexpr int kClockReps = 16, kClockLaunches = 48;
 struct StageClock {
   hipEvent_t ev[kClockReps][ST_N + 1]; int launches[ST_N]; bool on = false; int rep = 0;
@@ -3059,14 +3207,18 @@
   k->launches[stage_done] = launches;
 }
 
-static int enqueue_linearize(lvf_problem* p, double huber, bool gated, bool iteration = false) {
+static inline void acc_patch(SpArgs& a, const AccSel* acc) {
+  if (acc && a.src.B) { a.src.sel = acc->sel; a.src.B1 = (const double*)(double*)acc->B; a.src.gc1 = (const double*)(double*)acc->gc; }
+}
+
+static int enqueue_linearize(lvf_problem* p, double huber, bool gated, bool iteration = false, const AccSel* acc = nullptr, bool lin = true) {
   hipStream_t q = p->ctx->stream;
   if (chain_stale(p)) LVF_TRY(build_chain(p));
   const Chain& c = *p->chain;
   const StateP s = state_ptrs(p->st);
   double* cost = p->scal.p + SC_COST;
   bool imu_done = false;
-  const bool clean = c.fast && p->accum_clean;
+  const bool clean = !lin || (c.fast && p->accum_clean);
   p->accum_clean = false;
   if (p->clk && p->clk->on) (void)hipEventRecord(p->clk->ev[p->clk->rep][0], q);
   if (!clean) LVF_CHAIN_LAUNCH(p, ST_IMU_LIN, k_zero_multi, dim3(512, c.zero.count), dim3(kT), 0, q, c.zero);
@@ -3080,13 +3232,19 @@
     static const bool lin_timing = std::getenv("LVF_LIN_TIMING") != nullptr;
     if (lin_timing) { LVF_TRY(p->dbg_lin.ensure((size_t)la.v.n_tfw * 24 + 8)); la.dbg = p->dbg_lin.p; }
     static const size_t lds_pad = [] { const char* e = std::getenv("LVF_LIN_LDS_PAD"); return e ? (size_t)std::atoi(e) : (size_t)0; }();
-    LVF_CHAIN_LAUNCH(p, ST_LIN_VISUAL, k_lin_visual, dim3(la.nblocks), dim3(kT), c.lin_lds + lds_pad, q, la);
-    stage_mark(p, ST_LIN_VISUAL, 1);
+    if (lin) LVF_CHAIN_LAUNCH(p, ST_LIN_VISUAL, k_lin_visual, dim3(la.nblocks), dim3(kT), c.lin_lds + lds_pad, q, la);
+    stage_mark(p, ST_LIN_VISUAL, lin ? 1 : 0);
     if (p->compact) {
       TfReduceArgs ra = c.red;
       if (!gated) ra.done = nullptr;
       if (!iteration) { ra.nblocks = ra.own_blocks; ra.ride.nblocks = 0; }
-      LVF_CHAIN_LAUNCH(p, ST_TF_REDUCE, k_tf_reduce, dim3(ra.nblocks), dim3(kT), ra.ride.nblocks > 0 ? c.red_lds : 0, q, ra);
+      int zero_wgs = 0;
+      if (acc) {
+        ra.acc = *acc; acc_patch(ra.ride, acc);
+        ra.pending = lin ? nullptr : &p->ctl.p->lin_pending;
+        ra.stand0 = c.stand0; ra.stand1 = c.stand1; ra.zero_wgs = zero_wgs = kEndZeroWgs;
+      }
+      LVF_CHAIN_LAUNCH(p, ST_TF_REDUCE, k_tf_reduce, dim3(ra.nblocks + zero_wgs), dim3(kT), ra.ride.nblocks > 0 ? c.red_lds : 0, q, ra);
     }
     stage_mark(p, ST_TF_REDUCE, p->compact ? 1 : 0);
     if (lin_timing) {
@@ -3178,11 +3336,12 @@
   return LVF_OK;
 }
 
-static int enqueue_reduced_system(lvf_problem* p, const double* radius_dev, bool reset_scalars, bool gated, bool* level0_done) {
+static int enqueue_reduced_system(lvf_problem* p, const double* radius_dev, bool reset_scalars, bool gated, bool* level0_done, const AccSel* acc = nullptr) {
   hipStream_t q = p->ctx->stream;
   const Chain& c = *p->chain;
   const bool early = c.early && level0_done != nullptr;
   PrepArgs pa = early ? c.prep_early : c.prep;
+  if (acc) { pa.acc = *acc; acc_patch(pa.ride, acc); }
   pa.radius = radius_dev;
   if (!reset_scalars) pa.scal = nullptr;
   if (!gated) pa.done = nullptr;
@@ -3196,6 +3355,7 @@
     LVF_TRY(await_band_work(p));
     if (c.merged_level0) {
       SchurSp0Args sa = c.ssp0;
+      if (acc) { sa.acc = *acc; acc_patch(sa.sp, acc); acc_patch(sa.sp_b, acc); acc_patch(sa.sp_c, acc); }
       if (!gated) sa.done = nullptr;
       if (!level0_done) { sa.nblocks = sa.n_work; sa.sp.nblocks = 0; sa.sp_b.nblocks = 0; sa.sp_c.nblocks = 0; }
       static const bool schur_timing = std::getenv("LVF_SCHUR_TIMING") != nullptr;
@@ -3228,10 +3388,13 @@
   return LVF_OK;
 }
 
-static int enqueue_iteration(lvf_problem* p, bool end_zero) {
+enum { kFusedOn = 1, kFusedNoLin = 2, kFusedTail = 4 };
+static int enqueue_iteration(lvf_problem* p, bool end_zero, int fused = 0) {
   hipStream_t q = p->ctx->stream;
   if (chain_stale(p)) LVF_TRY(build_chain(p));
   const Chain& c = *p->chain;
+  if (!c.fused_ok || !p->acc1_ready) fused = 0;
+  const AccSel* acc = (fused & kFusedOn) ? &c.acc : nullptr;
   static const bool sp_timing = std::getenv("LVF_SP_TIMING") != nullptr;
   if (sp_timing && c.early) {
     const int n_nodes = p->sp_levels.n ? p->sp_levels.first[p->sp_levels.n - 1] + p->sp_levels.count[p->sp_levels.n - 1] : 0;
@@ -3257,12 +3420,15 @@
       }
     }
   }
-  LVF_TRY(enqueue_linearize(p, p->huber, true, true));
+  LVF_TRY(enqueue_linearize(p, p->huber, true, true, acc, !(fused & kFusedNoLin)));
   bool level0_done = false;
-  LVF_TRY(enqueue_reduced_system(p, &p->ctl.p->radius, true, true, &level0_done));
+  LVF_TRY(enqueue_reduced_system(p, &p->ctl.p->radius, true, true, &level0_done, acc));
   const int own0 = level0_done ? c.first_own_level : 0;
-  for (int lv = own0; lv < c.n_levels; ++lv)
-    LVF_CHAIN_LAUNCH(p, ST_SP_LEVELS, k_sp_eliminate, dim3(c.sp[lv].nblocks), dim3(256), c.sp_lds[lv], q, c.sp[lv]);
+  for (int lv = own0; lv < c.n_levels; ++lv) {
+    SpArgs la = c.sp[lv];
+    acc_patch(la, acc);
+    LVF_CHAIN_LAUNCH(p, ST_SP_LEVELS, k_sp_eliminate, dim3(la.nblocks), dim3(256), c.sp_lds[lv], q, la);
+  }
   stage_mark(p, ST_SP_LEVELS, std::max(0, c.n_levels - own0));
   for (int kb = 0; kb < p->nb; ++kb) {
     CholArgs cha = c.chol;
@@ -3278,15 +3444,29 @@
     if (c.back_tail_merged) {
       BackTailArgs bt = c.bt;
       if (back_timing) bt.back.sp.dbg = p->dbg.p;
+      if (acc) bt.tail.acc = *acc;
       LVF_CHAIN_LAUNCH(p, ST_BACKSOLVE, k_backsolve_tail, dim3(2 + c.bt.g_lm), dim3(kBT), c.bt_lds, q, bt);
       stage_mark(p, ST_BACKSOLVE, 1);
       stage_mark(p, ST_STEP_TAIL, 0);
     } else {
       LVF_CHAIN_LAUNCH(p, ST_BACKSOLVE, k_chol_backsolve, dim3(1), dim3(kBT), c.back_lds, q, ba);
       stage_mark(p, ST_BACKSOLVE, 1);
-      LVF_CHAIN_LAUNCH(p, ST_STEP_TAIL, k_step_tail, dim3(c.tail.nblocks), dim3(kT), c.tail_lds, q, c.tail);
+      TailArgs ta = c.tail;
+      if (acc) ta.acc = *acc;
+      LVF_CHAIN_LAUNCH(p, ST_STEP_TAIL, k_step_tail, dim3(ta.nblocks), dim3(kT), c.tail_lds, q, ta);
       stage_mark(p, ST_STEP_TAIL, 1);
     }
+  }
+  if (fused & kFusedTail) {
+    FusedArgs fa = c.fused;
+    fa.lin.huber = p->huber;
+    LVF_CHAIN_LAUNCH(p, ST_FUSED, k_lin_cost_decide, dim3(fa.nblocks + fa.zero_wgs), dim3(kT), c.lin_lds, q, fa);
+    stage_mark(p, ST_COST, 0);
+    stage_mark(p, ST_FUSED, 1);
+    p->accum_clean = false;
+    p->linearized = false;
+    LVF_HIP(hipGetLastError());
+    return LVF_OK;
   }
   CostArgs ca = c.cost;
   ca.huber = p->huber;
@@ -3346,6 +3526,7 @@
   p->no_chain = true; p->unchained_solves = 0; p->chain_ready = false; p->handover_retries += 1;
   if (p->force_handover_timeouts > 0) p->force_handover_timeouts -= 1;
   c->done = 0; c->termination = 1; c->why = LVF_WHY_MAX_ITERATIONS;
+  c->aset = 0; c->lin_pending = 0;
   p->accum_clean = false;
   return upload_ctl(p, *c);
 }
@@ -3990,15 +4171,18 @@
   ctl_from_options(o, radius, 2.0, reps + 2, false, &c);
   p->huber = o->huber_a;
   LVF_TRY(upload_ctl(p, c));
-  LVF_TRY(enqueue_iteration(p, true));
+  const bool fz = p->chain->fused_ok && !p->no_chain;
+  if (fz) LVF_TRY(ensure_acc1(p));
+  LVF_TRY(enqueue_iteration(p, true, fz ? kFusedOn | kFusedTail : 0));
   int nk = 0;
   for (int r = 0; r < reps; ++r) {
     k.on = true; k.rep = r; k.nk = 0;
-    const int rc = enqueue_iteration(p, true);
+    const int rc = enqueue_iteration(p, true, fz ? kFusedOn | kFusedNoLin | kFusedTail : 0);
     k.on = false;
     nk = k.nk;
     LVF_TRY(rc);
   }
+  if (fz) LVF_TRY(enqueue_iteration(p, true, kFusedOn | kFusedNoLin));
   LVF_HIP(hipStreamSynchronize(q));
   for (int r = 0; r < reps; ++r) {
     for (int i = 0; i < ST_N; ++i) {
@@ -4090,12 +4274,26 @@
   const auto wall0 = std::chrono::steady_clock::now();
   bool timed_out = false;
   for (int first = 0;;) {
+    const bool fz = p->chain->fused_ok && !p->no_chain && o->max_num_iterations - first >= 2;
+    if (fz) LVF_TRY(ensure_acc1(p));
+    bool fused_tail = false;
     for (int it = first; it < o->max_num_iterations; ++it) {
-      LVF_TRY(enqueue_iteration(p, true));
+      const int f = fz ? kFusedOn | (it > first ? kFusedNoLin : 0) | (it + 1 < o->max_num_iterations ? kFusedTail : 0) : 0;
+      LVF_TRY(enqueue_iteration(p, true, f));
+      fused_tail = (f & kFusedTail) != 0;
       if (it >= first + 1) LVF_TRY(wait_for_iteration(p, it));
       if (p->rec->done) break;
       if (o->max_solver_time_in_seconds > 0.0 &&
           std::chrono::duration<double>(std::chrono::steady_clock::now() - wall0).count() >= o->max_solver_time_in_seconds) { timed_out = true; break; }
+    }
+    if (fused_tail) {
+      const Chain& ch = *p->chain;
+      ZeroList z = ch.stand0;
+      for (int k = 0; k < ch.stand1.count && z.count < kZeroListMax; ++k) { z.p[z.count] = ch.stand1.p[k]; z.n[z.count] = ch.stand1.n[k]; z.tri[z.count] = ch.stand1.tri[k]; ++z.count; }
+      hipLaunchKernelGGL(k_zero_multi, dim3(512, z.count), dim3(kT), 0, p->ctx->stream, z);
+      LVF_HIP(hipGetLastError());
+      LVF_HIP(hipMemsetAsync(p->scal.p + SC_COST, 0, kStripes * 8, p->ctx->stream));
+      p->accum_clean = ch.stand0.count + ch.stand1.count <= kZeroListMax;
     }
     const bool known_handover = p->rec->done && p->rec->why == LVF_WHY_HANDOVER && !p->no_chain;
     if (tail && !known_handover) LVF_TRY(tail(user));
```

After: 5137 iter/s, median of 6. 1.04x the previous value.
